# gmongaras/Stable-Diffusion-3-From-Scratch

Hardware: AMD Instinct MI355X
Metric: train images/sec MMDiT-B 256^2 bf16 (higher is better)
Workload: dtype bf16

## Files before the change

stable-diffusion-3-from-scratch_amd/_lib.py:

```python
import ctypes
import os
import re

_HERE = os.path.dirname(os.path.abspath(__file__))
def experiment(name: str, default: str) -> str:
    return os.environ.get(name, default) if os.environ.get("MMDIT_EXPERIMENTS") == "1" else default


LIB_PATH = os.environ.get("MMDIT_LIB") or os.path.join(_HERE, "libmmdit_hip.so")
HEADER_PATH = os.path.join(_HERE, "..", "include", "mmdit_hip.h")
HEADER_EXT_PATH = os.path.join(_HERE, "..", "include", "mmdit_hip_ext.h")
HEADER_HD128_PATH = os.path.join(_HERE, "..", "include", "mmdit_hip_hd128.h")
HEADER_ROPE3_PATH = os.path.join(_HERE, "..", "include", "mmdit_hip_rope3.h")

F32, BF16 = 0, 1
ACT_NONE, ACT_SILU, ACT_SWIGLU, ACT_SWIGLU_BWD = 0, 1, 2, 3
PREC_BF16, PREC_SPLIT = 0, 1
FP8 = 2

_vp, _i, _i64, _f, _d = ctypes.c_void_p, ctypes.c_int, ctypes.c_int64, ctypes.c_float, ctypes.c_double


class GemmArgs(ctypes.Structure):
    _fields_ = [
        ("A", _vp), ("a_dtype", _i), ("a_kmajor", _i), ("lda", _i64),
        ("B", _vp), ("b_dtype", _i), ("b_kmajor", _i), ("ldb", _i64),
        ("C", _vp), ("c_dtype", _i), ("ldc", _i64),
        ("M", _i), ("N", _i), ("K", _i),
        ("bias", _vp),
        ("act", _i),
        ("gate", _vp), ("ld_gate", _i64), ("rows_per_batch", _i),
        ("residual", _vp), ("ld_res", _i64),
        ("aux", _vp), ("aux_dtype", _i), ("ld_aux", _i64),
        ("accumulate", _i),
        ("precision", _i),
        ("split_k", _i),
        ("stream_k", _i),
        ("conv_mode", _i), ("conv_H", _i), ("conv_W", _i), ("conv_C", _i),
        ("scale_a", _vp), ("scale_b", _vp), ("scale_mode", _i), ("c_scales", _vp),
        ("dbias", _vp),
        ("cu_budget", _i),
    ]


class LnFwdProblem(ctypes.Structure):
    _fields_ = [("x", ctypes.c_void_p), ("acc", ctypes.c_void_p), ("gate", ctypes.c_void_p), ("ld_gate", ctypes.c_int64), ("x_out", ctypes.c_void_p),
                ("scale", ctypes.c_void_p), ("shift", ctypes.c_void_p), ("ld_mod", ctypes.c_int64), ("rows", ctypes.c_int), ("rows_per_batch", ctypes.c_int),
                ("out", ctypes.c_void_p), ("mean", ctypes.c_void_p), ("rstd", ctypes.c_void_p)]


class LnBwdProblem(ctypes.Structure):
    _fields_ = [("dout", ctypes.c_void_p), ("x", ctypes.c_void_p), ("mean", ctypes.c_void_p), ("rstd", ctypes.c_void_p), ("scale", ctypes.c_void_p),
                ("ld_mod", ctypes.c_int64), ("dres", ctypes.c_void_p), ("rows", ctypes.c_int), ("rows_per_batch", ctypes.c_int),
                ("dx", ctypes.c_void_p), ("dscale", ctypes.c_void_p), ("dshift", ctypes.c_void_p), ("ld_dmod", ctypes.c_int64),
                ("acc", ctypes.c_void_p), ("gate", ctypes.c_void_p), ("ld_gate", ctypes.c_int64), ("dacc", ctypes.c_void_p), ("dgate", ctypes.c_void_p),
                ("ld_dgate", ctypes.c_int64), ("dbias", ctypes.c_void_p), ("ld_dbias", ctypes.c_int64)]


class QkProblem(ctypes.Structure):
    _fields_ = [("qkv", ctypes.c_void_p), ("wq", ctypes.c_void_p), ("wk", ctypes.c_void_p), ("rope_cos", ctypes.c_void_p), ("rope_sin", ctypes.c_void_p),
                ("tokens", ctypes.c_int), ("tok0", ctypes.c_int), ("dqkv", ctypes.c_void_p), ("dwq", ctypes.c_void_p), ("dwk", ctypes.c_void_p)]


class MlpBwdProblem(ctypes.Structure):
    _fields_ = [("dh", ctypes.c_void_p), ("gu", ctypes.c_void_p), ("dgu", ctypes.c_void_p), ("rows", ctypes.c_int), ("dbias", ctypes.c_void_p)]


class QkEpilogue(ctypes.Structure):
    _fields_ = [("wq", _vp), ("wk", _vp), ("rope_cos", _vp), ("rope_sin", _vp), ("tokens", _i), ("tok0", _i)]


_SIGNATURES = {
    "mmdit_abi_version": ([], _i),
    "mmdit_struct_size": ([_i], _i),
    "mmdit_build_arch": ([], ctypes.c_char_p),
    "mmdit_gemm": ([ctypes.POINTER(GemmArgs), _vp], _i),
    "mmdit_gemm_grouped": ([ctypes.POINTER(GemmArgs), _i, _vp], _i),
    "mmdit_gemm_plan": ([ctypes.POINTER(GemmArgs), _i], _i),
    "mmdit_gemm_set_workspace": ([_vp, ctypes.c_longlong], _i),
    "mmdit_debug_occupy": ([_i, ctypes.c_longlong, _vp], _i),
    "mmdit_gemm_set_claiming": ([_i], _i),
    "mmdit_gemm_get_claiming": ([], _i),
    "mmdit_device_cus": ([], _i),
    "mmdit_gemm_qkv_norm_rope": ([ctypes.POINTER(GemmArgs), ctypes.POINTER(QkEpilogue), _i, _i, _i, _vp, _vp, _vp, _vp], _i),
    "mmdit_gemm_zero_mask": ([ctypes.POINTER(GemmArgs), _i, ctypes.POINTER(ctypes.c_uint)], _i),
    "mmdit_fp8_amax": ([_vp, _i, _i64, _vp, _vp], _i),
    "mmdit_fp8_quantize": ([_vp, _i, _i64, _vp, _vp, _vp, _vp], _i),
    "mmdit_fp8_quantize_delayed": ([_vp, _i, _i64, _vp, _i, ctypes.c_float, _vp, _vp], _i),
    "mmdit_mxfp8_quantize": ([_vp, _i, _i, _i, _i64, _vp, _vp, _vp], _i),
    "mmdit_ln_modulate_fwd_mx": ([_vp, _vp, _i, _vp, _i64, _vp, _vp, _vp, _i64, _i, _i, _i, _vp, _vp, _vp, _vp, _vp], _i),
    "mmdit_swiglu_fwd_mx": ([_vp, _i, _i, _i, _vp, _vp, _vp], _i),
    "mmdit_attn_fwd_mx": ([_vp, _vp, _vp, _i, _i, _i, _i, ctypes.c_float, _vp, _vp, _vp, _vp, _vp], _i),
    "mmdit_cast": ([_vp, _i, _vp, _i, _i64, _vp], _i),
    "mmdit_ln_modulate_fwd": ([ctypes.POINTER(LnFwdProblem), _i, _i, _i, _i, _vp], _i),
    "mmdit_ln_modulate_bwd": ([ctypes.POINTER(LnBwdProblem), _i, _i, _i, _vp], _i),
    "mmdit_qk_norm_rope_fwd": ([ctypes.POINTER(QkProblem), _i, _i, _i, _i, _i, _vp, _vp, _vp, _vp], _i),
    "mmdit_qk_norm_rope_bwd": ([ctypes.POINTER(QkProblem), _i, _vp, _vp, _vp, _i, _i, _i, _i, _i, _i, _vp], _i),
    "mmdit_qk_norm_rope_fwd_merge": ([ctypes.POINTER(QkProblem), _i, _i, _i, _i, _i, _vp, _vp, _vp, _vp], _i),
    "mmdit_qk_norm_rope_bwd_merge": ([ctypes.POINTER(QkProblem), _i, _vp, _vp, _vp, _i, _i, _i, _i, _i, _i, _vp], _i),
    "mmdit_mlp_act_bwd": ([ctypes.POINTER(MlpBwdProblem), _i, _i, _i, _i, _vp], _i),
    "mmdit_gate_residual_fwd": ([_vp, _vp, _i, _vp, _i64, _i, _i, _i, _vp, _vp], _i),
    "mmdit_text_rmsnorm_fwd": ([_vp, _i, _vp, _vp, _vp, _vp, _i, _i, _i, _i, _vp, _vp, _i, _vp], _i),
    "mmdit_text_rmsnorm_bwd": ([_vp, _vp, _i, _vp, _i, _vp, _vp, _vp, _vp, _i, _i, _i, _i, _vp, _vp, _vp, _vp, _vp], _i),
    "mmdit_attn_fwd": ([_vp, _vp, _vp, _i, _i, _i, _i, _f, _i, _vp, _vp, _vp, _vp], _i),
    "mmdit_attn_bwd_qk": ([_vp] * 9 + [_i, _i, _i, _i, _f] + [_vp] * 11 + [_vp], _i),
    "mmdit_attn_bwd": ([_vp, _vp, _vp, _vp, _vp, _vp, _vp, _vp, _vp, _i, _i, _i, _i, _f, _vp, _vp, _vp, _i, _vp], _i),
    "mmdit_attn_fwd_kv": ([_vp, _vp, _vp, _i, _i, _i, _i, _i, _f, _i, _vp, _vp, _vp, _vp], _i),
    "mmdit_attn_bwd_kv": ([_vp, _vp, _vp, _vp, _vp, _vp, _vp, _vp, _vp, _i, _i, _i, _i, _i, _f, _vp, _vp, _vp, _i, _vp], _i),
    "mmdit_swiglu_fwd": ([_vp, _vp, _i, _i, _i, _vp], _i),
    "mmdit_gelu_fwd": ([_vp, _vp, _i, _i, _i, _vp], _i),
    "mmdit_silu_bwd": ([_vp, _i, _vp, _vp, _i, _i, _i, _vp, _i, _vp], _i),
    "mmdit_gate_residual_bwd": ([_vp, _vp, _i, _vp, _i64, _i, _i, _i, _vp, _i, _vp, _i64, _vp, _i64, _vp], _i),
    "mmdit_flow_loss": ([_vp, _vp, _vp, _i, _i64, _f, _vp, _vp, _vp, _vp], _i),
    "mmdit_colsum": ([_vp, _i, _i, _i, _i64, _vp, _vp], _i),
    "mmdit_vae_nchw_to_nhwc": ([_vp, _i, _i, _i, _i, _i, _i, ctypes.c_float, ctypes.c_float, _vp, _vp], _i),
    "mmdit_vae_nhwc_to_nchw": ([_vp, _i, _i, _i, _i, _i, ctypes.c_float, ctypes.c_float, _vp, _vp], _i),
    "mmdit_vae_im2col3x3": ([_vp, _i, _i, _i, _i, _i, _vp, _vp], _i),
    "mmdit_vae_groupnorm": ([_vp, _i, _vp, _vp, _i, _i, _i, _i, _i, ctypes.c_float, _i, _vp, _vp, _i, _vp], _i),
    "mmdit_vae_pad_cast": ([_vp, _i, _i, _i, _i, _i, _i, _vp, _vp], _i),
    "mmdit_vae_softmax_rows": ([_vp, _i, _i, _i, ctypes.c_float, _vp, _vp], _i),
    "mmdit_vae_attn_fwd": ([_vp, _vp, _vp, _i, _i, _i, _i, _f, _vp, _vp], _i),
    "mmdit_patchify": ([_vp, _i, _i, _i, _i, _i, _vp, _i, _vp], _i),
    "mmdit_unpatchify": ([_vp, _i, _i, _i, _i, _i, _vp, _i, _vp], _i),
    "mmdit_time_embed_fwd": ([_vp, _vp, _vp, _i, _i, _vp, _i, _vp], _i),
    "mmdit_time_embed_bwd": ([_vp, _i, _vp, _vp, _vp, _i, _i, _vp, _vp], _i),
    "mmdit_grad_sumsq": ([_vp, _vp, _vp, _i, _vp, _vp], _i),
    "mmdit_clip_coef": ([_vp, _i, _vp, _f, _vp, _vp], _i),
    "mmdit_adamw_step": ([_vp, _vp, _vp, _i, _vp, _vp, _d, _d, _d, _d, _d, _vp], _i),
    "mmdit_adamw_step_dlr": ([_vp, _vp, _vp, _i, _vp, _vp, _vp, _d, _d, _d, _d, _vp], _i),
    "mmdit_cast_multi": ([_vp, _vp, _vp, _i, _vp], _i),
}
_EXT_SIGNATURES = {
    "mmdit_attn_fwd_e4m3": ([_vp, _vp, _vp, _i, _i, _i, _i, _f, _vp, _vp, _vp, _vp, _vp], _i),
}
ATTN_E4M3_KEY_TILE, ATTN_E4M3_QUERY_TILE = 64, 128
_HD128_SIGNATURES = {
    "mmdit_attn_fwd_hd128": _SIGNATURES["mmdit_attn_fwd"],
    "mmdit_attn_bwd_hd128": _SIGNATURES["mmdit_attn_bwd"],
    "mmdit_qk_norm_rope_fwd_hd128": _SIGNATURES["mmdit_qk_norm_rope_fwd"],
    "mmdit_qk_norm_rope_bwd_hd128": _SIGNATURES["mmdit_qk_norm_rope_bwd"],
}
ATTN_HD128_KEY_TILE, ATTN_HD128_QUERY_TILE = 32, 128
QK_HD128_MAX_HEADS, QK_HD128_RL_MIN_ROWS = 21, 2048
_ROPE3_SIGNATURES = {
    "mmdit_qk_norm_rope3_fwd": ([ctypes.POINTER(QkProblem), _i, _i, _i, _i, _i, _i, _vp, _vp, _vp, _vp], _i),
    "mmdit_qk_norm_rope3_bwd": ([ctypes.POINTER(QkProblem), _i, _vp, _vp, _vp, _i, _i, _i, _i, _i, _i, _i, _vp], _i),
}
HEAD_DIMS = (64, 128)
ADAMW_CHUNK = 65536
ABI_VERSION = 10
_STRUCTS = [("mmdit_gemm_args", GemmArgs), ("mmdit_ln_fwd_problem", LnFwdProblem), ("mmdit_ln_bwd_problem", LnBwdProblem),
            ("mmdit_qk_problem", QkProblem), ("mmdit_mlp_bwd_problem", MlpBwdProblem), ("mmdit_adamw_tensor", None), ("mmdit_cast_tensor", None), ("mmdit_qk_epilogue", QkEpilogue)]

_lib = None


def declared_symbols():
    with open(HEADER_PATH) as f:
        txt = f.read()
    return sorted(set(re.findall(r"\b(mmdit_[a-z0-9_]+)\s*\(", txt)) - {"mmdit_stream_t"})


def declared_ext_symbols():
    with open(HEADER_EXT_PATH) as f:
        txt = f.read()
    return sorted(set(re.findall(r"\b(mmdit_[a-z0-9_]+)\s*\(", txt)) - {"mmdit_stream_t"})


def declared_hd128_symbols():
    with open(HEADER_HD128_PATH) as f:
        txt = f.read()
    return sorted(set(re.findall(r"\b(mmdit_[a-z0-9_]+)\s*\(", txt)) - {"mmdit_stream_t"})


def declared_rope3_symbols():
    with open(HEADER_ROPE3_PATH) as f:
        txt = f.read()
    return sorted(set(re.findall(r"\b(mmdit_[a-z0-9_]+)\s*\(", txt)) - {"mmdit_stream_t"})


def lib():
    global _lib
    if _lib is None:
        if not os.path.exists(LIB_PATH):
            raise RuntimeError(
                f"{LIB_PATH} is missing: build it with `python __graft_entry__.py build` "
                "(hipcc --offload-arch=gfx950).  There is no PyTorch/CPU fallback for the MMDiT hot path.")
        try:
            import torch
            if torch.cuda.is_available():
                torch.cuda.init()
        except ImportError:
            pass
        L = ctypes.CDLL(LIB_PATH)
        for name, (argtypes, restype) in list(_SIGNATURES.items()) + list(_EXT_SIGNATURES.items()) + list(_HD128_SIGNATURES.items()) + list(_ROPE3_SIGNATURES.items()):
            fn = getattr(L, name)
            fn.argtypes = argtypes
            fn.restype = restype
        if L.mmdit_abi_version() != ABI_VERSION:
            raise RuntimeError(f"{LIB_PATH}: ABI version {L.mmdit_abi_version()}, this binding is written for {ABI_VERSION}: rebuild (python __graft_entry__.py build)")
        for which, (name, struct) in enumerate(_STRUCTS):
            if struct is not None and L.mmdit_struct_size(which) != ctypes.sizeof(struct):
                raise RuntimeError(f"{LIB_PATH}: sizeof({name}) = {L.mmdit_struct_size(which)}, the binding's ctypes mirror has {ctypes.sizeof(struct)} bytes")
        _lib = L
    return _lib


ERR_ARG, ERR_DTYPE, ERR_SHAPE = -1, -2, -3


def check(status: int, what: str):
    if status != 0:
        kind = {-1: "invalid argument", -2: "dtype combination not built", -3: "unsupported shape"}.get(status, f"hipError {status}")
        raise RuntimeError(f"{what} failed: {kind}")
```

stable-diffusion-3-from-scratch_amd/build.py:

```python
import hashlib
import os
import subprocess
import sys
from concurrent.futures import ThreadPoolExecutor

HERE = os.path.dirname(os.path.abspath(__file__))
CSRC = os.path.join(HERE, "csrc")
LIB = os.path.join(HERE, "libmmdit_hip.so")
HEADER = os.path.join(HERE, "..", "include", "mmdit_hip.h")
HEADER_EXT = os.path.join(HERE, "..", "include", "mmdit_hip_ext.h")
HEADER_HD128 = os.path.join(HERE, "..", "include", "mmdit_hip_hd128.h")
HEADER_ROPE3 = os.path.join(HERE, "..", "include", "mmdit_hip_rope3.h")
SOURCES = ["gemm.hip", "gemm_dma.hip", "gemm_lean.hip", "gemm8p.hip", "gemm8p_inf.hip", "rowops.hip", "attention.hip", "attention_e4m3.hip", "attention_hd128.hip", "rowops_rope3.hip", "vae.hip", "vae_attn.hip", "optim.hip"]
HIPCC = os.environ.get("HIPCC", "/opt/rocm/bin/hipcc")
FLAGS = ["--offload-arch=gfx950", "-O3", "-std=c++17", "-fPIC"] + os.environ.get("MMDIT_EXTRA_HIPCC_FLAGS", "").split()
SOURCE_FLAGS = {"vae_attn.hip": ["-mllvm", "-amdgpu-mfma-vgpr-form=1"]}


def _sha(paths, extra=""):
    h = hashlib.sha256(extra.encode())
    for p in paths:
        with open(p, "rb") as f:
            h.update(os.path.basename(p).encode() + b"\0" + f.read() + b"\0")
    return h.hexdigest()


def _read(path):
    try:
        with open(path) as f:
            return f.read().strip()
    except OSError:
        return None


def source_hash(src):
    headers = sorted(os.path.join(CSRC, f) for f in os.listdir(CSRC) if f.endswith(".h")) + [HEADER, HEADER_EXT, HEADER_HD128, HEADER_ROPE3]
    if src == "gemm8p_inf.hip":
        headers.append(os.path.join(CSRC, "gemm8p.hip"))
    return _sha([os.path.join(CSRC, src)] + headers, " ".join([HIPCC] + FLAGS + SOURCE_FLAGS.get(src, [])))


def build(force: bool = False, verbose: bool = False) -> str:
    want = {src: source_hash(src) for src in SOURCES}

    def cc(src):
        obj = os.path.join(CSRC, src.replace(".hip", ".o"))
        if not force and os.path.exists(obj) and _read(obj + ".sha") == want[src]:
            return obj, False
        cmd = [HIPCC] + FLAGS + SOURCE_FLAGS.get(src, []) + ["-c", os.path.join(CSRC, src), "-o", obj]
        if verbose:
            print(" ".join(cmd), flush=True)
        subprocess.run(cmd, check=True)
        with open(obj + ".sha", "w") as f:
            f.write(want[src])
        return obj, True

    with ThreadPoolExecutor(max_workers=8) as ex:
        res = list(ex.map(cc, SOURCES))
    objs = [o for o, _ in res]
    libsha = hashlib.sha256("".join(want[s] for s in SOURCES).encode()).hexdigest()
    if force or any(c for _, c in res) or not os.path.exists(LIB) or _read(LIB + ".sha") != libsha:
        cmd = [HIPCC, "--offload-arch=gfx950", "-shared", "-fPIC", "-o", LIB] + objs
        if verbose:
            print(" ".join(cmd), flush=True)
        subprocess.run(cmd, check=True)
        with open(LIB + ".sha", "w") as f:
            f.write(libsha)
    return LIB


def is_current() -> bool:
    libsha = hashlib.sha256("".join(source_hash(s) for s in SOURCES).encode()).hexdigest()
    return os.path.exists(LIB) and _read(LIB + ".sha") == libsha


if __name__ == "__main__":
    print(build(force="--force" in sys.argv, verbose=True))
```

stable-diffusion-3-from-scratch_amd/csrc/gemm.hip:

```cpp
#include "gemm_common.h"
#include <stdlib.h>

using namespace gemm;

namespace {

constexpr int BM = 128, BN = 128;
constexpr int RM_PITCH = 144;
constexpr int KM_PITCH = 320;
constexpr int TILE_BYTES = 20480;
constexpr int CHUNKS = 4;

template <typename T> struct Stage;
template <> struct Stage<bf16_t> { u32x4 v[CHUNKS]; };
template <> struct Stage<float> { f32x4 v[CHUNKS][2]; };

template <bool KM>
__device__ __forceinline__ void chunk_coords(int c, int& r, int& kc) {
  if (!KM) { r = c >> 3; kc = (c & 7) * 8; }
  else { kc = c >> 4; r = (c & 15) * 8; }
}

template <typename T, bool KM>
__device__ __forceinline__ void load_tile(Stage<T>& st, const T* base, int64_t ld, int row0, int k0, int rows, int K, int tid) {
#pragma unroll
  for (int i = 0; i < CHUNKS; i++) {
    int c = tid + 256 * i, r, kc;
    chunk_coords<KM>(c, r, kc);
    bool ok = (row0 + r < rows) && (k0 + kc < K);
    const T* p = KM ? base + (int64_t)(k0 + kc) * ld + row0 + r : base + (int64_t)(row0 + r) * ld + k0 + kc;
    if constexpr (sizeof(T) == 2) {
      st.v[i] = ok ? *(const u32x4*)p : (u32x4){0, 0, 0, 0};
    } else {
      st.v[i][0] = ok ? *(const f32x4*)p : (f32x4){0, 0, 0, 0};
      st.v[i][1] = ok ? *(const f32x4*)(p + 4) : (f32x4){0, 0, 0, 0};
    }
  }
}

template <typename T, bool KM, bool SPLIT>
__device__ __forceinline__ void store_tile(const Stage<T>& st, char* hi, char* mid, char* lo, int tid) {
#pragma unroll
  for (int i = 0; i < CHUNKS; i++) {
    int c = tid + 256 * i, r, kc;
    chunk_coords<KM>(c, r, kc);
    int off = KM ? kc * KM_PITCH + r * 2 : r * RM_PITCH + kc * 2;
    if constexpr (sizeof(T) == 2) {
      *LDS_PTR(u32x4, hi + off) = st.v[i];
    } else {
      float f[8] = {st.v[i][0][0], st.v[i][0][1], st.v[i][0][2], st.v[i][0][3], st.v[i][1][0], st.v[i][1][1], st.v[i][1][2], st.v[i][1][3]};
      uint32_t h[4], md[4], l[4];
#pragma unroll
      for (int j = 0; j < 4; j++) {
        bf16_t h0 = f2bf(f[2 * j]), h1 = f2bf(f[2 * j + 1]);
        h[j] = (uint32_t)h0 | ((uint32_t)h1 << 16);
        if constexpr (SPLIT) {
          const float r0 = f[2 * j] - bf2f(h0), r1 = f[2 * j + 1] - bf2f(h1);
          const bf16_t m0 = f2bf(r0), m1 = f2bf(r1);
          md[j] = (uint32_t)m0 | ((uint32_t)m1 << 16);
          l[j] = pack_bf2(r0 - bf2f(m0), r1 - bf2f(m1));
        }
      }
      *LDS_PTR(u32x4, hi + off) = (u32x4){h[0], h[1], h[2], h[3]};
      if constexpr (SPLIT) {
        *LDS_PTR(u32x4, mid + off) = (u32x4){md[0], md[1], md[2], md[3]};
        *LDS_PTR(u32x4, lo + off) = (u32x4){l[0], l[1], l[2], l[3]};
      }
    }
  }
}

template <bool KM>
__device__ __forceinline__ bf16x8 load_frag(const char* tile, int r0, int ks, int lane) {
  if (!KM) {
    const char* p = tile + (r0 + (lane & 31)) * RM_PITCH + (ks * 16 + (lane >> 5) * 8) * 2;
    return *LDS_PTR(const bf16x8, p);
  } else {
    int kr = ks * 16 + (lane >> 5) * 8 + ((lane & 15) >> 2);
    int col = r0 + 16 * ((lane >> 4) & 1) + (lane & 3) * 4;
    const char* p = tile + kr * KM_PITCH + col * 2;
    s16x4 lo = lds_tr16(p), hi = lds_tr16(p + 4 * KM_PITCH);
    s16x8 r = {lo[0], lo[1], lo[2], lo[3], hi[0], hi[1], hi[2], hi[3]};
    return __builtin_bit_cast(bf16x8, r);
  }
}

template <typename TA, typename TB, bool A_KM, bool B_KM, bool SPLIT, typename TC, typename TAUX>
__global__ __launch_bounds__(256) void gemm_kernel(GroupParams gp) {
  constexpr int NT = SPLIT ? 6 : 2;
  constexpr int NSTAGE = SPLIT ? 1 : 2;
  extern __shared__ __attribute__((aligned(16))) char smem[];

  int tm, tn, sk;
  const Problem& p = locate_tile(gp, blockIdx.x, tm, tn, sk);
  const int m0 = tm * BM, n0 = tn * BN;

  const int tid = threadIdx.x, lane = tid & 63, wave = tid >> 6;
  const int wm = wave >> 1, wn = wave & 1;
  const TA* A = (const TA*)p.A;
  const TB* B = (const TB*)p.B;
  const int M = p.M, N = p.N, K = p.K;
  const int64_t lda = p.lda, ldb = p.ldb;

  f32x16 acc[2][2];
#pragma unroll
  for (int i = 0; i < 2; i++)
#pragma unroll
    for (int j = 0; j < 2; j++)
#pragma unroll
      for (int r = 0; r < 16; r++) acc[i][j][r] = 0.f;

  Stage<TA> sa;
  Stage<TB> sb;
  const int nk = (K + BK - 1) / BK;
  auto tile_ptr = [&](int stage, int which) { return smem + (stage * NT + which) * TILE_BYTES; };

  load_tile<TA, A_KM>(sa, A, lda, m0, 0, M, K, tid);
  load_tile<TB, B_KM>(sb, B, ldb, n0, 0, N, K, tid);
  store_tile<TA, A_KM, SPLIT>(sa, tile_ptr(0, 0), tile_ptr(0, 2), tile_ptr(0, 4), tid);
  store_tile<TB, B_KM, SPLIT>(sb, tile_ptr(0, 1), tile_ptr(0, 3), tile_ptr(0, 5), tid);
  __syncthreads();

  int cur = 0;
  for (int kt = 0; kt < nk; kt++) {
    const bool more = kt + 1 < nk;
    if (more) {
      load_tile<TA, A_KM>(sa, A, lda, m0, (kt + 1) * BK, M, K, tid);
      load_tile<TB, B_KM>(sb, B, ldb, n0, (kt + 1) * BK, N, K, tid);
    }
    const char* ta = tile_ptr(cur, 0);
    const char* tb = tile_ptr(cur, 1);
#pragma unroll
    for (int ks = 0; ks < BK / 16; ks++) {
      bf16x8 a[2], b[2];
#pragma unroll
      for (int i = 0; i < 2; i++) a[i] = load_frag<A_KM>(ta, wm * 64 + i * 32, ks, lane);
#pragma unroll
      for (int j = 0; j < 2; j++) b[j] = load_frag<B_KM>(tb, wn * 64 + j * 32, ks, lane);
      if constexpr (SPLIT) {
        bf16x8 a1[2], b1[2], a2[2], b2[2];
#pragma unroll
        for (int i = 0; i < 2; i++) { a1[i] = load_frag<A_KM>(tile_ptr(cur, 2), wm * 64 + i * 32, ks, lane); a2[i] = load_frag<A_KM>(tile_ptr(cur, 4), wm * 64 + i * 32, ks, lane); }
#pragma unroll
        for (int j = 0; j < 2; j++) { b1[j] = load_frag<B_KM>(tile_ptr(cur, 3), wn * 64 + j * 32, ks, lane); b2[j] = load_frag<B_KM>(tile_ptr(cur, 5), wn * 64 + j * 32, ks, lane); }
#pragma unroll
        for (int i = 0; i < 2; i++)
#pragma unroll
          for (int j = 0; j < 2; j++) {
            acc[i][j] = __builtin_amdgcn_mfma_f32_32x32x16_bf16(b[j], a2[i], acc[i][j], 0, 0, 0);
            acc[i][j] = __builtin_amdgcn_mfma_f32_32x32x16_bf16(b1[j], a1[i], acc[i][j], 0, 0, 0);
            acc[i][j] = __builtin_amdgcn_mfma_f32_32x32x16_bf16(b2[j], a[i], acc[i][j], 0, 0, 0);
            acc[i][j] = __builtin_amdgcn_mfma_f32_32x32x16_bf16(b[j], a1[i], acc[i][j], 0, 0, 0);
            acc[i][j] = __builtin_amdgcn_mfma_f32_32x32x16_bf16(b1[j], a[i], acc[i][j], 0, 0, 0);
            acc[i][j] = __builtin_amdgcn_mfma_f32_32x32x16_bf16(b[j], a[i], acc[i][j], 0, 0, 0);
          }
      } else {
#pragma unroll
        for (int i = 0; i < 2; i++)
#pragma unroll
          for (int j = 0; j < 2; j++) acc[i][j] = __builtin_amdgcn_mfma_f32_32x32x16_bf16(b[j], a[i], acc[i][j], 0, 0, 0);
      }
    }
    if (more) {
      if constexpr (NSTAGE == 1) __syncthreads();
      const int nxt = NSTAGE == 1 ? 0 : cur ^ 1;
      store_tile<TA, A_KM, SPLIT>(sa, tile_ptr(nxt, 0), tile_ptr(nxt, 2), tile_ptr(nxt, 4), tid);
      store_tile<TB, B_KM, SPLIT>(sb, tile_ptr(nxt, 1), tile_ptr(nxt, 3), tile_ptr(nxt, 5), tid);
      __syncthreads();
      cur = nxt;
    }
  }

  __syncthreads();
  epilogue<TC, TAUX>(acc, p, gp, m0, n0, wm, wn, lane, sk, smem + wave * EP_WAVE_BYTES);
}

template <typename TA, typename TB, bool A_KM, bool B_KM, bool SPLIT, typename TC, typename TAUX>
int launch(const GroupParams& gp, hipStream_t s) {
  constexpr int smem = (SPLIT ? 6 : 4) * TILE_BYTES;
  auto k = gemm_kernel<TA, TB, A_KM, B_KM, SPLIT, TC, TAUX>;
  static unsigned long long attr_done = 0;
  if (!mmdit_device_once(attr_done)) {
    hipError_t e = hipFuncSetAttribute((const void*)k, hipFuncAttributeMaxDynamicSharedMemorySize, smem);
    if (e != hipSuccess) return (int)e;
    mmdit_device_mark(attr_done);
  }
  hipLaunchKernelGGL(k, dim3(gp.total_tiles), dim3(256), smem, s, gp);
  return mmdit_launch_status();
}

template <typename TA, typename TB, bool SPLIT, typename TC, typename TAUX>
int dispatch_layout(bool a_km, bool b_km, const GroupParams& p, hipStream_t s) {
  if (!a_km && !b_km) return launch<TA, TB, false, false, SPLIT, TC, TAUX>(p, s);
  if (!a_km && b_km) return launch<TA, TB, false, true, SPLIT, TC, TAUX>(p, s);
  if (a_km && b_km) return launch<TA, TB, true, true, SPLIT, TC, TAUX>(p, s);
  return MMDIT_ERR_DTYPE;
}

template <typename TA, typename TB, bool SPLIT>
int dispatch_out(int c_dt, int aux_dt, bool a_km, bool b_km, const GroupParams& p, hipStream_t s) {
  if (c_dt == MMDIT_F32 && aux_dt == MMDIT_F32) return dispatch_layout<TA, TB, SPLIT, float, float>(a_km, b_km, p, s);
  if (c_dt == MMDIT_F32 && aux_dt == MMDIT_BF16) return dispatch_layout<TA, TB, SPLIT, float, bf16_t>(a_km, b_km, p, s);
  if (c_dt == MMDIT_BF16 && aux_dt == MMDIT_BF16) return dispatch_layout<TA, TB, SPLIT, bf16_t, bf16_t>(a_km, b_km, p, s);
  if (c_dt == MMDIT_BF16 && aux_dt == MMDIT_F32) return dispatch_layout<TA, TB, SPLIT, bf16_t, float>(a_km, b_km, p, s);
  return MMDIT_ERR_DTYPE;
}

inline bool aligned16(const void* p) { return ((uintptr_t)p & 15) == 0; }

int check_problem(const mmdit_gemm_args* a) {
  MMDIT_CHECK_ARG(a->A && a->B && a->C);
  MMDIT_CHECK_ARG(a->M > 0 && a->N > 0 && a->K > 0 && a->N % 4 == 0);
  const int esa = a->a_dtype == MMDIT_F32 ? 4 : a->a_dtype == MMDIT_FP8 ? 1 : 2, esb = a->b_dtype == MMDIT_F32 ? 4 : a->b_dtype == MMDIT_FP8 ? 1 : 2, esc = a->c_dtype == MMDIT_F32 ? 4 : 2;
  MMDIT_CHECK_ARG(a->c_dtype == MMDIT_F32 || a->c_dtype == MMDIT_BF16 || (a->c_dtype == MMDIT_FP8 && a->act == MMDIT_ACT_SWIGLU && a->c_scales));
  MMDIT_CHECK_ARG(aligned16(a->A) && aligned16(a->B) && ((uintptr_t)a->C & (4 * esc - 1)) == 0);
  MMDIT_CHECK_ARG((a->lda * esa) % 16 == 0 && (a->ldb * esb) % 16 == 0 && a->ldc % 4 == 0);
  if (a->a_kmajor) { MMDIT_CHECK_ARG(a->M % 8 == 0 && a->lda >= a->M); } else { MMDIT_CHECK_ARG(a->K % 8 == 0 && a->lda >= a->K); }
  if (a->b_kmajor) { MMDIT_CHECK_ARG(a->N % 8 == 0 && a->ldb >= a->N); } else { MMDIT_CHECK_ARG(a->K % 8 == 0 && a->ldb >= a->K); }
  MMDIT_CHECK_ARG(a->ldc >= (a->act == MMDIT_ACT_SWIGLU ? a->N / 2 : a->act == MMDIT_ACT_SWIGLU_BWD ? 2 * a->N : a->N));
  if (a->bias) MMDIT_CHECK_ARG(aligned16(a->bias));
  if (a->gate) MMDIT_CHECK_ARG(a->residual && a->rows_per_batch > 0 && aligned16(a->gate) && a->ld_gate % 4 == 0);
  if (a->residual) MMDIT_CHECK_ARG(aligned16(a->residual) && a->ld_res % 4 == 0);
  if (a->aux) MMDIT_CHECK_ARG(a->ld_aux % 4 == 0 && ((uintptr_t)a->aux & 7) == 0);
  if (a->accumulate) MMDIT_CHECK_ARG(a->c_dtype == MMDIT_F32);
  return 0;
}

}

static void* g_ws[64] = {};
static long long g_ws_bytes[64] = {};
static unsigned g_sched_next[64] = {};
static int g_claiming[64] = {};
extern "C" int mmdit_gemm_set_claiming(int on) { g_claiming[mmdit_current_device()] = on != 0; return 0; }
extern "C" int mmdit_gemm_get_claiming(void) { return g_claiming[mmdit_current_device()]; }
extern "C" int mmdit_device_cus(void) {
  static int cus[64] = {};
  const int dev = mmdit_current_device();
  if (!cus[dev]) {
    int n = 0;
    if (hipDeviceGetAttribute(&n, hipDeviceAttributeMultiprocessorCount, dev) != hipSuccess || n < 8) { (void)hipGetLastError(); n = 256; }
    cus[dev] = n / 8 * 8;
  }
  return cus[dev];
}

struct PlannerSwitches {
  int cfg = -1, cfg_epi = -1;
  bool no_dma = false, no_streamk = false, no_persist = false;
  int lean = 1;
  bool qk8 = false;
  bool kdec_streamk = false, kdec_plain = false;
  int tail_s = 0, debug = 0;
  int epi_direct = 0, raster = 8;
};
#ifdef MMDIT_PROBES
static const PlannerSwitches& planner_switches() {
  static const PlannerSwitches sw = [] {
    PlannerSwitches w;
    auto num = [](const char* name, int& v) { if (const char* e = getenv(name)) v = atoi(e); };
    num("MMDIT_GEMM_CFG", w.cfg); num("MMDIT_GEMM_CFG_EPI", w.cfg_epi); num("MMDIT_GEMM_LEAN", w.lean); num("MMDIT_GEMM_TAIL_S", w.tail_s);
    num("MMDIT_GEMM_DEBUG", w.debug); num("MMDIT_GEMM_RASTER", w.raster);
    w.no_dma = getenv("MMDIT_GEMM_NO_DMA"); w.no_streamk = getenv("MMDIT_GEMM_NO_STREAMK"); w.no_persist = getenv("MMDIT_GEMM_NO_PERSIST");
    int qk8 = 0;
    num("MMDIT_QK_8PHASE", qk8); w.qk8 = qk8 > 0;
    if (const char* e = getenv("MMDIT_GEMM_EPI")) w.epi_direct = atoi(e) == 0;
    if (const char* e = getenv("MMDIT_GEMM_KDEC")) { w.kdec_streamk = e[0] == 's'; w.kdec_plain = e[0] == 'p'; }
    return w;
  }();
  return sw;
}
#else
static constexpr PlannerSwitches planner_switches() { return {}; }
#endif

static int pick_dma_cfg(const mmdit_gemm_args* args, int count, int split_k, bool stream_k, bool lean_ok, long cu) {
  const PlannerSwitches& sw = planner_switches();
  if (sw.cfg >= 0) return sw.cfg == CFG_320x256 && !lean_ok ? CFG_256x256 : sw.cfg;
  if (sw.cfg_epi >= 0 && args[0].gate) return sw.cfg_epi;
  if (stream_k) return CFG_256x256;
  long t128 = 0, t256 = 0;
  for (int i = 0; i < count; i++) {
    t128 += (long)((args[i].M + 127) / 128) * ((args[i].N + 127) / 128);
    t256 += (long)((args[i].M + 255) / 256) * ((args[i].N + 255) / 256);
  }
  const bool mx8 = args[0].a_dtype == MMDIT_FP8 && args[0].K % 128 == 0 && !args[0].gate && !args[0].residual && !args[0].aux &&
                   (args[0].c_dtype == MMDIT_BF16 || args[0].act == MMDIT_ACT_SWIGLU);
  const double r256 = mx8 ? 1.2 : args[0].a_dtype == MMDIT_FP8 ? 1.67 : 1.58;
  const double c128 = (double)((t128 * split_k + 2 * cu - 1) / (2 * cu)), c256 = r256 * (double)((t256 * split_k + cu - 1) / cu);
  if (lean_ok) {
    long t320 = 0;
    for (int i = 0; i < count; i++) t320 += (long)((args[i].M + 319) / 320) * ((args[i].N + 255) / 256);
    const double c320 = 1.25 * 1.58 * (double)((t320 + cu - 1) / cu);
    if (c320 < c256 && c320 < c128) return CFG_320x256;
  }
  return c256 < c128 ? CFG_256x256 : CFG_128x128;
}

static inline int split_k_of(const mmdit_gemm_args* a) { return a->split_k > 1 ? a->split_k : 1; }

struct QkRequest {
  const mmdit_qk_epilogue* qk;
  int heads, s_total;
  void* Q; void* K; void* V;
  unsigned no_raw;
};

enum GemmKernel { KERNEL_REG, KERNEL_DMA, KERNEL_WIDE, KERNEL_8P, KERNEL_8P_CONV };
struct GemmPlan {
  GroupParams gp;
  GemmKernel kernel;
  int cfg;
  bool a_km, b_km, fp8, mx8, ktail;
  int a_dt, b_dt, c_dt, aux_dt, precision;
  int cu;
  int* sched_page;
  int code;
  unsigned zero_mask;
};

struct DeviceState { bool claiming; void* ws; long long ws_bytes; };

static int choose_kernel(const mmdit_gemm_args* args, int count, const QkRequest* qkr, const DeviceState& ds, bool dma, bool conv, GemmPlan* pl) {
  const PlannerSwitches& sw = planner_switches();
  const mmdit_gemm_args* a0 = &args[0];
  const bool fp8 = pl->fp8;
  const int bk = fp8 ? 2 * BK : BK;
  const int split_k = split_k_of(a0);
  GroupParams& gp = pl->gp;
  gp.tail_first = -1; gp.tail_rounds = 0; gp.tail_G = 0;
  if (conv) MMDIT_CHECK_ARG(dma);
  const bool swiglu = a0->act == MMDIT_ACT_SWIGLU;
  if (swiglu) {
    if (!dma) return MMDIT_ERR_SHAPE;
    for (int i = 0; i < count; i++) {
      const mmdit_gemm_args* a = &args[i];
      MMDIT_CHECK_ARG(a->c_dtype == MMDIT_BF16 || (a->c_dtype == MMDIT_FP8 && a->c_scales && !a->aux && fp8 && a->scale_mode == 1 && a->c_dtype == a0->c_dtype));
      MMDIT_CHECK_ARG(!a->a_kmajor && !a->b_kmajor && (!a->aux || a->aux_dtype == MMDIT_BF16) && !a->gate && !a->residual &&
                      !a->accumulate && split_k == 1 && !a->stream_k && !a->conv_mode);
      if (a->N % 256 != 0) return MMDIT_ERR_SHAPE;
      MMDIT_CHECK_ARG(a->ldc >= a->N / 2 && a->ldc % 8 == 0 && aligned16(a->C));
      if (a->aux) MMDIT_CHECK_ARG(a->ld_aux >= a->N && a->ld_aux % 8 == 0 && aligned16(a->aux));
    }
  }
  const bool swiglu_bwd = a0->act == MMDIT_ACT_SWIGLU_BWD;
  if (swiglu_bwd) {
    if (!dma) return MMDIT_ERR_SHAPE;
    for (int i = 0; i < count; i++) {
      const mmdit_gemm_args* a = &args[i];
      MMDIT_CHECK_ARG(a->c_dtype == MMDIT_BF16 && !a->a_kmajor && a->b_kmajor && a->aux && a->aux_dtype == MMDIT_BF16 && !a->bias && !a->gate && !a->residual &&
                      !a->accumulate && split_k == 1 && !a->stream_k && !a->conv_mode && !fp8);
      MMDIT_CHECK_ARG(a->N % 8 == 0 && a->ldc >= 2 * a->N && a->ldc % 8 == 0 && aligned16(a->C) && a->ld_aux >= 2 * a->N && a->ld_aux % 8 == 0 && aligned16(a->aux));
      if (a->dbias) MMDIT_CHECK_ARG(((uintptr_t)a->dbias & 3) == 0);
    }
  }
  int bm = BM, bn = BN, cfg = CFG_128x128;
  const bool stream_k = dma && !sw.no_streamk && a0->stream_k && a0->c_dtype == MMDIT_F32 && split_k == 1 && a0->act == MMDIT_ACT_NONE && !a0->accumulate;
  bool lean_ok = dma && sw.lean > 0 && !fp8 && !conv && !stream_k && split_k == 1 && !a0->a_kmajor && a0->c_dtype == MMDIT_BF16 &&
                 (a0->act == MMDIT_ACT_NONE || a0->act == MMDIT_ACT_SILU || swiglu || swiglu_bwd) && !a0->accumulate;
  for (int i = 0; i < count && lean_ok; i++) {
    const mmdit_gemm_args* a = &args[i];
    lean_ok = (!a->aux || swiglu || swiglu_bwd) && !a->gate && !a->residual && a->N % 8 == 0 && a->ldc % 8 == 0 && aligned16(a->C) && (!a->b_kmajor || a->N >= 8);
  }
  if (dma) {
    cfg = pick_dma_cfg(args, count, split_k, stream_k, lean_ok, pl->cu);
    if (swiglu && cfg != CFG_320x256) cfg = CFG_256x256;
    if (swiglu_bwd) cfg = CFG_256x256;
    if (qkr && (fp8 || sw.qk8 || ds.claiming)) cfg = CFG_256x256;
    dma_cfg_tile(cfg, bm, bn);
  }
  const bool lean = lean_ok && (cfg == CFG_320x256 || (cfg == CFG_256x256 && sw.lean == 1));
  int tiles = 0, units = 0;
  int order[MAXG];
  for (int i = 0; i < count; i++) order[i] = i;
  if (stream_k && !sw.kdec_streamk)
    for (int i = 1; i < count; i++)
      for (int j = i; j > 0 && args[order[j]].K > args[order[j - 1]].K; j--) { const int t = order[j]; order[j] = order[j - 1]; order[j - 1] = t; }
  for (int i = 0; i < count; i++) {
    const mmdit_gemm_args* a = &args[order[i]];
    Problem& p = gp.p[i];
    p.A = a->A; p.B = a->B; p.C = a->C; p.aux = a->aux;
    p.bias = a->bias; p.gate = a->gate; p.residual = a->residual;
    p.lda = a->lda; p.ldb = a->ldb; p.ldc = a->ldc; p.ld_gate = a->ld_gate; p.ld_res = a->ld_res; p.ld_aux = a->ld_aux;
    p.M = a->M; p.N = a->N; p.K = a->K;
    p.rows_per_batch = a->rows_per_batch > 0 ? a->rows_per_batch : 1;
    p.conv_mode = a->conv_mode; p.cC = a->conv_C; p.cHp = a->conv_H + 2; p.cWp = a->conv_W + 2;
    p.cHo = a->conv_mode == 2 ? a->conv_H / 2 : a->conv_H; p.cWo = a->conv_mode == 2 ? a->conv_W / 2 : a->conv_W;
    p.tiles_n = (a->N + bn - 1) / bn;
    p.tiles_m = (a->M + bm - 1) / bm;
    p.tile_start = tiles;
    p.nk = a->K / bk;
    p.scale_a = (const float*)a->scale_a; p.scale_b = (const float*)a->scale_b; p.c_scales = (unsigned char*)a->c_scales;
    p.dbias = a->dbias;
    p.unit_start = units;
    tiles += p.tiles_n * p.tiles_m;
    units += p.tiles_n * p.tiles_m * p.nk;
    if (stream_k) MMDIT_CHECK_ARG(!a->aux && !a->gate && a->stream_k);
  }
  gp.stream_k = stream_k; gp.total_units = units;
  gp.mx = fp8 && a0->scale_mode == 1;
  int full_tiles = split_k > 1 ? 0 : tiles, tail_split = split_k;
  const bool tail_mode = stream_k && !sw.kdec_streamk;
  if (tail_mode) {
    gp.stream_k = 0;
    const int G = pl->cu * (cfg == CFG_128x128 ? 2 : 1), r = tiles % G;
    int nk_min = 1 << 30;
    for (int i = 0; i < count; i++) nk_min = gp.p[i].nk < nk_min ? gp.p[i].nk : nk_min;
    full_tiles = tiles - r;
    tail_split = 1;
    if (r) {
      double best = 1e30;
      for (int S = 1; S <= 64 && S * 2 <= nk_min; S++) {
        const double c = (double)((r * S + G - 1) / G) / S + (S > 1 ? 0.0028 * r * S : 0.0);
        if (c < best) { best = c; tail_split = S; }
      }
      if (sw.tail_s > 0 && sw.tail_s * 2 <= nk_min) { tail_split = sw.tail_s; best = -1.0; }
      if (full_tiles == G && !sw.kdec_plain) {
        const int nk_max = gp.p[0].nk;
        int first_short = G, nk_short = 0, nk_tail = 0;
        for (int i = 0; i < count; i++) {
          const Problem& q = gp.p[i];
          if (q.nk < nk_max && q.tile_start < G && first_short == G) { first_short = q.tile_start; nk_short = q.nk; }
          if (q.tile_start + q.tiles_m * q.tiles_n > full_tiles) nk_tail = q.nk > nk_tail ? q.nk : nk_tail;
        }
        const int E = G - first_short;
        if (E > 0) {
          double bbest = 1e30;
          int bS = 0, brounds = 0;
          for (int S = 1; S <= 64 && S * 2 <= nk_min; S++) {
            const int rounds = (r * S + E - 1) / E, extra = rounds * ((nk_tail + S - 1) / S);
            const double load = (double)(nk_short + extra) / nk_max, c = (load > 1.0 ? load - 1.0 : 0.0) + (S > 1 ? 0.0028 * r * S : 0.0);
            if (c < bbest) { bbest = c; bS = S; brounds = rounds; }
          }
          if (bbest < best) {
            tail_split = bS;
            if (!(ds.ws && ds.claiming)) { gp.tail_first = first_short; gp.tail_rounds = brounds; gp.tail_G = G; }
          }
        }
      }
    }
  }
  gp.persistent = !sw.no_persist;
  gp.count = count; gp.total_tiles = tiles; gp.act = a0->act; gp.accumulate = a0->accumulate; gp.split_k = tail_split; gp.full_tiles = full_tiles;
  gp.debug = sw.debug; gp.epi_direct = sw.epi_direct; gp.raster = sw.raster;
  if (split_k > 1) {
    MMDIT_CHECK_ARG(dma && a0->c_dtype == MMDIT_F32 && a0->act == MMDIT_ACT_NONE && !a0->accumulate && split_k <= 64);
    for (int i = 0; i < count; i++) MMDIT_CHECK_ARG(!args[i].aux && !args[i].gate);
  }
  bool wgrad8 = dma && !fp8 && !conv && !gp.stream_k && cfg == CFG_256x256 && a0->a_kmajor && a0->b_kmajor &&
            a0->c_dtype == MMDIT_F32 && a0->act == MMDIT_ACT_NONE;
  for (int i = 0; i < count && wgrad8; i++) {
    const mmdit_gemm_args* a = &args[i];
    wgrad8 = !a->bias && !a->gate && !a->residual && !a->aux && a->N % 4 == 0 && a->ldc % 4 == 0 && aligned16(a->C);
  }
  gp.ws_slots = nullptr; gp.ws_count = nullptr; gp.sched = nullptr;
  gp.qk_on = 0; gp.qkQ = gp.qkK = gp.qkV = nullptr; gp.qk_heads = 0; gp.qk_s_total = 0;
  if (qkr) {
    const bool mxqk = dma && fp8 && gp.mx && cfg == CFG_256x256 && !a0->a_kmajor && a0->c_dtype == MMDIT_BF16;
    if (!(lean || mxqk) || count > 2 || a0->act != MMDIT_ACT_NONE || a0->b_kmajor) return MMDIT_ERR_SHAPE;
    if (qkr->no_raw && !(cfg == CFG_256x256 && (mxqk || ds.claiming))) return MMDIT_ERR_SHAPE;
    for (int i = 0; i < count; i++) {
      if (order[i] != i || args[i].bias || args[i].N != 3 * qkr->heads * 64 || qkr->qk[i].tokens <= 0 || args[i].M % qkr->qk[i].tokens) return MMDIT_ERR_SHAPE;
      gp.qk[i].wq = qkr->qk[i].wq; gp.qk[i].wk = qkr->qk[i].wk;
      gp.qk[i].rcos = qkr->qk[i].rope_cos; gp.qk[i].rsin = qkr->qk[i].rope_sin;
      gp.qk[i].tokens = qkr->qk[i].tokens; gp.qk[i].tok0 = qkr->qk[i].tok0;
    }
    if (count == 1) gp.qk[1] = gp.qk[0];
    for (int i = 0; i < count; i++)
      if ((qkr->no_raw >> i) & 1) gp.p[i].C = nullptr;
    gp.qk_on = 1; gp.qk_heads = qkr->heads; gp.qk_s_total = qkr->s_total;
    gp.qkQ = (bf16_t*)qkr->Q; gp.qkK = (bf16_t*)qkr->K; gp.qkV = (bf16_t*)qkr->V;
  }
  if (wgrad8 && gp.split_k > 1) {
    const long long tail_tiles = tiles - full_tiles;
    if (ds.ws && tail_tiles <= 1024 && 8192 + tail_tiles * gp.split_k * 65536LL * 4 <= ds.ws_bytes) {
      gp.ws_count = (int*)ds.ws;
      gp.ws_slots = (float*)((char*)ds.ws + 8192);
    }
  }
  pl->zero_mask = 0;
  for (int i = 0; i < count; i++) {
    const Problem& q = gp.p[i];
    if (dma && !gp.ws_slots && (gp.stream_k || (gp.split_k > 1 && q.tile_start + q.tiles_m * q.tiles_n > gp.full_tiles))) pl->zero_mask |= 1u << order[i];
  }
  bool mx8 = dma && fp8 && cfg == CFG_256x256 && (!qkr || gp.mx) && !stream_k && split_k == 1 && (a0->act == MMDIT_ACT_NONE || swiglu) && !a0->accumulate;
  for (int i = 0; i < count && mx8; i++) {
    const mmdit_gemm_args* a = &args[i];
    mx8 = (a->c_dtype == MMDIT_BF16 || (swiglu && a->c_dtype == MMDIT_FP8)) && (!a->aux || (swiglu && a->c_dtype == MMDIT_BF16)) && !a->gate && !a->residual && a->K % 128 == 0 &&
          a->N % 8 == 0 && a->ldc % 8 == 0 && aligned16(a->C) && (int64_t)a->M * a->lda < (1ll << 32) && (int64_t)a->N * a->ldb < (1ll << 32);
  }
  const bool p8 = mx8 || wgrad8 || (lean && (cfg == CFG_256x256 || (cfg == CFG_320x256 && !qkr)));
  bool conv8 = conv && dma && !fp8 && cfg == CFG_256x256 && !stream_k && split_k == 1 && a0->act == MMDIT_ACT_NONE && !a0->accumulate &&
               (a0->c_dtype == MMDIT_BF16 || a0->c_dtype == MMDIT_F32);
  for (int i = 0; i < count && conv8; i++) {
    const mmdit_gemm_args* a = &args[i];
    conv8 = a->conv_mode && a->conv_C % 64 == 0 && !a->aux && !a->gate && (a->c_dtype == MMDIT_F32 || !a->residual) && a->N % 8 == 0 && a->ldc % 8 == 0 && aligned16(a->C) &&
            (!a->residual || (a->ld_res % 4 == 0 && aligned16(a->residual))) && (!a->bias || aligned16(a->bias));
  }
  if (swiglu_bwd && !p8) return MMDIT_ERR_SHAPE;
  pl->kernel = conv8 ? KERNEL_8P_CONV : p8 ? KERNEL_8P : lean ? KERNEL_WIDE : dma ? KERNEL_DMA : KERNEL_REG;
  pl->cfg = cfg; pl->mx8 = mx8;
  pl->code = dma ? (cfg | (gp.stream_k ? 16 : 0) | (tail_mode ? 32 : 0) | (lean || wgrad8 ? 128 : 0) | (p8 || conv8 ? 256 : 0)) : 64;
  const bool claimed = pl->kernel == KERNEL_8P && !mx8 && cfg == CFG_256x256 && gp.persistent && gp.tail_first < 0 && total_work(gp) > pl->cu;
  pl->sched_page = claimed && ds.ws && ds.claiming ? (int*)((char*)ds.ws + 4096) : nullptr;
  return 0;
}

static int plan_gemm(const mmdit_gemm_args* args, int count, const QkRequest* qkr, GemmPlan* pl) {
  MMDIT_CHECK_ARG(args && count >= 1 && count <= MAXG);
  const mmdit_gemm_args* a0 = &args[0];
  const int dev = mmdit_current_device();
  const DeviceState ds{g_claiming[dev] != 0, g_ws[dev], g_ws_bytes[dev]};
  const int cus = mmdit_device_cus();
  MMDIT_CHECK_ARG(a0->cu_budget == 0 || (a0->cu_budget >= 64 && a0->cu_budget <= cus && a0->cu_budget % 8 == 0));
  pl->cu = a0->cu_budget ? a0->cu_budget : cus;
  int aux_dt = -1;
  const bool fp8 = a0->a_dtype == MMDIT_FP8 || a0->b_dtype == MMDIT_FP8;
  bool dma = !planner_switches().no_dma && a0->precision == MMDIT_PREC_BF16 && a0->a_dtype == MMDIT_BF16 && a0->b_dtype == MMDIT_BF16;
  bool ktail = false;
  if (fp8) {
    MMDIT_CHECK_ARG(a0->a_dtype == MMDIT_FP8 && a0->b_dtype == MMDIT_FP8 && a0->precision == MMDIT_PREC_BF16 && split_k_of(a0) == 1 && !a0->stream_k);
    dma = true;
  }
  const int bk = fp8 ? 2 * BK : BK;
  bool conv = false;
  const int split_k = split_k_of(a0);
  for (int i = 0; i < count; i++) {
    const mmdit_gemm_args* a = &args[i];
    int rc = check_problem(a);
    if (rc) return rc;
    MMDIT_CHECK_ARG(a->a_dtype == a0->a_dtype && a->b_dtype == a0->b_dtype && a->c_dtype == a0->c_dtype && a->a_kmajor == a0->a_kmajor &&
                    a->b_kmajor == a0->b_kmajor && a->precision == a0->precision && a->act == a0->act && a->accumulate == a0->accumulate &&
                    a->cu_budget == a0->cu_budget);
    if (a->aux) { MMDIT_CHECK_ARG(aux_dt < 0 || aux_dt == a->aux_dtype); aux_dt = a->aux_dtype; }
    MMDIT_CHECK_ARG(split_k_of(a) == split_k);
    if (fp8) MMDIT_CHECK_ARG(!a->a_kmajor && !a->b_kmajor && a->K % bk == 0 && a->scale_a && a->scale_b && !a->conv_mode && a->scale_mode == a0->scale_mode &&
                             (a->scale_mode == 0 || (a->scale_mode == 1 && aligned16(a->scale_a) && aligned16(a->scale_b))));
    if (a->K % bk != 0) {
      if (!fp8 && a->a_kmajor && a->b_kmajor && a->c_dtype == MMDIT_F32 && a->K > bk && !a->conv_mode) ktail = true;
      else dma = false;
    }
    if (a->a_kmajor && a->M < 8) dma = false;
    if (a->b_kmajor && a->N < 8) dma = false;
    if (a->conv_mode) {
      MMDIT_CHECK_ARG((a->conv_mode == 1 || a->conv_mode == 2) && !a->a_kmajor && !a->b_kmajor && a->conv_C > 0 && a->conv_C % 32 == 0 && a->K == 9 * a->conv_C && a->K % BK == 0);
      MMDIT_CHECK_ARG(a->conv_H > 0 && a->conv_W > 0 && (a->conv_mode == 1 || (a->conv_H % 2 == 0 && a->conv_W % 2 == 0)));
      const int64_t px = a->conv_mode == 1 ? (int64_t)a->conv_H * a->conv_W : (int64_t)(a->conv_H / 2) * (a->conv_W / 2);
      MMDIT_CHECK_ARG(a->M % px == 0 && split_k == 1 && !a->stream_k && a->a_dtype == MMDIT_BF16 && a->b_dtype == MMDIT_BF16 && a->precision == MMDIT_PREC_BF16);
      MMDIT_CHECK_ARG((a->M / px) * (int64_t)(a->conv_H + 2) * (a->conv_W + 2) * a->conv_C * 2 < (1ll << 32));
      conv = true;
      continue;
    }
    if ((int64_t)(a->a_kmajor ? a->K : a->M) * a->lda * 2 >= (1ll << 32) || (int64_t)(a->b_kmajor ? a->K : a->N) * a->ldb * 2 >= (1ll << 32)) {
      MMDIT_CHECK_ARG(!fp8);
      dma = false;
    }
  }
  pl->a_km = a0->a_kmajor; pl->b_km = a0->b_kmajor; pl->fp8 = fp8; pl->ktail = ktail;
  pl->a_dt = a0->a_dtype; pl->b_dt = a0->b_dtype; pl->c_dt = a0->c_dtype; pl->precision = a0->precision;
  pl->aux_dt = aux_dt >= 0 ? aux_dt : a0->c_dtype == MMDIT_FP8 ? MMDIT_BF16 : a0->c_dtype;
  int rc = choose_kernel(args, count, qkr, ds, dma, conv, pl);
  if (rc == 0 && dma && ktail && pl->kernel != KERNEL_8P) rc = choose_kernel(args, count, qkr, ds, false, conv, pl);
  return rc;
}

static int launch_plan(const GemmPlan& pl, hipStream_t s) {
  const GroupParams* gp = &pl.gp;
  GroupParams claimed;
  if (pl.sched_page) {
    claimed = pl.gp;
    claimed.sched = pl.sched_page + (__atomic_fetch_add(&g_sched_next[mmdit_current_device()], 1u, __ATOMIC_RELAXED) & 63u) * 16;
    gp = &claimed;
  }
  switch (pl.kernel) {
    case KERNEL_8P_CONV: return launch_gemm8_conv(pl.c_dt == MMDIT_F32, *gp, s, pl.cu);
    case KERNEL_8P: return launch_gemm8(pl.cfg, pl.a_km, pl.b_km, *gp, s, pl.cu, pl.ktail, pl.mx8);
    case KERNEL_WIDE: return launch_lean_cfg(pl.cfg, pl.b_km, *gp, s, pl.cu);
    case KERNEL_DMA: return launch_dma(pl.cfg, pl.a_km, pl.b_km, pl.c_dt, pl.aux_dt, pl.fp8, *gp, s, pl.cu);
    case KERNEL_REG:
      if (pl.precision == MMDIT_PREC_BF16 && pl.a_dt == MMDIT_BF16 && pl.b_dt == MMDIT_BF16) return dispatch_out<bf16_t, bf16_t, false>(pl.c_dt, pl.aux_dt, pl.a_km, pl.b_km, *gp, s);
      if (pl.precision == MMDIT_PREC_SPLIT && pl.a_dt == MMDIT_F32 && pl.b_dt == MMDIT_F32) return dispatch_out<float, float, true>(pl.c_dt, pl.aux_dt, pl.a_km, pl.b_km, *gp, s);
      return MMDIT_ERR_DTYPE;
  }
  return MMDIT_ERR_ARG;
}

extern "C" int mmdit_gemm_grouped(const mmdit_gemm_args* args, int count, mmdit_stream_t stream) {
  GemmPlan pl;
  const int rc = plan_gemm(args, count, nullptr, &pl);
  return rc ? rc : launch_plan(pl, (hipStream_t)stream);
}

extern "C" int mmdit_gemm_qkv_norm_rope(const mmdit_gemm_args* args, const mmdit_qk_epilogue* qk, int count, int heads, int s_total,
                                        void* Q, void* K, void* V, mmdit_stream_t stream) {
  MMDIT_CHECK_ARG(args && qk && count >= 1 && count <= 2 && heads > 0 && s_total > 0 && Q && K && V);
  for (int i = 0; i < count; i++) {
    MMDIT_CHECK_ARG(qk[i].wq && qk[i].wk && qk[i].tokens > 0 && qk[i].tok0 >= 0 && qk[i].tok0 + qk[i].tokens <= s_total);
    MMDIT_CHECK_ARG((qk[i].rope_cos == nullptr) == (qk[i].rope_sin == nullptr));
  }
  mmdit_gemm_args tmp[2];
  unsigned no_raw = 0;
  for (int i = 0; i < count; i++) {
    tmp[i] = args[i];
    if (!tmp[i].C) { tmp[i].C = Q; no_raw |= 1u << i; }
  }
  const QkRequest r{qk, heads, s_total, Q, K, V, no_raw};
  GemmPlan pl;
  const int rc = plan_gemm(no_raw ? tmp : args, count, &r, &pl);
  return rc ? rc : launch_plan(pl, (hipStream_t)stream);
}

extern "C" int mmdit_gemm_set_workspace(void* ptr, long long bytes) {
  MMDIT_CHECK_ARG((ptr == nullptr && bytes == 0) || (ptr != nullptr && bytes >= 8192 + 65536 * 4 && ((uintptr_t)ptr & 15) == 0));
  const int dev = mmdit_current_device();
  g_ws[dev] = ptr;
  g_ws_bytes[dev] = bytes;
  return 0;
}

namespace {
__global__ void occupy_kernel(long long cycles, int* sink) {
  __shared__ int pad[256];
  pad[threadIdx.x & 255] = threadIdx.x;
  const long long t0 = __builtin_readcyclecounter();
  while ((long long)__builtin_readcyclecounter() - t0 < cycles) __builtin_amdgcn_s_sleep(32);
  if (cycles < 0) sink[0] = pad[0];
}
}
extern "C" int mmdit_debug_occupy(int wgs, long long cycles, mmdit_stream_t stream) {
  MMDIT_CHECK_ARG(wgs >= 1 && wgs <= 256 && cycles >= 0 && cycles <= (1ll << 36));
  hipLaunchKernelGGL(occupy_kernel, dim3(wgs), dim3(64), 0, (hipStream_t)stream, cycles, (int*)nullptr);
  return mmdit_launch_status();
}

extern "C" int mmdit_gemm_plan(const mmdit_gemm_args* args, int count) {
  GemmPlan pl;
  const int rc = plan_gemm(args, count, nullptr, &pl);
  return rc ? rc : pl.code;
}

extern "C" int mmdit_gemm_zero_mask(const mmdit_gemm_args* args, int count, unsigned* mask) {
  MMDIT_CHECK_ARG(mask);
  GemmPlan pl;
  const int rc = plan_gemm(args, count, nullptr, &pl);
  *mask = rc ? 0 : pl.zero_mask;
  return rc;
}

extern "C" int mmdit_gemm(const mmdit_gemm_args* a, mmdit_stream_t stream) {
  MMDIT_CHECK_ARG(a);
  return mmdit_gemm_grouped(a, 1, stream);
}
```

stable-diffusion-3-from-scratch_amd/csrc/gemm8p.hip:

```cpp
#include "gemm_tile.h"

using namespace gemm;
typedef __attribute__((ext_vector_type(4))) int i32x4_t;

namespace {

template <int MT> struct Geo {
  static constexpr int QR = MT / 4, FI = QR / 16;
  static constexpr int HTA = 2 * QR * 128, HTB = 16384;
  static constexpr int KBUF = 2 * HTA + 2 * HTB;
  static constexpr int XA0 = 0, XA1 = HTA, XB0 = 2 * HTA, XB1 = 2 * HTA + HTB;
  static constexpr int PA = 2 * QR / 8;
  static constexpr int PAW = (PA + 7) / 8;
  static constexpr int STAGE0 = MT == 256 ? 2 * KBUF : 0;
  static constexpr int SMEM = MT == 256 ? 2 * KBUF + 8 * EP32_WAVE_BYTES : 2 * KBUF;
  static constexpr int NB32 = MT / 64;
};

enum Epi8 { EPI_BF16 = 0, EPI_SWIGLU = 1, EPI_QK = 2, EPI_F32 = 3, EPI_SWIGLU_BWD = 4, EPI_F32R = 5 };

#define SWZ_R(r) (((r) >> 1) & 7)
#define SWZ_K(k) ((((k) & 3) << 2) ^ ((((k) >> 3) & 1) << 1))

template <int MT> struct AccT { f32x4 a[2][2][2 * Geo<MT>::FI]; };

template <int MT>
__device__ __forceinline__ f32x4& grp(AccT<MT>& acc, int i32, int q) {
  constexpr int FI = Geo<MT>::FI;
  const int f16 = i32 * 2 + (q >> 2), j16 = q & 3;
  return acc.a[f16 / FI][j16 >> 1][(f16 % FI) * 2 + (j16 & 1)];
}

template <int MT, bool SC = false, bool LAUNDER = SC>
__device__ __forceinline__ void epi8_bf16(AccT<MT>& acc, const Problem& p, const GroupParams& gp, int m0, int n0, int wm, int wn, int lane, char* stage, float alpha = 1.f) {
  bf16_t* C = (bf16_t*)p.C;
  const float* bias = p.bias;
  const int wr = lane & 15, wq = lane >> 4;
  const int rr = lane >> 3, rc = lane & 7;
  const int colw = n0 + wn * 64;
  float bv[4][4];
  if (bias) {
#pragma unroll
    for (int j = 0; j < 4; j++) {
      const int c = colw + j * 16 + wq * 4;
      ld4(bias + (c < p.N ? c : 0), bv[j]);
      if (c >= p.N) bv[j][0] = bv[j][1] = bv[j][2] = bv[j][3] = 0.f;
    }
  }
#ifdef MMDIT_PROBES
  if (gp.debug & 64) {
#pragma unroll
    for (int i = 0; i < Geo<MT>::NB32; i++)
#pragma unroll
      for (int q = 0; q < 8; q++) {
        const f32x4& a = grp(acc, i, q);
        float v[4] = {a[0], a[1], a[2], a[3]};
        if (bias) {
#pragma unroll
          for (int e = 0; e < 4; e++) v[e] += bv[q & 3][e];
        }
        if (gp.act == MMDIT_ACT_SILU) {
#pragma unroll
          for (int e = 0; e < 4; e++) v[e] = silu_f(v[e]);
        }
        const int row = m0 + wm * (MT / 2) + i * 32 + (q >> 2) * 16 + wr, col = colw + (q & 3) * 16 + wq * 4;
        if (row < p.M && col < p.N) *(u32x2*)(C + (int64_t)row * p.ldc + col) = (u32x2){pack_bf2(v[0], v[1]), pack_bf2(v[2], v[3])};
      }
    return;
  }
  if (gp.debug & 32) {
#pragma unroll
    for (int i = 0; i < Geo<MT>::NB32; i++)
#pragma unroll
      for (int it = 0; it < 4; it++) {
        const f32x4& a = grp(acc, i, it);
        const int row = m0 + wm * (MT / 2) + i * 32 + it * 8 + rr, col = colw + rc * 8;
        if (row < p.M && col < p.N) *(u32x4*)(C + (int64_t)row * p.ldc + col) = __builtin_bit_cast(u32x4, a);
      }
    return;
  }
#endif
#pragma unroll
  for (int i = 0; i < Geo<MT>::NB32; i++) {
    int ln = lane;
    if constexpr (LAUNDER) asm volatile("" : "+v"(ln));
    const int wr = ln & 15, wq = ln >> 4, rr = ln >> 3, rc = ln & 7;
#pragma unroll
    for (int q = 0; q < 8; q++) {
      const f32x4& a = grp(acc, i, q);
      float v[4] = {a[0], a[1], a[2], a[3]};
      if constexpr (SC) {
#pragma unroll
        for (int e = 0; e < 4; e++) v[e] *= alpha;
      }
      if (bias) {
#pragma unroll
        for (int e = 0; e < 4; e++) v[e] += bv[q & 3][e];
      }
      if (gp.act == MMDIT_ACT_SILU) {
#pragma unroll
        for (int e = 0; e < 4; e++) v[e] = silu_f(v[e]);
      }
      const int row = (q >> 2) * 16 + wr, chunk = (q & 3) * 2 + (wq >> 1);
      *LDS_PTR(u32x2, stage + row * 128 + ((chunk ^ (row & 7)) << 4) + (wq & 1) * 8) = (u32x2){pack_bf2(v[0], v[1]), pack_bf2(v[2], v[3])};
    }
    asm volatile("s_waitcnt lgkmcnt(0)" ::: "memory");
    const int col = colw + rc * 8;
#pragma unroll
    for (int it = 0; it < 4; it++) {
      const int r = it * 8 + rr;
      const u32x4 t = *LDS_PTR(const u32x4, stage + r * 128 + ((rc ^ (r & 7)) << 4));
      const int row = m0 + wm * (MT / 2) + i * 32 + r;
#ifdef MMDIT_PROBES
      if (gp.debug & 16) { if (t[0] == 0x12345678u) *(u32x4*)(C + (int64_t)row * p.ldc + col) = t; continue; }
#endif
#ifdef MMDIT_PROBES
      if (gp.debug & 1024) { if (row < p.M && col < p.N) __builtin_nontemporal_store(t, (u32x4*)(C + (int64_t)row * p.ldc + col)); continue; }
#endif
      if (row < p.M && col < p.N) *(u32x4*)(C + (int64_t)row * p.ldc + col) = t;
    }
    asm volatile("s_waitcnt lgkmcnt(0)" ::: "memory");
  }
}

template <int MT>
__device__ __forceinline__ void epi8_swiglu_bwd(AccT<MT>& acc, const Problem& p, int m0, int n0, int wm, int wn, int lane, char* stage) {
  constexpr int NB = Geo<MT>::NB32;
  const bf16_t* GU = (const bf16_t*)p.aux;
  bf16_t* D = (bf16_t*)p.C;
  const int wr = lane & 15, wq = lane >> 4;
  const int rr = lane >> 3, rc = lane & 7;
  const int col = n0 + wn * 64 + rc * 8;
  const bool cok = col < p.N;
  const int row0 = m0 + wm * (MT / 2) + rr;
  u32x4 gq[2][4], uq[2][4];
  const int colc = cok ? col : p.N - 8;
  auto request = [&](int i, int b) __attribute__((always_inline)) {
#pragma unroll
    for (int it = 0; it < 4; it++) {
      const int row = min(row0 + i * 32 + it * 8, p.M - 1);
      const bf16_t* src = GU + (int64_t)row * p.ld_aux + colc;
      gq[b][it] = __builtin_nontemporal_load((const u32x4*)src);
      uq[b][it] = __builtin_nontemporal_load((const u32x4*)(src + p.N));
    }
  };
  float sg[8], su[8];
#pragma unroll
  for (int e = 0; e < 8; e++) sg[e] = su[e] = 0.f;
  request(0, 0);
#pragma unroll
  for (int i = 0; i < NB; i++) {
    if (i + 1 < NB) request(i + 1, (i + 1) & 1);
#pragma unroll
    for (int q = 0; q < 8; q++) {
      const f32x4& a = grp(acc, i, q);
      const int row = (q >> 2) * 16 + wr, chunk = (q & 3) * 2 + (wq >> 1);
      *LDS_PTR(u32x2, stage + row * 128 + ((chunk ^ (row & 7)) << 4) + (wq & 1) * 8) = (u32x2){pack_bf2(a[0], a[1]), pack_bf2(a[2], a[3])};
    }
    asm volatile("s_waitcnt lgkmcnt(0)" ::: "memory");
#pragma unroll
    for (int it = 0; it < 4; it++) {
      const int r = it * 8 + rr;
      const u32x4 t = *LDS_PTR(const u32x4, stage + r * 128 + ((rc ^ (r & 7)) << 4));
      const int row = row0 + i * 32 + it * 8;
      const u32x4 gw = gq[i & 1][it], uw = uq[i & 1][it];
      float og[8], ou[8];
#pragma unroll
      for (int e = 0; e < 4; e++) {
#pragma unroll
        for (int h = 0; h < 2; h++) {
          const float d = __builtin_bit_cast(float, h ? t[e] & 0xffff0000u : t[e] << 16);
          const float g = __builtin_bit_cast(float, h ? gw[e] & 0xffff0000u : gw[e] << 16);
          const float u = __builtin_bit_cast(float, h ? uw[e] & 0xffff0000u : uw[e] << 16);
          swiglu_bwd_f(d, g, u, og[2 * e + h], ou[2 * e + h]);
        }
      }
      if (row < p.M && cok) {
#pragma unroll
        for (int e = 0; e < 8; e++) { sg[e] += og[e]; su[e] += ou[e]; }
        bf16_t* dst = D + (int64_t)row * p.ldc + col;
        st8_uncounted(dst, og);
        st8_uncounted(dst + p.N, ou);
      }
    }
    asm volatile("s_waitcnt lgkmcnt(0)" ::: "memory");
  }
  if (p.dbias) {
#pragma unroll
    for (int e = 0; e < 8; e++) {
#pragma unroll
      for (int o = 8; o < 64; o <<= 1) { sg[e] += __shfl_xor(sg[e], o, 64); su[e] += __shfl_xor(su[e], o, 64); }
    }
    if (rr == 0 && cok) {
#pragma unroll
      for (int e = 0; e < 8; e++) { atomicAdd(p.dbias + col + e, sg[e]); atomicAdd(p.dbias + p.N + col + e, su[e]); }
    }
  }
}

template <int MT>
__device__ __forceinline__ void epi8_qk(AccT<MT>& acc, const Problem& p, const GroupParams& gp, const QkEpi& e, int m0, int n0, int wm, int wn, int lane, char* stage) {
  bf16_t* C = (bf16_t*)p.C;
  const int colw = n0 + wn * 64;
  const int D = gp.qk_heads * 64, part = colw / D, head = (colw - part * D) >> 6;
  if (colw >= p.N) return;
  bf16_t* obase = part == 0 ? gp.qkQ : part == 1 ? gp.qkK : gp.qkV;
  const int rowt = m0 + wm * (MT / 2);
  const bool rope = e.rcos != nullptr;
  const float* tc = rope ? e.rcos : e.wq;
  const float* ts = rope ? e.rsin : e.wq;
  float w8[8], cb[2][8], sb[2][8];
#pragma unroll
  for (int q = 0; q < 8; q++) w8[q] = 0.f;
  if (part < 2) ld8((part == 0 ? e.wq : e.wk) + (lane & 7) * 8, w8);
  auto token_of = [&](int rowb, int b0, int r, int& b, int& n) __attribute__((always_inline)) {
    b = b0; n = rowb - b0 * e.tokens + r;
    if (e.tokens >= 32) { if (n >= e.tokens) { n -= e.tokens; b++; } }
    else { b = (rowb + r) / e.tokens; n = rowb + r - b * e.tokens; }
  };
  auto request = [&](int i, int it, int ln, float (&cn)[8], float (&sn)[8]) __attribute__((always_inline)) {
    const int rowb = rowt + i * 32;
    const int b0 = __builtin_amdgcn_readfirstlane(rowb / e.tokens);
    int b, n;
    token_of(rowb, b0, it * 8 + (ln >> 3), b, n);
    n = rope ? min(n, e.tokens - 1) : 0;
    ld8(tc + (int64_t)n * 64 + (ln & 7) * 8, cn);
    ld8(ts + (int64_t)n * 64 + (ln & 7) * 8, sn);
  };
  auto stage_block = [&](int i, int ln) __attribute__((always_inline)) {
    const int wr = ln & 15, wq = ln >> 4;
#pragma unroll
    for (int q = 0; q < 8; q++) {
      const f32x4& a = grp(acc, i, q);
      const int row = (q >> 2) * 16 + wr, chunk = (q & 3) * 2 + (wq >> 1);
      *LDS_PTR(u32x2, stage + row * 128 + ((chunk ^ (row & 7)) << 4) + (wq & 1) * 8) = (u32x2){pack_bf2(a[0], a[1]), pack_bf2(a[2], a[3])};
    }
    asm volatile("s_waitcnt lgkmcnt(0)" ::: "memory");
  };
  if (part == 2) {
#pragma unroll
    for (int i = 0; i < Geo<MT>::NB32; i++) {
      int ln = lane;
      asm volatile("" : "+v"(ln));
      stage_block(i, ln);
      const int rr = ln >> 3, rc = ln & 7;
      const int rowb = rowt + i * 32;
      const int b0 = __builtin_amdgcn_readfirstlane(rowb / e.tokens);
#pragma unroll
      for (int it = 0; it < 4; it++) {
        const int r = it * 8 + rr;
        const u32x4 t = *LDS_PTR(const u32x4, stage + r * 128 + ((rc ^ (r & 7)) << 4));
        int b, n;
        token_of(rowb, b0, r, b, n);
        if (rowb + r < p.M) *(u32x4*)(obase + (((int64_t)b * gp.qk_heads + head) * gp.qk_s_total + e.tok0 + n) * 64 + rc * 8) = t;
      }
      asm volatile("s_waitcnt lgkmcnt(0)" ::: "memory");
    }
    return;
  }
  auto qk_loop = [&](auto full_t, auto raw_t) __attribute__((always_inline)) {
    constexpr bool FULL = decltype(full_t)::value;
    constexpr bool RAW = decltype(raw_t)::value;
    request(0, 0, lane, cb[0], sb[0]);
#pragma unroll
    for (int i = 0; i < Geo<MT>::NB32; i++) {
      int ln = lane;
      asm volatile("" : "+v"(ln));
      stage_block(i, ln);
      const int rr = ln >> 3, rc = ln & 7;
      const int col = colw + rc * 8;
      const int rowb = rowt + i * 32;
      const int b0 = __builtin_amdgcn_readfirstlane(rowb / e.tokens);
#pragma unroll
      for (int it = 0; it < 4; it++) {
        const int r = it * 8 + rr;
        const u32x4 t = *LDS_PTR(const u32x4, stage + r * 128 + ((rc ^ (r & 7)) << 4));
        const int row = rowb + r;
        int b, n;
        token_of(rowb, b0, r, b, n);
        bf16_t* dst = obase + (((int64_t)b * gp.qk_heads + head) * gp.qk_s_total + e.tok0 + n) * 64 + rc * 8;
        const int cur = (i * 4 + it) & 1;
        float (&c8)[8] = cb[cur];
        float (&s8)[8] = sb[cur];
        if (it < 3) request(i, it + 1, ln, cb[cur ^ 1], sb[cur ^ 1]);
        else if (i + 1 < Geo<MT>::NB32) request(i + 1, 0, ln, cb[cur ^ 1], sb[cur ^ 1]);
        float x[8];
#pragma unroll
        for (int q = 0; q < 4; q++) { x[2 * q] = __builtin_bit_cast(float, t[q] << 16); x[2 * q + 1] = __builtin_bit_cast(float, t[q] & 0xffff0000u); }
        float ss = 0.f;
#pragma unroll
        for (int q = 0; q < 8; q++) ss += x[q] * x[q];
        ss = sum8(ss);
        const float rinv = rsqrtf(ss * (1.f / 64.f) + 1.1920929e-07f);
#pragma unroll
        for (int q = 0; q < 8; q++) x[q] = x[q] * rinv * w8[q];
        if (rope) {
#pragma unroll
          for (int q = 0; q < 4; q++) {
            const float a = x[2 * q], bb = x[2 * q + 1];
            x[2 * q] = a * c8[2 * q] - bb * s8[2 * q];
            x[2 * q + 1] = bb * c8[2 * q + 1] + a * s8[2 * q + 1];
          }
        }
        if (FULL || row < p.M) {
          if constexpr (RAW) *(u32x4*)(C + (int64_t)row * p.ldc + col) = t;
          st8(dst, x);
        }
      }
      asm volatile("s_waitcnt lgkmcnt(0)" ::: "memory");
    }
  };
  using std::integral_constant;
  const bool full = m0 + MT <= p.M;
  if (C) {
    if (full) qk_loop(integral_constant<bool, true>{}, integral_constant<bool, true>{});
    else qk_loop(integral_constant<bool, false>{}, integral_constant<bool, true>{});
  } else {
    if (full) qk_loop(integral_constant<bool, true>{}, integral_constant<bool, false>{});
    else qk_loop(integral_constant<bool, false>{}, integral_constant<bool, false>{});
  }
}

template <int MT, bool MXOUT = false>
__device__ __forceinline__ void epi8_swiglu(AccT<MT>& acc, const Problem& p, int m0, int tn, int wm, int wn, int lane, char* stage, float alpha = 1.f) {
  bf16_t* Hout = (bf16_t*)p.C;
  bf16_t* GU = (bf16_t*)p.aux;
  const float* bias = p.bias;
  const int h = p.N >> 1;
  const int wr = lane & 15, wq = lane >> 4;
  const int hc = tn * 128 + wn * 32;
  float bgv[2][4], buv[2][4];
#pragma unroll
  for (int j = 0; j < 2; j++)
#pragma unroll
    for (int e = 0; e < 4; e++) bgv[j][e] = buv[j][e] = 0.f;
  if (bias) {
#pragma unroll
    for (int j = 0; j < 2; j++) {
      ld4(bias + hc + j * 16 + wq * 4, bgv[j]);
      ld4(bias + h + hc + j * 16 + wq * 4, buv[j]);
    }
  }
#pragma unroll
  for (int i = 0; i < Geo<MT>::NB32; i++) {
    u32x2 pa[2][2];
    int ln = lane;
    if constexpr (MXOUT) asm volatile("" : "+v"(ln));
    const int wr = ln & 15, wq = ln >> 4;
#pragma unroll
    for (int il = 0; il < 2; il++)
#pragma unroll
      for (int j = 0; j < 2; j++) {
        const f32x4& ag = grp(acc, i, il * 4 + j);
        const f32x4& au = grp(acc, i, il * 4 + 2 + j);
        float vg[4] = {ag[0], ag[1], ag[2], ag[3]}, vu[4] = {au[0], au[1], au[2], au[3]};
        if constexpr (MXOUT) {
#pragma unroll
          for (int e = 0; e < 4; e++) { vg[e] *= alpha; vu[e] *= alpha; }
        }
#pragma unroll
        for (int e = 0; e < 4; e++) { vg[e] += bgv[j][e]; vu[e] += buv[j][e]; }
        const u32x2 pg = {pack_bf2(vg[0], vg[1]), pack_bf2(vg[2], vg[3])}, pu = {pack_bf2(vu[0], vu[1]), pack_bf2(vu[2], vu[3])};
        const int row = il * 16 + wr;
        if (GU) {
          *LDS_PTR(u32x2, stage + row * 128 + (((j * 2 + (wq >> 1)) ^ (row & 7)) << 4) + (wq & 1) * 8) = pg;
          *LDS_PTR(u32x2, stage + row * 128 + (((4 + j * 2 + (wq >> 1)) ^ (row & 7)) << 4) + (wq & 1) * 8) = pu;
        }
        float a[4];
#pragma unroll
        for (int e = 0; e < 2; e++) {
          const float g0 = __builtin_bit_cast(float, pg[e] << 16), g1 = __builtin_bit_cast(float, pg[e] & 0xffff0000u);
          const float u0 = __builtin_bit_cast(float, pu[e] << 16), u1 = __builtin_bit_cast(float, pu[e] & 0xffff0000u);
          a[2 * e] = silu_f(g0) * u0;
          a[2 * e + 1] = silu_f(g1) * u1;
        }
        pa[il][j] = u32x2{pack_bf2(a[0], a[1]), pack_bf2(a[2], a[3])};
      }
    asm volatile("s_waitcnt lgkmcnt(0)" ::: "memory");
    if (GU) {
      const int rr = ln >> 3, rc = ln & 7;
      const int col = (rc & 4 ? h : 0) + hc + (rc & 3) * 8;
#pragma unroll
      for (int it = 0; it < 4; it++) {
        const int r = it * 8 + rr;
        const u32x4 t = *LDS_PTR(const u32x4, stage + r * 128 + ((rc ^ (r & 7)) << 4));
        const int row = m0 + wm * (MT / 2) + i * 32 + r;
        if (row < p.M) __builtin_nontemporal_store(t, (u32x4*)(GU + (int64_t)row * p.ld_aux + col));
      }
    }
    asm volatile("s_waitcnt lgkmcnt(0)" ::: "memory");
    if (MXOUT && p.c_scales) {
#pragma unroll
      for (int il = 0; il < 2; il++) {
        float hv[8];
#pragma unroll
        for (int j = 0; j < 2; j++)
#pragma unroll
          for (int e = 0; e < 2; e++) { hv[4 * j + 2 * e] = __builtin_bit_cast(float, pa[il][j][e] << 16); hv[4 * j + 2 * e + 1] = __builtin_bit_cast(float, pa[il][j][e] & 0xffff0000u); }
        float amax = 0.f;
#pragma unroll
        for (int e = 0; e < 8; e++) amax = fmaxf(amax, fabsf(hv[e]));
        amax = fmaxf(amax, __shfl_xor(amax, 16, 64));
        amax = fmaxf(amax, __shfl_xor(amax, 32, 64));
        float inv;
        const int ex = mx_exponent(amax, inv);
        const int row = il * 16 + wr;
#pragma unroll
        for (int j = 0; j < 2; j++) *LDS_PTR(unsigned, stage + row * 32 + j * 16 + wq * 4) = mx_pack4(hv + 4 * j, inv);
        const int myrow = m0 + wm * (MT / 2) + i * 32 + row;
        if (wq == 0 && myrow < p.M) p.c_scales[mx_scale_index(myrow, hc >> 5, p.M)] = (unsigned char)(ex + 127);
      }
      asm volatile("s_waitcnt lgkmcnt(0)" ::: "memory");
      const int r = ln >> 1, row = m0 + wm * (MT / 2) + i * 32 + r;
      const u32x4 t = *LDS_PTR(const u32x4, stage + r * 32 + (ln & 1) * 16);
      if (row < p.M) *(u32x4*)((unsigned char*)p.C + (int64_t)row * p.ldc + hc + (ln & 1) * 16) = t;
      asm volatile("s_waitcnt lgkmcnt(0)" ::: "memory");
      continue;
    }
#pragma unroll
    for (int il = 0; il < 2; il++)
#pragma unroll
      for (int j = 0; j < 2; j++) {
        const int row = il * 16 + wr;
        *LDS_PTR(u32x2, stage + row * 64 + (((j * 2 + (wq >> 1)) ^ (row & 3)) << 4) + (wq & 1) * 8) = pa[il][j];
      }
    asm volatile("s_waitcnt lgkmcnt(0)" ::: "memory");
    {
      const int rr = ln >> 2, rc = ln & 3;
#pragma unroll
      for (int it = 0; it < 2; it++) {
        const int r = it * 16 + rr;
        const u32x4 t = *LDS_PTR(const u32x4, stage + r * 64 + ((rc ^ (r & 3)) << 4));
        const int row = m0 + wm * (MT / 2) + i * 32 + r;
        if (row < p.M) *(u32x4*)(Hout + (int64_t)row * p.ldc + hc + rc * 8) = t;
      }
    }
    asm volatile("s_waitcnt lgkmcnt(0)" ::: "memory");
  }
}

template <int MT>
__device__ __forceinline__ void epi8_f32(AccT<MT>& acc, const Problem& p, int m0, int n0, int wm, int wn, int lane, char* stage, bool atomic_out, bool accumulate) {
  float* C = (float*)p.C;
  const int wr = lane & 15, wq = lane >> 4;
  const int rr = lane >> 3, rc = lane & 7;
#pragma unroll
  for (int i = 0; i < Geo<MT>::NB32; i++)
#pragma unroll
    for (int j = 0; j < 2; j++) {
      const int col = n0 + wn * 64 + j * 32 + rc * 4;
      const int row0 = m0 + wm * (MT / 2) + i * 32 + rr;
#pragma unroll
      for (int il = 0; il < 2; il++)
#pragma unroll
        for (int jj = 0; jj < 2; jj++) {
          const int row = il * 16 + wr;
          *LDS_PTR(f32x4, stage + row * 128 + (((jj * 4 + wq) ^ (row & 7)) << 4)) = grp(acc, i, il * 4 + j * 2 + jj);
        }
      asm volatile("s_waitcnt lgkmcnt(0)" ::: "memory");
#pragma unroll
      for (int it = 0; it < 4; it++) {
        const int r = it * 8 + rr;
        f32x4 t = *LDS_PTR(const f32x4, stage + r * 128 + ((rc ^ (r & 7)) << 4));
        const int row = row0 + it * 8;
        if (row >= p.M || col >= p.N) continue;
        float* cp = C + (int64_t)row * p.ldc + col;
        if (atomic_out) {
#pragma unroll
          for (int e = 0; e < 4; e++) atomicAdd(cp + e, t[e]);
          continue;
        }
        if (accumulate) t += *(const f32x4*)cp;
        __builtin_nontemporal_store(t, (f32x4*)cp);
      }
      asm volatile("s_waitcnt lgkmcnt(0)" ::: "memory");
    }
}

template <int MT>
__device__ __forceinline__ void epi8_f32r(AccT<MT>& acc, const Problem& p, int m0, int n0, int wm, int wn, int lane, char* stage) {
  float* C = (float*)p.C;
  constexpr int NBLK = Geo<MT>::NB32 * 2;
  const int wr = lane & 15, wq = lane >> 4;
  const int rr = lane >> 3, rc = lane & 7;
  const int rowt = m0 + wm * (MT / 2) + rr;
  const int colj[2] = {n0 + wn * 64 + rc * 4, n0 + wn * 64 + 32 + rc * 4};
  f32x4 b4[2] = {{0.f, 0.f, 0.f, 0.f}, {0.f, 0.f, 0.f, 0.f}};
  if (p.bias) {
#pragma unroll
    for (int j = 0; j < 2; j++) b4[j] = *(const f32x4*)(p.bias + min(colj[j], p.N - 4));
  }
  auto stage_block = [&](int k) __attribute__((always_inline)) {
    const int i = k >> 1, j = k & 1;
#pragma unroll
    for (int il = 0; il < 2; il++)
#pragma unroll
      for (int jj = 0; jj < 2; jj++) {
        const int row = il * 16 + wr;
        *LDS_PTR(f32x4, stage + row * 128 + (((jj * 4 + wq) ^ (row & 7)) << 4)) = grp(acc, i, il * 4 + j * 2 + jj);
      }
    asm volatile("s_waitcnt lgkmcnt(0)" ::: "memory");
  };
  if (!p.residual) {
#pragma unroll
    for (int k = 0; k < NBLK; k++) {
      stage_block(k);
      const int col = colj[k & 1];
#pragma unroll
      for (int it = 0; it < 4; it++) {
        const int r = it * 8 + rr;
        f32x4 t = *LDS_PTR(const f32x4, stage + r * 128 + ((rc ^ (r & 7)) << 4));
        const int row = rowt + (k >> 1) * 32 + it * 8;
        if (row >= p.M || col >= p.N) continue;
        t += b4[k & 1];
        *(f32x4*)(C + (int64_t)row * p.ldc + col) = t;
      }
      asm volatile("s_waitcnt lgkmcnt(0)" ::: "memory");
    }
    return;
  }
  f32x4 res[2][4];
  auto request = [&](int k, f32x4 (&dst)[4]) __attribute__((always_inline)) {
    const int col = min(colj[k & 1], p.N - 4);
#pragma unroll
    for (int it = 0; it < 4; it++) {
      const int row = min(rowt + (k >> 1) * 32 + it * 8, p.M - 1);
      dst[it] = *(const f32x4*)(p.residual + (int64_t)row * p.ld_res + col);
    }
  };
  request(0, res[0]);
#pragma unroll
  for (int k = 0; k < NBLK; k++) {
    if (k + 1 < NBLK) request(k + 1, res[(k + 1) & 1]);
    stage_block(k);
    const int col = colj[k & 1];
#pragma unroll
    for (int it = 0; it < 4; it++) {
      const int r = it * 8 + rr;
      f32x4 t = *LDS_PTR(const f32x4, stage + r * 128 + ((rc ^ (r & 7)) << 4));
      const int row = rowt + (k >> 1) * 32 + it * 8;
      t += b4[k & 1];
      t += res[k & 1][it];
      if (row < p.M && col < p.N) st16_uncounted(C + (int64_t)row * p.ldc + col, __builtin_bit_cast(u32x4, t));
    }
    asm volatile("s_waitcnt lgkmcnt(0)" ::: "memory");
  }
}

template <int MT>
__device__ __forceinline__ void epi8_f32_slot(AccT<MT>& acc, float* slot, int wm, int wn, int lane, char* stage) {
#pragma unroll
  for (int i = 0; i < Geo<MT>::NB32; i++)
#pragma unroll
    for (int j = 0; j < 2; j++) {
      int ln = lane;
      asm volatile("" : "+v"(ln));
      const int wr = ln & 15, wq = ln >> 4;
      const int rr = ln >> 3, rc = ln & 7;
#pragma unroll
      for (int il = 0; il < 2; il++)
#pragma unroll
        for (int jj = 0; jj < 2; jj++) {
          const int row = il * 16 + wr;
          *LDS_PTR(f32x4, stage + row * 128 + (((jj * 4 + wq) ^ (row & 7)) << 4)) = grp(acc, i, il * 4 + j * 2 + jj);
        }
      asm volatile("s_waitcnt lgkmcnt(0)" ::: "memory");
#pragma unroll
      for (int it = 0; it < 4; it++) {
        const int r = it * 8 + rr;
        const f32x4 t = *LDS_PTR(const f32x4, stage + r * 128 + ((rc ^ (r & 7)) << 4));
        float* dst = slot + (int64_t)(wm * (MT / 2) + i * 32 + r) * 256 + wn * 64 + j * 32 + rc * 4;
        asm volatile("global_store_dwordx4 %0, %1, off sc1" ::"v"(dst), "v"(t) : "memory");
      }
      asm volatile("s_waitcnt lgkmcnt(0)" ::: "memory");
    }
}

#define BAR8() asm volatile("s_barrier" ::: "memory")
#define LGKM0() asm volatile("s_waitcnt lgkmcnt(0)" ::: "memory")
#define VMCNT8(n) asm volatile("s_waitcnt vmcnt(%0)" ::"n"(n) : "memory")

template <int MT, bool A_KM, bool B_KM, int EPI, bool KT = false, bool MX = false, bool CONV = false, bool PT = false>
__global__ __launch_bounds__(512) void gemm8_kernel(GroupParams gp) {
  static_assert(!PT || MX, "per-tensor scales: the e4m3-operand kernel");
  static_assert(MT == 256 || MT == 320, "tile rows");
  static_assert(!CONV || (!A_KM && !B_KM && MT == 256 && !MX && (EPI == EPI_BF16 || EPI == EPI_F32R)), "implicit-GEMM convolution: row-major operands, 256-row tiles");
  static_assert(EPI != EPI_F32R || (!A_KM && MT == 256), "fp32 + residual epilogue: row-major A, 256-row tiles");
  static_assert(!MX || (!A_KM && !B_KM && MT == 256 && (EPI == EPI_BF16 || EPI == EPI_SWIGLU || EPI == EPI_QK)), "MX: row-major e4m3 operands, 256-row tiles, bf16 / SwiGLU / QKV epilogue");
  static_assert(!KT || (A_KM && B_KM && EPI == EPI_F32), "K tail: the weight-gradient kernel");
  static_assert(EPI == EPI_F32 ? (A_KM && B_KM && MT == 256) : !A_KM, "fp32 epilogue = weight gradients (both operands k-major, 256 rows); bf16 epilogues take a row-major A");
  static_assert(!(EPI == EPI_SWIGLU || EPI == EPI_QK) || !B_KM, "fused epilogues: row-major weight");
  static_assert(EPI != EPI_SWIGLU_BWD || (B_KM && MT == 256), "SwiGLU backward epilogue: the data-gradient layout, 256-row tiles");
  using GE = Geo<MT>;
  constexpr int QR = GE::QR, FI = GE::FI, KBUF = GE::KBUF, XA0 = GE::XA0, XA1 = GE::XA1, XB0 = GE::XB0, XB1 = GE::XB1, PAW = GE::PAW;
  extern __shared__ __attribute__((aligned(1024))) char smem[];
  const int tid = threadIdx.x, lane = tid & 63, wave = __builtin_amdgcn_readfirstlane(tid >> 6);
  const int wr = wave >> 2, wc = wave & 3;
  const uint32_t lds0 = (uint32_t)(uintptr_t)LDS_PTR(char, smem);
  const uint32_t ldsw = lds0 + wave * 1024;
  const int G = (int)gridDim.x;
  const bool hiw = wave + 8 * (PAW - 1) < GE::PA;

  int pos = (int)blockIdx.x, end = total_work(gp);
  if (gp.tail_first >= 0) {
    const int e = xcd_chunk((int)blockIdx.x, gp.full_tiles) - gp.tail_first, E = gp.tail_G - gp.tail_first;
    const int left = (gp.total_tiles - gp.full_tiles) * gp.split_k - e;
    end = gp.full_tiles + (e < 0 || left <= 0 ? 0 : (left + E - 1) / E) * gp.tail_G;
  }
  end = __builtin_amdgcn_readfirstlane(end);

  int* const sq = gp.sched;
  const bool dyn = MT == 256 && !MX && !CONV && sq != nullptr;
  const int xq = (int)blockIdx.x & (NXCD - 1);
  char* const s_next = smem + 16;
  uint32_t claim_v = 0;
  auto claim_issue = [&](int q) {
    if (wave == 0) {
      uint64_t sv;
      asm volatile("s_nop 4\n\ts_mov_b64 %1, exec\n\ts_mov_b64 exec, 1\n\tglobal_atomic_add %0, %2, %3, %4 sc0\n\ts_mov_b64 exec, %1"
                   : "=&v"(claim_v), "=&s"(sv)
                   : "v"((uint32_t)(q * 4)), "v"(1u), "s"(sq)
                   : "memory");
    }
  };
  auto claim_take = [&](int q) -> int {
    asm volatile("s_waitcnt vmcnt(0)" : "+v"(claim_v)::"memory");
    if (tid == 0) {
      int got = (int)claim_v * NXCD + q;
      if (got >= end) {
        got = end;
        int hd[NXCD];
#pragma unroll
        for (int t = 1; t < NXCD; t++) hd[t] = __hip_atomic_load(sq + ((q + t) & (NXCD - 1)), __ATOMIC_RELAXED, __HIP_MEMORY_SCOPE_AGENT);
#pragma unroll
        for (int t = 1; t < NXCD; t++) {
          const int qq = (q + t) & (NXCD - 1);
          if (got == end && hd[t] * NXCD + qq < end) {
            const int p = atomicAdd(sq + qq, 1) * NXCD + qq;
            if (p < end) got = p;
          }
        }
      }
      *LDS_PTR(int, s_next) = got;
    }
    LGKM0(); BAR8();
    const int r = *LDS_PTR(const volatile int, s_next);
    LGKM0(); BAR8();
    return __builtin_amdgcn_readfirstlane(r);
  };
  if (dyn) claim_issue(xq);

  constexpr int NAO = A_KM ? 2 * FI : 2, NBO = B_KM ? 4 : 2;
  uint32_t aoff[NAO], boff[NBO];
#pragma unroll
  for (int ks = 0; ks < 2; ks++) {
    if (A_KM) {
#pragma unroll
      for (int i = 0; i < FI; i++) { const int kr = ks * 32 + 8 * (lane >> 4) + ((lane & 15) >> 2), c = wr * QR + i * 16 + 4 * (lane & 3); aoff[i * 2 + ks] = kr * 256 + (((c >> 3) ^ SWZ_K(kr)) << 4) + (c & 7) * 2; }
    } else {
      const int r = wr * QR + (lane & 15), kp = ks * 4 + (lane >> 4);
      aoff[ks] = r * 128 + ((kp ^ SWZ_R(r)) << 4);
    }
    if (B_KM) {
#pragma unroll
      for (int j = 0; j < 2; j++) { const int kr = ks * 32 + 8 * (lane >> 4) + ((lane & 15) >> 2), c = wc * 32 + j * 16 + 4 * (lane & 3); boff[j * 2 + ks] = kr * 256 + (((c >> 3) ^ SWZ_K(kr)) << 4) + (c & 7) * 2; }
    } else {
      const int r = wc * 32 + (lane & 15), kp = ks * 4 + (lane >> 4);
      boff[ks] = r * 128 + ((kp ^ SWZ_R(r)) << 4);
    }
  }
  auto frag = [&](bool km, const char* p) -> bf16x8 {
    if (!km) return *LDS_PTR(const bf16x8, p);
    const s16x4 lo = lds_tr16(p), hi = lds_tr16(p + 4 * 256);
    return __builtin_bit_cast(bf16x8, (s16x8){lo[0], lo[1], lo[2], lo[3], hi[0], hi[1], hi[2], hi[3]});
  };

  AccT<MT> acc;
  bf16x8 fa[2 * FI], fb0[4], fb1s[4];
  bf16x8 (&fb1)[4] = MT == 256 ? fb1s : fb0;
#define FB1 fb1
#ifdef MMDIT_G8_SPLITWAIT
  auto readA1 = [&](int buf, int x, int ks) {
#pragma unroll
    for (int i = 0; i < FI; i++) fa[i * 2 + ks] = frag(A_KM, smem + buf * KBUF + x + (A_KM ? aoff[A_KM ? i * 2 + ks : 0] : aoff[ks] + i * 2048));
  };
  auto readB1 = [&](bf16x8 (&fb)[4], int buf, int x, int ks) {
#pragma unroll
    for (int j = 0; j < 2; j++) fb[j * 2 + ks] = frag(B_KM, smem + buf * KBUF + x + (B_KM ? boff[B_KM ? j * 2 + ks : 0] : boff[ks] + j * 2048));
  };
#endif
  auto readA = [&](int buf, int x) {
#pragma unroll
    for (int i = 0; i < FI; i++)
#pragma unroll
      for (int ks = 0; ks < 2; ks++) fa[i * 2 + ks] = frag(A_KM, smem + buf * KBUF + x + (A_KM ? aoff[A_KM ? i * 2 + ks : 0] : aoff[ks] + i * 2048));
  };
  auto readB = [&](bf16x8 (&fb)[4], int buf, int x) {
#pragma unroll
    for (int j = 0; j < 2; j++)
#pragma unroll
      for (int ks = 0; ks < 2; ks++) fb[j * 2 + ks] = frag(B_KM, smem + buf * KBUF + x + (B_KM ? boff[B_KM ? j * 2 + ks : 0] : boff[ks] + j * 2048));
  };
  auto mma = [&](f32x4 (&c)[2 * FI], const bf16x8 (&fb)[4]) {
#pragma unroll
    for (int ks = 0; ks < 2; ks++)
#pragma unroll
      for (int i = 0; i < FI; i++)
#pragma unroll
        for (int j = 0; j < 2; j++) c[i * 2 + j] = __builtin_amdgcn_mfma_f32_16x16x32_bf16(fb[j * 2 + ks], fa[i * 2 + ks], c[i * 2 + j], 0, 0, 0);
  };

  auto mma0 = [&](f32x4 (&c)[2 * FI], const bf16x8 (&fb)[4]) {
    const f32x4 z = {0.f, 0.f, 0.f, 0.f};
#pragma unroll
    for (int i = 0; i < FI; i++)
#pragma unroll
      for (int j = 0; j < 2; j++) c[i * 2 + j] = __builtin_amdgcn_mfma_f32_16x16x32_bf16(fb[j * 2], fa[i * 2], z, 0, 0, 0);
#pragma unroll
    for (int i = 0; i < FI; i++)
#pragma unroll
      for (int j = 0; j < 2; j++) c[i * 2 + j] = __builtin_amdgcn_mfma_f32_16x16x32_bf16(fb[j * 2 + 1], fa[i * 2 + 1], c[i * 2 + j], 0, 0, 0);
  };

  uint32_t rowA = 0, chkA = 0, rowB = 0, chkB = 0;
  uint32_t ld2A = 0, ld2B = 0;
  int limA = 0, limB = 0;
  uint64_t curA = 0, curB = 0, stepA = 0, stepB = 0;
  int nkt = 0, krem = 0;
#ifdef MMDIT_G8_STREAM
  constexpr bool STREAM = MT == 256 && EPI != EPI_F32 && !CONV && !KT;
#else
  constexpr bool STREAM = false;
#endif
  uint32_t rowA_n = 0, rowB_n = 0;
  uint64_t curA_n = 0, curB_n = 0;
  uint64_t scurA_n = 0, scurB_n = 0;
  int nkt_n = 0;
  bool strm = false;
  int swig_h = 0;
  constexpr int NSC = !MX ? 1 : EPI == EPI_SWIGLU ? 6 : 4;
  i32x8 xa[MX ? FI : 1], xb0[MX ? 2 : 1], xb1[MX ? 2 : 1];
  uint32_t sc[2][NSC];
  uint32_t soffA = 0, soffB = 0;
  uint64_t scurA = 0, scurB = 0, sstepA = 0, sstepB = 0, supB = 0;
  auto xreadA = [&](int buf, int x) {
#pragma unroll
    for (int i = 0; i < (MX ? FI : 1); i++) {
      xa[i].lo = *LDS_PTR(const i32x4_t, smem + buf * KBUF + x + aoff[0] + i * 2048);
      xa[i].hi = *LDS_PTR(const i32x4_t, smem + buf * KBUF + x + aoff[1] + i * 2048);
    }
  };
  auto xreadB = [&](i32x8 (&xb)[MX ? 2 : 1], int buf, int x) {
#pragma unroll
    for (int j = 0; j < (MX ? 2 : 1); j++) {
      xb[j].lo = *LDS_PTR(const i32x4_t, smem + buf * KBUF + x + boff[0] + j * 2048);
      xb[j].hi = *LDS_PTR(const i32x4_t, smem + buf * KBUF + x + boff[1] + j * 2048);
    }
  };
  auto sload = [&](int set, int d, bool gen = true) {
    if constexpr (MX && !PT) {
      const bool nx = gen && STREAM && strm && d > krem;
      const int dd = !gen ? d : nx ? min(d - krem - 1, nkt_n - 1) : min(d, krem);
      const uint64_t pa = (nx ? scurA_n : scurA) + (uint64_t)(uint32_t)dd * sstepA, pb = (nx ? scurB_n : scurB) + (uint64_t)(uint32_t)dd * sstepB;
      const uint64_t ua = ((uint64_t)(uint32_t)__builtin_amdgcn_readfirstlane((uint32_t)(pa >> 32)) << 32) | (uint32_t)__builtin_amdgcn_readfirstlane((uint32_t)pa);
      const uint64_t ub = ((uint64_t)(uint32_t)__builtin_amdgcn_readfirstlane((uint32_t)(pb >> 32)) << 32) | (uint32_t)__builtin_amdgcn_readfirstlane((uint32_t)pb);
      asm volatile("s_nop 4\n\tglobal_load_dword %0, %2, %3\n\tglobal_load_dword %1, %2, %3 offset:128" : "=v"(sc[set][0]), "=v"(sc[set][1]) : "v"(soffA), "s"(ua) : "memory");
      asm volatile("s_nop 4\n\tglobal_load_dword %0, %2, %3\n\tglobal_load_dword %1, %2, %3 offset:128" : "=v"(sc[set][2]), "=v"(sc[set][3]) : "v"(soffB), "s"(ub) : "memory");
      if constexpr (EPI == EPI_SWIGLU) {
        const uint64_t pu = pb + supB;
        const uint64_t uu = ((uint64_t)(uint32_t)__builtin_amdgcn_readfirstlane((uint32_t)(pu >> 32)) << 32) | (uint32_t)__builtin_amdgcn_readfirstlane((uint32_t)pu);
        asm volatile("s_nop 4\n\tglobal_load_dword %0, %2, %3\n\tglobal_load_dword %1, %2, %3 offset:128" : "=v"(sc[set][4]), "=v"(sc[set][5]) : "v"(soffB), "s"(uu) : "memory");
      }
    }
  };
  auto spin = [&](int set) {
    if constexpr (MX && !PT) {
#pragma unroll
      for (int k = 0; k < NSC; k++) asm volatile("" : "+v"(sc[set][k]));
    }
  };
  auto mmax = [&](f32x4 (&c)[2 * FI], const i32x8 (&xb)[MX ? 2 : 1], int set, int qm, int qn) {
    if constexpr (MX) {
      uint32_t sb[2];
#pragma unroll
      for (int j = 0; j < 2; j++) sb[j] = PT ? 0x7f7f7f7fu : EPI == EPI_SWIGLU ? sc[set][2 + 2 * qn + j] >> (8 * wc) : sc[set][2 + j] >> (16 * (wc & 1));
#pragma unroll
      for (int i = 0; i < FI; i++)
#pragma unroll
        for (int j = 0; j < 2; j++)
          c[i * 2 + j] = mx16_mfma(xb[j], xa[i], c[i * 2 + j], EPI == EPI_SWIGLU ? 0 : qn, (int)sb[j], qm * 2 + (i >> 1), PT ? 0x7f7f7f7f : (int)sc[set][i & 1]);
    }
  };

  uint32_t cvA[2][CONV ? PAW : 1];
  int cseg_left = 0, cseg_len = 0;
  uint64_t cjump = 0;
  auto item_rows = [&](const Item& it, uint32_t& ra, uint32_t& rb) {
    const int m0 = it.tm * MT, n0 = it.tn * 256;
    if (A_KM) { const int kr = wave * 4 + (lane >> 4), lr0 = ((lane & 15) ^ SWZ_K(kr)) * 8; ra = m0 + (lr0 >> 6) * 128 + (lr0 & 63); }
    else ra = m0 + wave * 8 + (lane >> 3);
    if (B_KM) { const int kr = wave * 4 + (lane >> 4), lr0 = ((lane & 15) ^ SWZ_K(kr)) * 8; rb = n0 + (lr0 >> 5) * 64 + (lr0 & 31); }
    else { const int lr = wave * 8 + (lane >> 3); rb = EPI == EPI_SWIGLU ? it.tn * 128 + lr : n0 + (lr >> 5) * 64 + (lr & 31); }
  };
  auto item_setup = [&](const Item& it) {
    const Problem& q = gp.p[it.pi];
    const int m0 = it.tm * MT, n0 = it.tn * 256;
    ld2A = (uint32_t)q.lda * (MX ? 1 : 2); ld2B = (uint32_t)q.ldb * (MX ? 1 : 2);
    item_rows(it, rowA, rowB);
    if (A_KM) {
      const int kr = wave * 4 + (lane >> 4);
      chkA = kr * ld2A; limA = q.M - 8;
    } else {
      const int lr = wave * 8 + (lane >> 3);
      chkA = ((lane & 7) ^ SWZ_R(lr)) * 16; limA = q.M - 1;
    }
    if (B_KM) {
      const int kr = wave * 4 + (lane >> 4);
      chkB = kr * ld2B; limB = q.N - 8;
    } else {
      const int lr = wave * 8 + (lane >> 3);
      chkB = ((lane & 7) ^ SWZ_R(lr)) * 16;
      if (EPI == EPI_SWIGLU) swig_h = q.N >> 1;
      limB = q.N - 1;
    }
    const int kt0 = it.h0 >> 1;
    nkt = (it.h1 - it.h0) >> 1;
    krem = nkt - 1;
    stepA = A_KM ? (uint64_t)64 * q.lda * 2 : 128;
    stepB = B_KM ? (uint64_t)64 * q.ldb * 2 : 128;
    curA = (uint64_t)(uintptr_t)q.A + kt0 * stepA;
    curB = (uint64_t)(uintptr_t)q.B + kt0 * stepB;
    if constexpr (CONV) {
      const int hw = q.cHo * q.cWo, sdn = q.conv_mode == 2 ? 2 : 1, o = q.conv_mode == 2 ? 1 : 0;
#pragma unroll
      for (int h = 0; h < 2; h++)
#pragma unroll
        for (int i = 0; i < PAW; i++) {
          const int lr = 64 * i + wave * 8 + (lane >> 3);
          const int m = min(m0 + (lr >> 6) * 128 + h * 64 + (lr & 63), q.M - 1);
          const int bimg = m / hw, rem = m - bimg * hw, yo = rem / q.cWo, xo = rem - yo * q.cWo;
          cvA[h][i] = (uint32_t)((((int64_t)bimg * q.cHp + sdn * yo) * q.cWp + sdn * xo) * q.cC * 2);
        }
      cseg_len = 3 * (q.cC / 64);
      const int kh = kt0 / cseg_len, within = kt0 - kh * cseg_len;
      cjump = (uint64_t)((int64_t)q.cWp - 3) * q.cC * 2;
      curA = (uint64_t)(uintptr_t)q.A + (uint64_t)((((int64_t)(kh + o) * q.cWp + o) * q.cC) * 2) + (uint64_t)within * 128;
      cseg_left = cseg_len - within;
    }
    if constexpr (MX && !PT) {
      const int64_t padA = ((int64_t)q.M + 127) & ~(int64_t)127, padB = ((int64_t)q.N + 127) & ~(int64_t)127;
      sstepA = (uint64_t)padA * 4; sstepB = (uint64_t)padB * 4;
      const uint32_t lane_part = (uint32_t)((lane & 15) * 8 + ((lane >> 4) & 1) * 4);
      soffA = (uint32_t)(wr * 256) + lane_part + (uint32_t)(lane >> 5) * (uint32_t)(padA * 2);
      scurA = (uint64_t)(uintptr_t)q.scale_a + (uint64_t)kt0 * sstepA + (uint64_t)m0 * 2;
      if constexpr (EPI == EPI_SWIGLU) {
        soffB = lane_part + (uint32_t)(lane >> 5) * (uint32_t)(padB * 2);
        scurB = (uint64_t)(uintptr_t)q.scale_b + (uint64_t)kt0 * sstepB + (uint64_t)(it.tn * 128) * 2;
        supB = (uint64_t)(q.N >> 1) * 2;
      } else {
        soffB = (uint32_t)((wc >> 1) * 256) + lane_part + (uint32_t)(lane >> 5) * (uint32_t)(padB * 2);
        scurB = (uint64_t)(uintptr_t)q.scale_b + (uint64_t)kt0 * sstepB + (uint64_t)n0 * 2;
      }
    }
  };
  auto stageA = [&](int h, int d, int buf, bool gen = true) {
    const bool nx = gen && STREAM && strm && d > krem;
    const int dd = !gen ? d : nx ? min(d - krem - 1, nkt_n - 1) : min(d, krem);
    const char* src = (const char*)(uintptr_t)((nx ? curA_n : curA) + (uint64_t)(uint32_t)dd * stepA + (CONV && dd >= cseg_left ? cjump : 0));
    const uint32_t rA = nx ? rowA_n : rowA;
    const uint32_t dst = ldsw + buf * KBUF + (h ? XA1 : XA0);
#pragma unroll
    for (int i = 0; i < PAW; i++) {
      if (!(i < PAW - 1 || GE::PA % 8 == 0 || hiw)) continue;
      uint32_t voff;
      if (A_KM) voff = (uint32_t)min((int)rA + h * 64, limA) * 2 + chkA + (uint32_t)(i * 32) * ld2A;
      else {
        const int lr0 = 64 * i;
        int drow;
        if (MT == 256) drow = i * 128 + h * 64;
        else drow = 0;
        if (CONV) voff = cvA[h][CONV ? i : 0] + chkA;
        else if (MT == 256) voff = (uint32_t)min((int)rA + drow, limA) * ld2A + chkA;
        else {
          const int lr = lr0 + (int)rA;
          const int lrl = lr0 + wave * 8;
          voff = (uint32_t)min(lr + (lrl >= 80 ? 80 : 0) + h * 80, limA) * ld2A + chkA;
        }
      }
      glds16(voff, src, dst + i * 8192);
    }
  };
  auto stageB = [&](int h, int d, int buf, bool gen = true) {
    const bool nx = gen && STREAM && strm && d > krem;
    const int dd = !gen ? d : nx ? min(d - krem - 1, nkt_n - 1) : min(d, krem);
    const char* src = (const char*)(uintptr_t)((nx ? curB_n : curB) + (uint64_t)(uint32_t)dd * stepB);
    const uint32_t rB = nx ? rowB_n : rowB;
    const uint32_t dst = ldsw + buf * KBUF + (h ? XB1 : XB0);
#pragma unroll
    for (int i = 0; i < 2; i++) {
      uint32_t voff;
      if (B_KM) voff = (uint32_t)min((int)rB + h * 32, limB) * 2 + chkB + (uint32_t)(i * 32) * ld2B;
      else if (EPI == EPI_SWIGLU) voff = (uint32_t)((int)rB + i * 64 + h * swig_h) * ld2B + chkB;
      else voff = (uint32_t)min((int)rB + i * 128 + h * 32, limB) * ld2B + chkB;
      glds16(voff, src, dst + i * 8192);
    }
  };
  auto next_ktile = [&]() {
    curA += stepA; curB += stepB; krem--;
    if constexpr (MX && !PT) { scurA += sstepA; scurB += sstepB; }
    if constexpr (CONV) { if (--cseg_left == 0) { curA += cjump; cseg_left = cseg_len; } }
  };
  constexpr bool REREAD = MT != 256;
  auto wait3 = [&]() {
    constexpr int NA = REREAD ? 2 : 1, NB = REREAD ? 1 : 2;
    if (GE::PA % 8 == 0 || hiw) VMCNT8(NA * PAW + NB * 2);
    else VMCNT8(NA * (PAW - 1) + NB * 2);
  };

#ifdef MMDIT_G8_SPLITWAIT
#define P1_READS(cur) readB1(fb0, cur, XB0, 0); readA1(cur, XA0, 0); __builtin_amdgcn_sched_barrier(0); readB1(fb0, cur, XB0, 1); readA1(cur, XA0, 1);
#define P1_WAIT() asm volatile("s_waitcnt lgkmcnt(%0)" ::"n"(((A_KM ? 2 : 1) * FI + (B_KM ? 4 : 2)) > 15 ? 15 : ((A_KM ? 2 : 1) * FI + (B_KM ? 4 : 2))) : "memory")
#define P3_READS(cur) readA1(cur, XA1, 0); __builtin_amdgcn_sched_barrier(0); readA1(cur, XA1, 1);
#define P3_WAIT() asm volatile("s_waitcnt lgkmcnt(%0)" ::"n"((A_KM ? 2 : 1) * FI) : "memory")
#else
#define P1_READS(cur) readB(fb0, cur, XB0); __builtin_amdgcn_sched_barrier(0); readA(cur, XA0);
#define P1_WAIT() LGKM0()
#define P3_READS(cur) readA(cur, XA1);
#define P3_WAIT() LGKM0()
#endif
#ifdef MMDIT_PROBES
#define WAIT3X() do { if (DRAIN && relax > 0) { relax--; VMCNT8(1 * PAW + 2 * 2 + 4 * FI); } else wait3(); } while (0)
#else
#define WAIT3X() wait3()
#endif
#define KTILE8(cur, gen)                                                                                          \
  {                                                                                                          \
                                                                                                     \
    P1_READS(cur)                                                                                            \
    if (REREAD) stageB(0, 1, (cur) ^ 1, gen); else stageA(1, 1, (cur) ^ 1, gen);                           \
    P1_WAIT(); BAR8(); __builtin_amdgcn_sched_barrier(0);                                                    \
    mma(acc.a[0][0], fb0);                                                                                   \
    __builtin_amdgcn_sched_barrier(0); BAR8();                                                               \
                                                                                                     \
    readB(FB1, cur, XB1);                                                                                    \
    stageA(0, 2, cur, gen);                                                                                 \
    LGKM0(); BAR8(); __builtin_amdgcn_sched_barrier(0);                                                      \
    mma(acc.a[0][1], FB1);                                                                                   \
    __builtin_amdgcn_sched_barrier(0); BAR8();                                                               \
                                                                                                     \
    P3_READS(cur)                                                                                            \
    if (REREAD) stageB(1, 2, cur, gen); else stageB(0, 2, cur, gen);                                       \
    P3_WAIT(); BAR8(); __builtin_amdgcn_sched_barrier(0);                                                    \
    mma(acc.a[1][1], FB1);                                                                                   \
    __builtin_amdgcn_sched_barrier(0); BAR8();                                                               \
                                                                                                     \
    if (REREAD) { readB(fb0, cur, XB0); stageA(1, 2, cur, gen); } else stageB(1, 2, cur, gen);             \
    WAIT3X();                                                                                                \
    LGKM0(); BAR8(); __builtin_amdgcn_sched_barrier(0);                                                      \
    mma(acc.a[1][0], fb0);                                                                                   \
    __builtin_amdgcn_sched_barrier(0); BAR8();                                                               \
    next_ktile();                                                                                            \
  }

#define KTILE8X(cur, gen)                                                                                         \
  {                                                                                                          \
    xreadB(xb0, cur, XB0); __builtin_amdgcn_sched_barrier(0); xreadA(cur, XA0);                              \
    sload((cur) ^ 1, 1, gen);                                                                                     \
    stageA(1, 1, (cur) ^ 1, gen);                                                                                 \
    LGKM0(); BAR8(); __builtin_amdgcn_sched_barrier(0);                                                      \
    mmax(acc.a[0][0], xb0, cur, 0, 0);                                                                       \
    __builtin_amdgcn_sched_barrier(0); BAR8();                                                               \
    xreadB(xb1, cur, XB1);                                                                                   \
    stageA(0, 2, cur, gen);                                                                                       \
    LGKM0(); BAR8(); __builtin_amdgcn_sched_barrier(0);                                                      \
    mmax(acc.a[0][1], xb1, cur, 0, 1);                                                                       \
    __builtin_amdgcn_sched_barrier(0); BAR8();                                                               \
    xreadA(cur, XA1);                                                                                        \
    stageB(0, 2, cur, gen);                                                                                       \
    LGKM0(); BAR8(); __builtin_amdgcn_sched_barrier(0);                                                      \
    mmax(acc.a[1][1], xb1, cur, 1, 1);                                                                       \
    __builtin_amdgcn_sched_barrier(0); BAR8();                                                               \
    stageB(1, 2, cur, gen);                                                                                       \
    wait3();                                                                                                 \
    spin((cur) ^ 1);                                                                                         \
    LGKM0(); BAR8(); __builtin_amdgcn_sched_barrier(0);                                                      \
    mmax(acc.a[1][0], xb0, cur, 1, 0);                                                                       \
    __builtin_amdgcn_sched_barrier(0); BAR8();                                                               \
    next_ktile();                                                                                            \
  }

#define KTILE8D(cur)                                                                                         \
  {                                                                                                          \
    P1_READS(cur)                                                                                            \
    if (dr) drain_q(acc.a[0][0], 0, 0);                                                                      \
    stageA(1, 1, (cur) ^ 1);                                                                                 \
    P1_WAIT(); BAR8(); __builtin_amdgcn_sched_barrier(0);                                                    \
    mma0(acc.a[0][0], fb0);                                                                                  \
    __builtin_amdgcn_sched_barrier(0); BAR8();                                                               \
    readB(FB1, cur, XB1);                                                                                    \
    if (dr) drain_q(acc.a[0][1], 0, 1);                                                                      \
    stageA(0, 2, cur);                                                                                       \
    LGKM0(); BAR8(); __builtin_amdgcn_sched_barrier(0);                                                      \
    mma0(acc.a[0][1], FB1);                                                                                  \
    __builtin_amdgcn_sched_barrier(0); BAR8();                                                               \
    P3_READS(cur)                                                                                            \
    if (dr) drain_q(acc.a[1][1], 1, 1);                                                                      \
    stageB(0, 2, cur);                                                                                       \
    P3_WAIT(); BAR8(); __builtin_amdgcn_sched_barrier(0);                                                    \
    mma0(acc.a[1][1], FB1);                                                                                  \
    __builtin_amdgcn_sched_barrier(0); BAR8();                                                               \
    if (dr) drain_q(acc.a[1][0], 1, 0);                                                                      \
    stageB(1, 2, cur);                                                                                       \
    if (dr) VMCNT8(1 * PAW + 2 * 2 + 3 * FI); else wait3();                                                  \
    LGKM0(); BAR8(); __builtin_amdgcn_sched_barrier(0);                                                      \
    mma0(acc.a[1][0], fb0);                                                                                  \
    __builtin_amdgcn_sched_barrier(0); BAR8();                                                               \
    next_ktile();                                                                                            \
  }

  char* stage = smem + GE::STAGE0 + wave * EP32_WAVE_BYTES;
  int* s_ticket = (int*)smem;

  constexpr bool DEFER = MT == 256 && EPI != EPI_F32;
#ifdef MMDIT_PROBES
  constexpr bool DRAIN = DEFER && EPI == EPI_BF16 && !MX;
#else
  constexpr bool DRAIN = false;
#endif
  char* dr_ptr = nullptr;
  uint32_t dr_ld = 0;
  bool prev_drain = false;
  auto drain_q = [&](f32x4 (&c)[2 * FI], int qm, int qn) {
    char* pq = dr_ptr + (int64_t)(qm * QR) * dr_ld + qn * 64;
#pragma unroll
    for (int i = 0; i < FI; i++) {
      const f32x4 a = c[i * 2], b = c[i * 2 + 1];
      const uint32_t a0 = pack_bf2(a[0], a[1]), a1 = pack_bf2(a[2], a[3]), b0 = pack_bf2(b[0], b[1]), b1 = pack_bf2(b[2], b[3]);
      const auto x = __builtin_amdgcn_permlane16_swap(a0, b0, false, false), y = __builtin_amdgcn_permlane16_swap(a1, b1, false, false);
#ifdef MMDIT_PROBES
      if (gp.debug & 512) { asm volatile("" ::"v"(x[0]), "v"(y[0]), "v"(x[1]), "v"(y[1])); continue; }
#endif
#ifdef MMDIT_PROBES
      if (gp.debug & 1024) { __builtin_nontemporal_store((u32x4){x[0], y[0], x[1], y[1]}, (u32x4*)(pq + (int64_t)(i * 16) * dr_ld)); continue; }
#endif
      *(u32x4*)(pq + (int64_t)(i * 16) * dr_ld) = (u32x4){x[0], y[0], x[1], y[1]};
    }
  };
  auto run_epilogue = [&](const Item& it) __attribute__((always_inline)) {
  const Problem& q = gp.p[it.pi];
  const int m0 = it.tm * MT, n0 = it.tn * 256;
#ifdef MMDIT_PROBES
  if (gp.debug & 8) { if (acc.a[0][0][0][0] == 12345.f) ((float*)q.C)[0] = 1.f; return; }
#endif
  float alpha = 1.f;
  if constexpr (PT) alpha = q.scale_a[0] * q.scale_b[0];
  if constexpr (EPI == EPI_BF16) epi8_bf16<MT, MX, MX || (MT == 320 && B_KM)>(acc, q, gp, m0, n0, wr, wc, lane, stage, alpha);
  else if constexpr (EPI == EPI_SWIGLU) epi8_swiglu<MT, MX>(acc, q, m0, it.tn, wr, wc, lane, stage, alpha);
  else if constexpr (EPI == EPI_QK) epi8_qk<MT>(acc, q, gp, gp.qk[it.pi & 1], m0, n0, wr, wc, lane, stage);
  else if constexpr (EPI == EPI_SWIGLU_BWD) epi8_swiglu_bwd<MT>(acc, q, m0, n0, wr, wc, lane, stage);
  else if constexpr (EPI == EPI_F32R) epi8_f32r<MT>(acc, q, m0, n0, wr, wc, lane, stage);
  else {
    if (it.atomic && gp.ws_slots) {
      constexpr int TE = 256 * 256, NW = 8;
      const int tt = it.tile - gp.full_tiles, S = gp.split_k;
      float* slots = gp.ws_slots + (int64_t)tt * S * TE;
      epi8_f32_slot<MT>(acc, slots + (int64_t)it.sk * TE, wr, wc, lane, stage);
      asm volatile("s_waitcnt vmcnt(0)" ::: "memory");
      __syncthreads();
      if (tid == 0) *s_ticket = atomicAdd(gp.ws_count + tt, 1);
      __syncthreads();
      if (*s_ticket == S - 1) {
        float* C = (float*)q.C;
        constexpr int NCH = TE / 4 / (64 * NW);
#pragma unroll 1
        for (int b0 = 0; b0 < NCH; b0 += 4) {
          f32x4 tsum[4];
#pragma unroll
          for (int u = 0; u < 4; u++) tsum[u] = (f32x4){0.f, 0.f, 0.f, 0.f};
#pragma unroll 1
          for (int s0 = 0; s0 < S; s0 += 4) {
            f32x4 v[4][4];
#pragma unroll
            for (int u = 0; u < 4; u++) {
              const int idx = tid + (b0 + u) * (64 * NW), r = idx / 64, c = (idx % 64) * 4;
#pragma unroll
              for (int k = 0; k < 4; k++) {
                const float* src = slots + (int64_t)min(s0 + k, S - 1) * TE + (int64_t)r * 256 + c;
                asm volatile("global_load_dwordx4 %0, %1, off sc1" : "=v"(v[u][k]) : "v"(src) : "memory");
              }
            }
#pragma unroll
            for (int u = 0; u < 4; u++)
              asm volatile("s_waitcnt vmcnt(0)" : "+v"(v[u][0]), "+v"(v[u][1]), "+v"(v[u][2]), "+v"(v[u][3])::"memory");
#pragma unroll
            for (int u = 0; u < 4; u++)
#pragma unroll
              for (int k = 0; k < 4; k++)
                if (s0 + k < S) tsum[u] += v[u][k];
          }
#pragma unroll
          for (int u = 0; u < 4; u++) {
            const int idx = tid + (b0 + u) * (64 * NW), r = idx / 64, c = (idx % 64) * 4;
            if (m0 + r < q.M && n0 + c < q.N) {
              float* cp = C + (int64_t)(m0 + r) * q.ldc + n0 + c;
              if (gp.accumulate) tsum[u] += *(const f32x4*)cp;
              __builtin_nontemporal_store(tsum[u], (f32x4*)cp);
            }
          }
        }
        if (tid == 0) gp.ws_count[tt] = 0;
      }
      __syncthreads();
    } else {
      epi8_f32<MT>(acc, q, m0, n0, wr, wc, lane, stage, it.atomic, gp.accumulate != 0);
    }
  }
  };

#ifdef MMDIT_PROBES
  if (gp.debug >> 16) {
    const long long span = (long long)(gp.debug >> 16) * 256, until = __builtin_readcyclecounter() + span * (((int)blockIdx.x / 8) % 32) / 32;
    while ((long long)__builtin_readcyclecounter() < until) __builtin_amdgcn_s_sleep(8);
  }
#endif
  if (dyn) pos = claim_take(xq);
  bool left = false;
  Item item = item_at(gp, pos, end), prev = item;
  bool pending = false;
  bool streamed = false;
  while (item.valid) {
    if (STREAM && streamed) {
      rowA = rowA_n; rowB = rowB_n; curA = curA_n; curB = curB_n; nkt = nkt_n; krem = nkt - 1;
      if constexpr (MX && !PT) { scurA = scurA_n; scurB = scurB_n; }
    } else {
      item_setup(item);
    }
    if constexpr (STREAM) {
      const Item nxt = item_at(gp, item.pos + G, end);
      strm = !dyn && nxt.valid && nxt.pi == item.pi && nkt >= 2 && (nkt & 1) == 0 && nxt.h1 > nxt.h0;
#ifdef MMDIT_PROBES
      if (gp.debug & 4096) strm = false;
#endif
      if (strm) {
        const Problem& q = gp.p[nxt.pi];
        item_rows(nxt, rowA_n, rowB_n);
        curA_n = (uint64_t)(uintptr_t)q.A + (uint64_t)(nxt.h0 >> 1) * stepA;
        curB_n = (uint64_t)(uintptr_t)q.B + (uint64_t)(nxt.h0 >> 1) * stepB;
        nkt_n = (nxt.h1 - nxt.h0) >> 1;
        if constexpr (MX && !PT) {
          scurA_n = (uint64_t)(uintptr_t)q.scale_a + (uint64_t)(nxt.h0 >> 1) * sstepA + (uint64_t)(nxt.tm * MT) * 2;
          scurB_n = (uint64_t)(uintptr_t)q.scale_b + (uint64_t)(nxt.h0 >> 1) * sstepB + (uint64_t)(EPI == EPI_SWIGLU ? nxt.tn * 128 : nxt.tn * 256) * 2;
        }
      }
    }
    constexpr bool LATE = !DRAIN && !STREAM;
    const int qcl = item.pos & (NXCD - 1), tcl = dyn ? (LATE && nkt >= 2 ? (nkt - 2) & ~1 : -1) : -2;
    if (tcl == -1) claim_issue(qcl);
    if (nkt > 0 && !(STREAM && streamed)) {
      if constexpr (MX) sload(0, 0);
      if (REREAD) { stageA(0, 0, 0); stageB(1, 0, 0); stageA(1, 0, 0); stageB(0, 0, 0); stageA(0, 1, 1); stageB(1, 1, 1); stageA(1, 1, 1); }
      else { stageA(0, 0, 0); stageB(0, 0, 0); stageB(1, 0, 0); stageA(1, 0, 0); stageA(0, 1, 1); stageB(0, 1, 1); stageB(1, 1, 1); }
    }
    const bool dr = DRAIN && pending && prev_drain && nkt > 0;
#ifdef MMDIT_PROBES
    int relax = (dr && (gp.debug & 256)) ? 2 : 0;
#endif
    if (DEFER && pending && !dr) run_epilogue(prev);
    if (!DRAIN || nkt == 0) {
#pragma unroll
      for (int a = 0; a < 2; a++)
#pragma unroll
        for (int b = 0; b < 2; b++)
#pragma unroll
          for (int i = 0; i < 2 * FI; i++) acc.a[a][b][i] = (f32x4){0.f, 0.f, 0.f, 0.f};
    }
    if (nkt > 0) {
      if (!(STREAM && streamed)) wait3();
      BAR8();
      if (wr == 1) BAR8();
      int t = 0;
      if constexpr (DRAIN) {
        KTILE8D(0)
#pragma unroll 1
        for (t = 1; t + 1 < nkt; t += 2) {
          KTILE8(1, true)
          KTILE8(0, true)
        }
        if (t < nkt) KTILE8(1, true)
      } else if constexpr (MX) {
        spin(0);
        if constexpr (STREAM) {
#pragma unroll 1
          for (; t + 3 < nkt; t += 2) {
            KTILE8X(0, false)
            KTILE8X(1, false)
          }
        }
#pragma unroll 1
        for (; t + 1 < nkt; t += 2) {
          if (t == tcl) claim_issue(qcl);
          KTILE8X(0, true)
          KTILE8X(1, true)
        }
        if (t < nkt) KTILE8X(0, true)
      } else {
        if constexpr (STREAM) {
#pragma unroll 1
          for (; t + 3 < nkt; t += 2) {
            KTILE8(0, false)
            KTILE8(1, false)
          }
        }
#pragma unroll 1
        for (; t + 1 < nkt; t += 2) {
          if (t == tcl) claim_issue(qcl);
          KTILE8(0, true)
          KTILE8(1, true)
        }
        if (t < nkt) KTILE8(0, true)
      }
      if (!(STREAM && strm)) VMCNT8(0);
      if (wr == 0) BAR8();
      BAR8();
    }
    if constexpr (KT) {
      const Problem& q = gp.p[item.pi];
      const int kfull = q.nk * 64, ktail = q.K - kfull;
      if (ktail > 0 && item.h1 == 2 * q.nk && item.h0 < item.h1) {
        const bf16_t* Ab = (const bf16_t*)q.A + (int64_t)kfull * q.lda;
        const bf16_t* Bb = (const bf16_t*)q.B + (int64_t)kfull * q.ldb;
        const int kr0 = wave * 4 + (lane >> 4);
#pragma unroll
        for (int h = 0; h < 2; h++)
#pragma unroll
          for (int i = 0; i < 2; i++) {
            const int kr = kr0 + 32 * i;
            u32x4 va = {0u, 0u, 0u, 0u}, vb = {0u, 0u, 0u, 0u};
            if (kr < ktail) {
              va = *(const u32x4*)(Ab + (int64_t)kr * q.lda + min((int)rowA + h * 64, limA));
              vb = *(const u32x4*)(Bb + (int64_t)kr * q.ldb + min((int)rowB + h * 32, limB));
            }
            *LDS_PTR(u32x4, smem + (h ? XA1 : XA0) + wave * 1024 + lane * 16 + i * 8192) = va;
            *LDS_PTR(u32x4, smem + (h ? XB1 : XB0) + wave * 1024 + lane * 16 + i * 8192) = vb;
          }
        __syncthreads();
        readB(fb0, 0, XB0); readB(fb1s, 0, XB1); readA(0, XA0);
        mma(acc.a[0][0], fb0); mma(acc.a[0][1], fb1s);
        readA(0, XA1);
        mma(acc.a[1][1], fb1s); mma(acc.a[1][0], fb0);
        __syncthreads();
      }
    }
    int npos = item.pos + G;
    if (dyn) {
      npos = claim_take(qcl);
      if (npos == end) { claim_issue(NXCD); left = true; }
    }
    if (DEFER) {
      prev = item; pending = true;
      if constexpr (DRAIN) {
        const Problem& q = gp.p[item.pi];
        const int m0 = item.tm * MT, n0 = item.tn * 256;
        prev_drain = m0 + MT <= q.M && n0 + 256 <= q.N && !q.bias && gp.act == MMDIT_ACT_NONE && (q.ldc & 7) == 0 && ((uintptr_t)q.C & 15) == 0;
#ifdef MMDIT_PROBES
        if (gp.debug & 128) prev_drain = false;
#endif
        dr_ld = (uint32_t)q.ldc * 2;
#ifdef MMDIT_PROBES
        const int m0w = (gp.debug & 2048) ? 0 : m0;
#else
        const int m0w = m0;
#endif
        dr_ptr = (char*)q.C + ((int64_t)(m0w + wr * (MT / 2) + (lane & 15)) * q.ldc + n0 + wc * 64 + ((lane >> 4) & 1) * 16 + (lane >> 5) * 8) * 2;
      }
    } else {
      run_epilogue(item);
      if (MT != 256) BAR8();
    }
    streamed = STREAM && strm;
    item = item_at(gp, npos, end);
  }
  if (DEFER && pending) run_epilogue(prev);
  if (dyn) {
    if (!left) claim_issue(NXCD);
    asm volatile("s_waitcnt vmcnt(0)" : "+v"(claim_v)::"memory");
    if (tid == 0 && (int)claim_v == G - 1) {
#pragma unroll
      for (int q = 0; q <= NXCD; q++) atomicExch(sq + q, 0);
    }
  }
}

template <int MT, bool A_KM, bool B_KM, int EPI, bool KT = false, bool MX = false, bool CONV = false, bool PT = false>
int launch8(const GroupParams& gp, hipStream_t s, int cu) {
  auto k = gemm8_kernel<MT, A_KM, B_KM, EPI, KT, MX, CONV, PT>;
  constexpr int smem = Geo<MT>::SMEM;
  static unsigned long long attr_done = 0;
  if (!mmdit_device_once(attr_done)) {
    hipError_t e = hipFuncSetAttribute((const void*)k, hipFuncAttributeMaxDynamicSharedMemorySize, smem);
    if (e != hipSuccess) return (int)e;
    mmdit_device_mark(attr_done);
  }
  const int work = total_work(gp);
  const int all = mmdit_device_cus(), grid = gp.sched ? (work < all ? work : all) : gp.persistent && work > cu ? cu : work;
  hipLaunchKernelGGL(k, dim3(grid), dim3(512), smem, s, gp);
  return mmdit_launch_status();
}

#ifndef MMDIT_G8_PART
#define MMDIT_G8_PART 1
#endif

#if MMDIT_G8_PART == 2
}
int gemm::launch_gemm8_fp8(bool b_km, const GroupParams& gp, hipStream_t s, int cu) {
  if (b_km || gp.act == MMDIT_ACT_SWIGLU_BWD || gp.act == MMDIT_ACT_SILU) return MMDIT_ERR_ARG;
  if (gp.qk_on) return gp.mx && gp.act == MMDIT_ACT_NONE ? launch8<256, false, false, EPI_QK, false, true>(gp, s, cu) : MMDIT_ERR_ARG;
  if (!gp.mx) return gp.act == MMDIT_ACT_SWIGLU ? launch8<256, false, false, EPI_SWIGLU, false, true, false, true>(gp, s, cu) : launch8<256, false, false, EPI_BF16, false, true, false, true>(gp, s, cu);
  return gp.act == MMDIT_ACT_SWIGLU ? launch8<256, false, false, EPI_SWIGLU, false, true>(gp, s, cu) : launch8<256, false, false, EPI_BF16, false, true>(gp, s, cu);
}

int gemm::launch_gemm8_conv(bool f32_out, const GroupParams& gp, hipStream_t s, int cu) {
  return f32_out ? launch8<256, false, false, EPI_F32R, false, false, true>(gp, s, cu) : launch8<256, false, false, EPI_BF16, false, false, true>(gp, s, cu);
}

#else

template <int MT>
int launch8_bf16(bool b_km, const GroupParams& gp, hipStream_t s, int cu) {
  if (gp.qk_on) {
    if constexpr (MT == 256) return b_km ? MMDIT_ERR_ARG : launch8<MT, false, false, EPI_QK>(gp, s, cu);
    else return MMDIT_ERR_SHAPE;
  }
  if (gp.act == MMDIT_ACT_SWIGLU) return b_km ? MMDIT_ERR_ARG : launch8<MT, false, false, EPI_SWIGLU>(gp, s, cu);
  if (gp.act == MMDIT_ACT_SWIGLU_BWD) {
    if constexpr (MT == 256) return b_km ? launch8<MT, false, true, EPI_SWIGLU_BWD>(gp, s, cu) : MMDIT_ERR_ARG;
    else return MMDIT_ERR_SHAPE;
  }
  return b_km ? launch8<MT, false, true, EPI_BF16>(gp, s, cu) : launch8<MT, false, false, EPI_BF16>(gp, s, cu);
}

}

int gemm::launch_gemm8(int cfg, bool a_km, bool b_km, const GroupParams& gp, hipStream_t s, int cu, bool ktail, bool fp8) {
  if (fp8) return cfg == CFG_256x256 && !a_km && !ktail ? launch_gemm8_fp8(b_km, gp, s, cu) : MMDIT_ERR_ARG;
  if (a_km) {
    if (!b_km || cfg != CFG_256x256) return MMDIT_ERR_ARG;
    return ktail ? launch8<256, true, true, EPI_F32, true>(gp, s, cu) : launch8<256, true, true, EPI_F32>(gp, s, cu);
  }
  if (ktail) return MMDIT_ERR_ARG;
  if (cfg == CFG_320x256) return launch8_bf16<320>(b_km, gp, s, cu);
  if (cfg == CFG_256x256) return launch8_bf16<256>(b_km, gp, s, cu);
  return MMDIT_ERR_ARG;
}
#endif
```

stable-diffusion-3-from-scratch_amd/csrc/gemm_common.h:

```cpp
#pragma once
#include "common.h"

namespace gemm {

constexpr int BK = 64;
constexpr int MAXG = 12;
constexpr int NXCD = 8;

struct Problem {
  const void* A; const void* B; void* C; void* aux;
  const float* bias; const float* gate; const float* residual;
  int64_t lda, ldb, ldc, ld_gate, ld_res, ld_aux;
  int M, N, K;
  int rows_per_batch, tiles_n, tiles_m, tile_start;
  int nk, unit_start;
  int conv_mode, cHo, cWo, cHp, cWp, cC;
  const float* scale_a; const float* scale_b;
  unsigned char* c_scales;
  float* dbias;
};
struct QkEpi {
  const float* wq; const float* wk;
  const float* rcos; const float* rsin;
  int tokens, tok0;
};
struct GroupParams {
  Problem p[MAXG];
  int count, total_tiles, act, accumulate, split_k, raster, debug, epi_direct;
  int full_tiles;
  int tail_first, tail_rounds, tail_G;
  int stream_k, total_units, persistent;
  int mx;
  float* ws_slots;
  int* ws_count;
  int* sched;
  QkEpi qk[2];
  bf16_t* qkQ; bf16_t* qkK; bf16_t* qkV;
  int qk_on, qk_heads, qk_s_total;
};

__device__ __host__ __forceinline__ int total_work(const GroupParams& gp) {
  return gp.tail_first >= 0 ? gp.full_tiles + gp.tail_rounds * gp.tail_G : gp.full_tiles + (gp.total_tiles - gp.full_tiles) * gp.split_k;
}
__device__ __forceinline__ bool is_split_work(const GroupParams& gp, int work) { return work >= gp.full_tiles && gp.split_k > 1; }

__device__ __forceinline__ int xcd_chunk(int w, int W) {
  const int q = W / NXCD, r = W % NXCD, xcd = w % NXCD, j = w / NXCD;
  return (xcd < r ? xcd * (q + 1) : r * (q + 1) + (xcd - r) * q) + j;
}

__device__ __forceinline__ const Problem& locate_in_problem(const GroupParams& gp, int t, int& tm, int& tn);

__device__ __forceinline__ int work_tile(const GroupParams& gp, int work, int& sk) {
  int t;
  if (work < gp.full_tiles) {
    sk = 0;
    t = xcd_chunk(work, gp.full_tiles);
  } else {
    const int Tt = gp.total_tiles - gp.full_tiles, lin = xcd_chunk(work - gp.full_tiles, Tt * gp.split_k);
    sk = lin / Tt;
    t = gp.full_tiles + lin - sk * Tt;
  }
  return t;
}

__device__ __forceinline__ const Problem& locate_tile(const GroupParams& gp, int work, int& tm, int& tn, int& sk) {
  return locate_in_problem(gp, work_tile(gp, work, sk), tm, tn);
}

__device__ __forceinline__ const Problem& locate_in_problem(const GroupParams& gp, int t, int& tm, int& tn) {
  int pi = 0;
#pragma unroll 1
  for (int i = 1; i < gp.count; i++) pi = (t >= gp.p[i].tile_start) ? i : pi;
  const Problem& p = gp.p[pi];
  t -= p.tile_start;
  const int gw = gp.raster, per_group = gw * p.tiles_m, grp = t / per_group, rem = t - grp * per_group;
  const int w = min(gw, p.tiles_n - grp * gw);
  tm = rem / w;
  tn = grp * gw + rem - tm * w;
  return p;
}

constexpr int EP_PITCH = 272;
constexpr int EP_WAVE_BYTES = 32 * EP_PITCH;

template <typename TC, typename TAUX, int MI = 2, int NJ = 2>
__device__ __forceinline__ void epilogue(const f32x16 (&acc)[MI][NJ], const Problem& p, const GroupParams& gp, int m0, int n0, int wm, int wn,
                                         int lane, int sk, char* stage , bool atomic_out = false) {
  static_assert(NJ == 2, "wave sub-tile must be 64 columns wide");
  TC* C = (TC*)p.C;
  TAUX* AUX = (TAUX*)p.aux;
  const bool first = sk == 0;
  const float* bias = first ? p.bias : nullptr;
  const float* gate = p.gate;
  const float* res = first ? p.residual : nullptr;
  const int c4 = (lane & 15) * 4, col = n0 + wn * 64 + c4;
  float b4[4] = {0.f, 0.f, 0.f, 0.f};
  if (bias && col < p.N) ld4(bias + col, b4);
#pragma unroll
  for (int i = 0; i < MI; i++) {
#pragma unroll
    for (int j = 0; j < NJ; j++)
#pragma unroll
      for (int g = 0; g < 4; g++)
        *LDS_PTR(f32x4, stage + (lane & 31) * EP_PITCH + (j * 32 + 8 * g + 4 * (lane >> 5)) * 4) =
            (f32x4){acc[i][j][g * 4], acc[i][j][g * 4 + 1], acc[i][j][g * 4 + 2], acc[i][j][g * 4 + 3]};
    asm volatile("s_waitcnt lgkmcnt(0)" ::: "memory");
#pragma unroll
    for (int it = 0; it < 8; it++) {
      const int r = it * 4 + (lane >> 4);
      const f32x4 t = *LDS_PTR(const f32x4, stage + r * EP_PITCH + c4 * 4);
      const int row = m0 + wm * (MI * 32) + i * 32 + r;
      if (row >= p.M || col >= p.N) continue;
      float v[4] = {t[0] + b4[0], t[1] + b4[1], t[2] + b4[2], t[3] + b4[3]};
      if (AUX) st4(AUX + (int64_t)row * p.ld_aux + col, v);
      if (gp.act == MMDIT_ACT_SILU) {
#pragma unroll
        for (int e = 0; e < 4; e++) v[e] = silu_f(v[e]);
      }
      if (res) {
        float r4[4];
        ld4(res + (int64_t)row * p.ld_res + col, r4);
        if (gate) {
          float g4[4];
          ld4(gate + (int64_t)(row / p.rows_per_batch) * p.ld_gate + col, g4);
#pragma unroll
          for (int e = 0; e < 4; e++) v[e] = r4[e] + g4[e] * v[e];
        } else {
#pragma unroll
          for (int e = 0; e < 4; e++) v[e] += r4[e];
        }
      }
      TC* cp = C + (int64_t)row * p.ldc + col;
      if constexpr (sizeof(TC) == 4) {
        if (gp.split_k > 1 || atomic_out) {
#pragma unroll
          for (int e = 0; e < 4; e++) atomicAdd((float*)cp + e, v[e]);
          continue;
        }
      }
      if (gp.accumulate) {
        float c4v[4];
        ld4(cp, c4v);
#pragma unroll
        for (int e = 0; e < 4; e++) v[e] += c4v[e];
      }
      st4(cp, v);
    }
    asm volatile("s_waitcnt lgkmcnt(0)" ::: "memory");
  }
}

template <typename TC, typename TAUX, int MI = 2, int NJ = 2>
__device__ __forceinline__ void epilogue_direct(const f32x16 (&acc)[MI][NJ], const Problem& p, const GroupParams& gp, int m0, int n0, int wm, int wn, int lane, int sk) {
  TC* C = (TC*)p.C;
  TAUX* AUX = (TAUX*)p.aux;
  const bool first = sk == 0;
  const float* bias = first ? p.bias : nullptr;
  const float* gate = p.gate;
  const float* res = first ? p.residual : nullptr;
#pragma unroll
  for (int i = 0; i < MI; i++) {
    const int row = m0 + wm * (MI * 32) + i * 32 + (lane & 31);
    if (row >= p.M) continue;
    const float* grow = gate ? gate + (int64_t)(row / p.rows_per_batch) * p.ld_gate : nullptr;
#pragma unroll
    for (int j = 0; j < NJ; j++) {
#pragma unroll
      for (int g = 0; g < 4; g++) {
        const int col = n0 + wn * (NJ * 32) + j * 32 + 8 * g + 4 * (lane >> 5);
        if (col >= p.N) continue;
        float v[4] = {acc[i][j][g * 4], acc[i][j][g * 4 + 1], acc[i][j][g * 4 + 2], acc[i][j][g * 4 + 3]};
        if (bias) {
          float b4[4];
          ld4(bias + col, b4);
#pragma unroll
          for (int e = 0; e < 4; e++) v[e] += b4[e];
        }
        if (AUX) st4(AUX + (int64_t)row * p.ld_aux + col, v);
        if (gp.act == MMDIT_ACT_SILU) {
#pragma unroll
          for (int e = 0; e < 4; e++) v[e] = silu_f(v[e]);
        }
        if (res) {
          float r4[4];
          ld4(res + (int64_t)row * p.ld_res + col, r4);
          if (grow) {
            float g4[4];
            ld4(grow + col, g4);
#pragma unroll
            for (int e = 0; e < 4; e++) v[e] = r4[e] + g4[e] * v[e];
          } else {
#pragma unroll
            for (int e = 0; e < 4; e++) v[e] += r4[e];
          }
        }
        TC* cp = C + (int64_t)row * p.ldc + col;
        if constexpr (sizeof(TC) == 4) {
          if (gp.split_k > 1) {
#pragma unroll
            for (int e = 0; e < 4; e++) atomicAdd((float*)cp + e, v[e]);
            continue;
          }
        }
        if (gp.accumulate) {
          float c4[4];
          ld4(cp, c4);
#pragma unroll
          for (int e = 0; e < 4; e++) v[e] += c4[e];
        }
        st4(cp, v);
      }
    }
  }
}


enum DmaCfg { CFG_128x128 = 0, CFG_256x128 = 1, CFG_256x256 = 2, CFG_320x256 = 3 };
inline void dma_cfg_tile(int cfg, int& bm, int& bn) { bm = cfg == CFG_128x128 ? 128 : cfg == CFG_320x256 ? 320 : 256; bn = cfg >= CFG_256x256 ? 256 : 128; }
int launch_dma(int cfg, bool a_km, bool b_km, int c_dtype, int aux_dtype, bool fp8, const GroupParams& gp, hipStream_t s, int cu);
int launch_lean_cfg(int cfg, bool b_km, const GroupParams& gp, hipStream_t s, int cu);
int launch_gemm8_fp8(bool b_km, const GroupParams& gp, hipStream_t s, int cu);
int launch_gemm8_conv(bool f32_out, const GroupParams& gp, hipStream_t s, int cu);
int launch_gemm8(int cfg, bool a_km, bool b_km, const GroupParams& gp, hipStream_t s, int cu, bool ktail, bool fp8);

}
```

stable-diffusion-3-from-scratch_amd/csrc/gemm_tile.h:

```cpp
#pragma once
#include "gemm_common.h"
#include <type_traits>

namespace gemm {
namespace {

constexpr int BKH = 32;
#ifndef MMDIT_GEMM_RING
#define MMDIT_GEMM_RING 4
#endif
constexpr int RING = MMDIT_GEMM_RING;
constexpr int EP32_WAVE_BYTES = 4096;

template <bool KM, int R, int ESZ = 2>
__device__ __forceinline__ uint32_t piece_voff(int c, int lane, int64_t ld, int row0, int rows) {
  if (!KM) {
    const int r = 16 * c + (lane >> 2), slot = lane & 3, piece = slot ^ ((lane >> 4) & 3);
    return (uint32_t)((int64_t)min(row0 + r, rows - 1) * ld * ESZ + piece * 16);
  } else {
    constexpr int PPR = R / 8;
    const int k = c * (64 / PPR) + lane / PPR, slot = lane % PPR, piece = slot ^ ((k & 3) << 2);
    return (uint32_t)((int64_t)k * ld * 2 + (int64_t)min(row0 + piece * 8, rows - 8) * 2);
  }
}

__device__ __forceinline__ uint32_t conv_voff(int c, int lane, const Problem& q, int row0) {
  const int r = 16 * c + (lane >> 2), slot = lane & 3, piece = slot ^ ((lane >> 4) & 3);
  const int m = min(row0 + r, q.M - 1), hw = q.cHo * q.cWo;
  const int b = m / hw, rem = m - b * hw, yo = rem / q.cWo, xo = rem - yo * q.cWo;
  const int s = q.conv_mode == 2 ? 2 : 1;
  return (uint32_t)((((int64_t)b * q.cHp + s * yo) * q.cWp + s * xo) * q.cC * 2 + piece * 16);
}

__device__ __forceinline__ void glds16(uint32_t voff, const char* sbase_, uint32_t lds_dst_) {
  const uint64_t a = (uint64_t)(uintptr_t)sbase_;
  const char* sbase = (const char*)(uintptr_t)(((uint64_t)(uint32_t)__builtin_amdgcn_readfirstlane((uint32_t)(a >> 32)) << 32) | (uint64_t)(uint32_t)__builtin_amdgcn_readfirstlane((uint32_t)a));
  const uint32_t lds_dst = __builtin_amdgcn_readfirstlane(lds_dst_);
  asm volatile("s_nop 4\n\ts_mov_b32 m0, %2\n\ts_nop 0\n\tglobal_load_lds_dwordx4 %0, %1" ::"v"(voff), "s"(sbase), "s"(lds_dst) : "memory", "m0");
}

#ifdef MMDIT_WIDE_SWZ_OLD
#define MMDIT_WIDE_SWZ(r) ((r) & 7)
#else
#define MMDIT_WIDE_SWZ(r) (((r) >> 1) & 7)
#endif
template <int ESZ = 2>
__device__ __forceinline__ uint32_t wide_voff(int c, int lane, int64_t ld, int row0, int rows) {
  const int r = 8 * c + (lane >> 3), chunk = (lane & 7) ^ MMDIT_WIDE_SWZ(r);
  return (uint32_t)((int64_t)min(row0 + r, rows - 1) * ld * ESZ + chunk * 16);
}
__device__ __forceinline__ bf16x8 load_frag_w(const char* tile, int r0, int ks, int lane) {
  const int r = r0 + (lane & 31), kp = ks * 2 + (lane >> 5);
  return *LDS_PTR(const bf16x8, tile + r * 128 + ((kp ^ MMDIT_WIDE_SWZ(r)) << 4));
}

__device__ __forceinline__ void glds16p(const void* gptr, uint32_t lds_dst_) {
  const uint32_t lds_dst = __builtin_amdgcn_readfirstlane(lds_dst_);
  asm volatile("s_mov_b32 m0, %1\n\ts_nop 0\n\tglobal_load_lds_dwordx4 %0, off" ::"v"(gptr), "s"(lds_dst) : "memory", "m0");
}

template <bool KM, int R>
__device__ __forceinline__ bf16x8 load_frag_h(const char* tile, int r0, int ks, int lane) {
  if (!KM) {
    const int r = r0 + (lane & 31), kp = ks * 2 + (lane >> 5);
    return *LDS_PTR(const bf16x8, tile + r * 64 + ((kp ^ ((r >> 2) & 3)) << 4));
  } else {
    const int kr = ks * 16 + (lane >> 5) * 8 + ((lane & 15) >> 2);
    const int bcol = (r0 + 16 * ((lane >> 4) & 1) + (lane & 3) * 4) * 2;
    const char* p = tile + kr * (2 * R) + ((((bcol >> 4) ^ ((kr & 3) << 2)) << 4) | (bcol & 15));
    s16x4 lo = lds_tr16(p), hi = lds_tr16(p + 4 * (2 * R));
    s16x8 r = {lo[0], lo[1], lo[2], lo[3], hi[0], hi[1], hi[2], hi[3]};
    return __builtin_bit_cast(bf16x8, r);
  }
}

template <int OA, int OB>
__device__ __forceinline__ f32x16 mx_mfma_lit(i32x8 a, i32x8 b, f32x16 c, int sa, int sb) {
  return __builtin_amdgcn_mfma_scale_f32_32x32x64_f8f6f4(a, b, c, 0, 0, OA, sa, OB, sb);
}
__device__ __forceinline__ f32x16 mx_mfma(i32x8 a, i32x8 b, f32x16 c, int oa, int sa, int ob, int sb) {
  switch (oa * 4 + ob) {
#define MMDIT_MX_CASE(A, B) case A * 4 + B: return mx_mfma_lit<A, B>(a, b, c, sa, sb);
    MMDIT_MX_CASE(0, 0) MMDIT_MX_CASE(0, 1) MMDIT_MX_CASE(0, 2) MMDIT_MX_CASE(0, 3)
    MMDIT_MX_CASE(1, 0) MMDIT_MX_CASE(1, 1) MMDIT_MX_CASE(1, 2) MMDIT_MX_CASE(1, 3)
    MMDIT_MX_CASE(2, 0) MMDIT_MX_CASE(2, 1) MMDIT_MX_CASE(2, 2) MMDIT_MX_CASE(2, 3)
    MMDIT_MX_CASE(3, 0) MMDIT_MX_CASE(3, 1) MMDIT_MX_CASE(3, 2)
#undef MMDIT_MX_CASE
    default: return mx_mfma_lit<3, 3>(a, b, c, sa, sb);
  }
}

template <int OA, int OB>
__device__ __forceinline__ f32x4 mx16_mfma_lit(i32x8 a, i32x8 b, f32x4 c, int sa, int sb) {
  return __builtin_amdgcn_mfma_scale_f32_16x16x128_f8f6f4(a, b, c, 0, 0, OA, sa, OB, sb);
}
__device__ __forceinline__ f32x4 mx16_mfma(i32x8 a, i32x8 b, f32x4 c, int oa, int sa, int ob, int sb) {
  switch (oa * 4 + ob) {
#define MMDIT_MX_CASE(A, B) case A * 4 + B: return mx16_mfma_lit<A, B>(a, b, c, sa, sb);
    MMDIT_MX_CASE(0, 0) MMDIT_MX_CASE(0, 1) MMDIT_MX_CASE(0, 2) MMDIT_MX_CASE(0, 3)
    MMDIT_MX_CASE(1, 0) MMDIT_MX_CASE(1, 1) MMDIT_MX_CASE(1, 2) MMDIT_MX_CASE(1, 3)
    MMDIT_MX_CASE(2, 0) MMDIT_MX_CASE(2, 1) MMDIT_MX_CASE(2, 2) MMDIT_MX_CASE(2, 3)
    MMDIT_MX_CASE(3, 0) MMDIT_MX_CASE(3, 1) MMDIT_MX_CASE(3, 2)
#undef MMDIT_MX_CASE
    default: return mx16_mfma_lit<3, 3>(a, b, c, sa, sb);
  }
}

__device__ __forceinline__ i32x8 load_frag8(const char* tile, int r0, int lane) {
  const int r = r0 + (lane & 31), s = (r >> 2) & 3, c0 = lane >> 5;
  const u32x4 lo = *LDS_PTR(const u32x4, tile + r * 64 + ((c0 ^ s) << 4)), hi = *LDS_PTR(const u32x4, tile + r * 64 + (((c0 + 2) ^ s) << 4));
  return i32x8{(int)lo[0], (int)lo[1], (int)lo[2], (int)lo[3], (int)hi[0], (int)hi[1], (int)hi[2], (int)hi[3]};
}

template <typename TC, typename TAUX, int MI, int NJ>
__device__ __forceinline__ void epilogue32(f32x16 (&acc)[MI][NJ], const Problem& p, const GroupParams& gp, int m0, int n0, int wm, int wn,
                                           int lane, int sk, char* stage, bool atomic_out, float alpha = 1.f, bool nt_out = false) {
  TC* C = (TC*)p.C;
  TAUX* AUX = (TAUX*)p.aux;
  const bool first = sk == 0;
  const float* bias = first ? p.bias : nullptr;
  const float* gate = p.gate;
  const float* res = first ? p.residual : nullptr;
  const int wr = lane & 31, wc = lane >> 5;
  const int rr = lane >> 3, rc = lane & 7;
#pragma unroll
  for (int i = 0; i < MI; i++) {
#pragma unroll
    for (int j = 0; j < NJ; j++) {
      const int col = n0 + wn * (NJ * 32) + j * 32 + rc * 4;
      const int row0 = m0 + wm * (MI * 32) + i * 32 + rr;
      float r4[4][4];
      if (res) {
#pragma unroll
        for (int it = 0; it < 4; it++) {
          const int row = row0 + it * 8;
          if (row < p.M && col < p.N) {
            ld4(res + (int64_t)row * p.ld_res + col, r4[it]);
          }
        }
      }
#pragma unroll
      for (int g = 0; g < 4; g++)
        *LDS_PTR(f32x4, stage + wr * 128 + (((2 * g + wc) ^ (wr & 7)) << 4)) =
            (f32x4){acc[i][j][g * 4], acc[i][j][g * 4 + 1], acc[i][j][g * 4 + 2], acc[i][j][g * 4 + 3]};
      asm volatile("s_waitcnt lgkmcnt(0)" ::: "memory");
      float b4[4] = {0.f, 0.f, 0.f, 0.f};
      if (bias && col < p.N) ld4(bias + col, b4);
#pragma unroll
      for (int it = 0; it < 4; it++) {
        const int r = it * 8 + rr;
        const f32x4 t = *LDS_PTR(const f32x4, stage + r * 128 + ((rc ^ (r & 7)) << 4));
        const int row = row0 + it * 8;
        if (row >= p.M || col >= p.N) continue;
        float v[4] = {t[0] * alpha + b4[0], t[1] * alpha + b4[1], t[2] * alpha + b4[2], t[3] * alpha + b4[3]};
        if (AUX) st4(AUX + (int64_t)row * p.ld_aux + col, v);
        if (gp.act == MMDIT_ACT_SILU) {
#pragma unroll
          for (int e = 0; e < 4; e++) v[e] = silu_f(v[e]);
        }
        if (res) {
          if (gate) {
            float g4[4];
            ld4(gate + (int64_t)(row / p.rows_per_batch) * p.ld_gate + col, g4);
#pragma unroll
            for (int e = 0; e < 4; e++) v[e] = r4[it][e] + g4[e] * v[e];
          } else {
#pragma unroll
            for (int e = 0; e < 4; e++) v[e] += r4[it][e];
          }
        }
        TC* cp = C + (int64_t)row * p.ldc + col;
        if constexpr (sizeof(TC) == 4) {
          if (atomic_out) {
#pragma unroll
            for (int e = 0; e < 4; e++) atomicAdd((float*)cp + e, v[e]);
            continue;
          }
        }
        if (gp.accumulate) {
          float c4v[4];
          ld4(cp, c4v);
#pragma unroll
          for (int e = 0; e < 4; e++) v[e] += c4v[e];
        }
        if constexpr (sizeof(TC) == 4) {
          if (nt_out) {
            __builtin_nontemporal_store(f32x4{v[0], v[1], v[2], v[3]}, (f32x4*)cp);
            continue;
          }
        }
        st4(cp, v);
      }
      asm volatile("s_waitcnt lgkmcnt(0)" ::: "memory");
    }
  }
}

template <int MI, int NJ>
__device__ __forceinline__ void epilogue_bf16(f32x16 (&acc)[MI][NJ], const Problem& p, const GroupParams& gp, int m0, int n0, int wm, int wn,
                                              int lane, char* stage, float alpha = 1.f) {
  static_assert(NJ == 2, "wave sub-tile must be 64 columns wide");
  bf16_t* C = (bf16_t*)p.C;
  const float* bias = p.bias;
  const int wr = lane & 31, wc = lane >> 5;
  const int rr = lane >> 3, rc = lane & 7;
  const int colw = n0 + wn * 64;
  float bv[NJ * 4][4];
  if (bias) {
#pragma unroll
    for (int q = 0; q < NJ * 4; q++) {
      const int c = colw + (q >> 2) * 32 + 8 * (q & 3) + 4 * wc;
      ld4(bias + (c < p.N ? c : 0), bv[q]);
      if (c >= p.N) bv[q][0] = bv[q][1] = bv[q][2] = bv[q][3] = 0.f;
    }
  }
#pragma unroll
  for (int i = 0; i < MI; i++) {
#pragma unroll
    for (int j = 0; j < NJ; j++)
#pragma unroll
      for (int g = 0; g < 4; g++) {
        float v[4] = {acc[i][j][g * 4] * alpha, acc[i][j][g * 4 + 1] * alpha, acc[i][j][g * 4 + 2] * alpha, acc[i][j][g * 4 + 3] * alpha};
        if (bias) {
#pragma unroll
          for (int e = 0; e < 4; e++) v[e] += bv[j * 4 + g][e];
        }
        if (gp.act == MMDIT_ACT_SILU) {
#pragma unroll
          for (int e = 0; e < 4; e++) v[e] = silu_f(v[e]);
        }
        const u32x2 pk = {pack_bf2(v[0], v[1]), pack_bf2(v[2], v[3])};
        *LDS_PTR(u32x2, stage + wr * 128 + (((j * 4 + g) ^ (wr & 7)) << 4) + wc * 8) = pk;
      }
    asm volatile("s_waitcnt lgkmcnt(0)" ::: "memory");
    const int col = colw + rc * 8;
#pragma unroll
    for (int it = 0; it < 4; it++) {
      const int r = it * 8 + rr;
      const u32x4 t = *LDS_PTR(const u32x4, stage + r * 128 + ((rc ^ (r & 7)) << 4));
      const int row = m0 + wm * (MI * 32) + i * 32 + r;
      if (row < p.M && col < p.N) *(u32x4*)(C + (int64_t)row * p.ldc + col) = t;
    }
    asm volatile("s_waitcnt lgkmcnt(0)" ::: "memory");
  }
}

template <int MI, int NJ>
__device__ __forceinline__ void epilogue_bf16_qk(f32x16 (&acc)[MI][NJ], const Problem& p, const GroupParams& gp, const QkEpi& e, int m0, int n0, int wm, int wn,
                                                 int lane, char* stage) {
  static_assert(NJ == 2, "wave sub-tile must be 64 columns wide");
  bf16_t* C = (bf16_t*)p.C;
  const int wr = lane & 31, wc = lane >> 5;
  const int rr = lane >> 3, rc = lane & 7;
  const int colw = n0 + wn * 64;
  const int D = gp.qk_heads * 64, part = colw / D, head = (colw - part * D) >> 6;
  const bool live = colw < p.N;
  float w8[8], c8[8], s8[8];
#pragma unroll
  for (int q = 0; q < 8; q++) w8[q] = 0.f;
  if (live && part < 2) ld8((part == 0 ? e.wq : e.wk) + rc * 8, w8);
  bf16_t* obase = part == 0 ? gp.qkQ : part == 1 ? gp.qkK : gp.qkV;
#pragma unroll
  for (int i = 0; i < MI; i++) {
#pragma unroll
    for (int j = 0; j < NJ; j++)
#pragma unroll
      for (int g = 0; g < 4; g++) {
        const u32x2 pk = {pack_bf2(acc[i][j][g * 4], acc[i][j][g * 4 + 1]), pack_bf2(acc[i][j][g * 4 + 2], acc[i][j][g * 4 + 3])};
        *LDS_PTR(u32x2, stage + wr * 128 + (((j * 4 + g) ^ (wr & 7)) << 4) + wc * 8) = pk;
      }
    asm volatile("s_waitcnt lgkmcnt(0)" ::: "memory");
    const int col = colw + rc * 8;
    const int rowb = m0 + wm * (MI * 32) + i * 32;
    const int b0 = __builtin_amdgcn_readfirstlane(rowb / e.tokens), n0r = rowb - b0 * e.tokens;
#pragma unroll
    for (int it = 0; it < 4; it++) {
      const int r = it * 8 + rr;
      const u32x4 t = *LDS_PTR(const u32x4, stage + r * 128 + ((rc ^ (r & 7)) << 4));
      const int row = rowb + r;
      if (!live || row >= p.M) continue;
      int b = b0, n = n0r + r;
      if (e.tokens >= 32) { if (n >= e.tokens) { n -= e.tokens; b++; } }
      else { b = row / e.tokens; n = row - b * e.tokens; }
      bf16_t* dst = obase + (((int64_t)b * gp.qk_heads + head) * gp.qk_s_total + e.tok0 + n) * 64 + rc * 8;
      if (part == 2) {
        *(u32x4*)dst = t;
        continue;
      }
      *(u32x4*)(C + (int64_t)row * p.ldc + col) = t;
      float x[8];
#pragma unroll
      for (int q = 0; q < 4; q++) { x[2 * q] = __builtin_bit_cast(float, t[q] << 16); x[2 * q + 1] = __builtin_bit_cast(float, t[q] & 0xffff0000u); }
      if (e.rcos) {
        ld8(e.rcos + (int64_t)n * 64 + rc * 8, c8);
        ld8(e.rsin + (int64_t)n * 64 + rc * 8, s8);
      }
      float ss = 0.f;
#pragma unroll
      for (int q = 0; q < 8; q++) ss += x[q] * x[q];
      ss += __shfl_xor(ss, 1, 64); ss += __shfl_xor(ss, 2, 64); ss += __shfl_xor(ss, 4, 64);
      const float rinv = rsqrtf(ss * (1.f / 64.f) + 1.1920929e-07f);
#pragma unroll
      for (int q = 0; q < 8; q++) x[q] = x[q] * rinv * w8[q];
      if (e.rcos) {
#pragma unroll
        for (int q = 0; q < 4; q++) {
          const float a = x[2 * q], bb = x[2 * q + 1];
          x[2 * q] = a * c8[2 * q] - bb * s8[2 * q];
          x[2 * q + 1] = bb * c8[2 * q + 1] + a * s8[2 * q + 1];
        }
      }
      st8(dst, x);
    }
    asm volatile("s_waitcnt lgkmcnt(0)" ::: "memory");
  }
}

template <int ESZ>
__device__ __forceinline__ uint32_t swiglu_voff(int c, int lane, int64_t ld, int tn, int h) {
  const int r = 16 * c + (lane >> 2), slot = lane & 3, piece = slot ^ ((lane >> 4) & 3);
  const int row = ((r >> 5) & 1) * h + tn * 128 + (r >> 6) * 32 + (r & 31);
  return (uint32_t)((int64_t)row * ld * ESZ + piece * 16);
}

template <int MI, bool SCALED>
__device__ __forceinline__ void epilogue_swiglu(f32x16 (&acc)[MI][2], const Problem& p, int m0, int tn, int wm, int wn, int lane, char* stage, float alpha_) {
  const float alpha = SCALED ? alpha_ : 1.f;
  bf16_t* Hout = (bf16_t*)p.C;
  bf16_t* GU = (bf16_t*)p.aux;
  const float* bias = p.bias;
  const int h = p.N >> 1;
  const int wr = lane & 31, wc = lane >> 5;
  const int hc = tn * 128 + wn * 32;
  float bgv[4][4], buv[4][4];
  if (bias) {
#pragma unroll
    for (int g = 0; g < 4; g++) {
      const int c = hc + 8 * g + 4 * wc;
      ld4(bias + c, bgv[g]);
      ld4(bias + h + c, buv[g]);
    }
  }
#pragma unroll
  for (int i = 0; i < MI; i++) {
    u32x2 pa[4];
#pragma unroll
    for (int g = 0; g < 4; g++) {
      float vg[4] = {acc[i][0][g * 4] * alpha, acc[i][0][g * 4 + 1] * alpha, acc[i][0][g * 4 + 2] * alpha, acc[i][0][g * 4 + 3] * alpha};
      float vu[4] = {acc[i][1][g * 4] * alpha, acc[i][1][g * 4 + 1] * alpha, acc[i][1][g * 4 + 2] * alpha, acc[i][1][g * 4 + 3] * alpha};
      if (bias) {
#pragma unroll
        for (int e = 0; e < 4; e++) { vg[e] += bgv[g][e]; vu[e] += buv[g][e]; }
      }
      const u32x2 pg = {pack_bf2(vg[0], vg[1]), pack_bf2(vg[2], vg[3])}, pu = {pack_bf2(vu[0], vu[1]), pack_bf2(vu[2], vu[3])};
      if (GU) {
        *LDS_PTR(u32x2, stage + wr * 128 + ((g ^ (wr & 7)) << 4) + wc * 8) = pg;
        *LDS_PTR(u32x2, stage + wr * 128 + (((4 + g) ^ (wr & 7)) << 4) + wc * 8) = pu;
      }
      float a[4];
#pragma unroll
      for (int e = 0; e < 2; e++) {
        const float g0 = __builtin_bit_cast(float, pg[e] << 16), g1 = __builtin_bit_cast(float, pg[e] & 0xffff0000u);
        const float u0 = __builtin_bit_cast(float, pu[e] << 16), u1 = __builtin_bit_cast(float, pu[e] & 0xffff0000u);
        a[2 * e] = silu_f(g0) * u0;
        a[2 * e + 1] = silu_f(g1) * u1;
      }
      pa[g] = u32x2{pack_bf2(a[0], a[1]), pack_bf2(a[2], a[3])};
    }
    asm volatile("s_waitcnt lgkmcnt(0)" ::: "memory");
    if (GU) {
      const int rr = lane >> 3, rc = lane & 7;
      const int col = (rc & 4 ? h : 0) + hc + (rc & 3) * 8;
#pragma unroll
      for (int it = 0; it < 4; it++) {
        const int r = it * 8 + rr;
        const u32x4 t = *LDS_PTR(const u32x4, stage + r * 128 + ((rc ^ (r & 7)) << 4));
        const int row = m0 + wm * (MI * 32) + i * 32 + r;
        if (row < p.M) __builtin_nontemporal_store(t, (u32x4*)(GU + (int64_t)row * p.ld_aux + col));
      }
    }
    asm volatile("s_waitcnt lgkmcnt(0)" ::: "memory");
    if (p.c_scales) {
      float hv[16];
#pragma unroll
      for (int g = 0; g < 4; g++)
#pragma unroll
        for (int e = 0; e < 2; e++) { hv[4 * g + 2 * e] = __builtin_bit_cast(float, pa[g][e] << 16); hv[4 * g + 2 * e + 1] = __builtin_bit_cast(float, pa[g][e] & 0xffff0000u); }
      float amax = 0.f;
#pragma unroll
      for (int e = 0; e < 16; e++) amax = fmaxf(amax, fabsf(hv[e]));
      amax = fmaxf(amax, __shfl_xor(amax, 32, 64));
      float inv;
      const int ex = mx_exponent(amax, inv);
#pragma unroll
      for (int g = 0; g < 4; g++) *LDS_PTR(unsigned, stage + wr * 32 + g * 8 + wc * 4) = mx_pack4(hv + 4 * g, inv);
      asm volatile("s_waitcnt lgkmcnt(0)" ::: "memory");
      const int r = lane >> 1, row = m0 + wm * (MI * 32) + i * 32 + r;
      const u32x4 t = *LDS_PTR(const u32x4, stage + r * 32 + (lane & 1) * 16);
      if (row < p.M) *(u32x4*)((unsigned char*)p.C + (int64_t)row * p.ldc + hc + (lane & 1) * 16) = t;
      const int myrow = m0 + wm * (MI * 32) + i * 32 + wr;
      if (wc == 0 && myrow < p.M) p.c_scales[mx_scale_index(myrow, hc >> 5, p.M)] = (unsigned char)(ex + 127);
      asm volatile("s_waitcnt lgkmcnt(0)" ::: "memory");
      continue;
    }
#pragma unroll
    for (int g = 0; g < 4; g++) *LDS_PTR(u32x2, stage + wr * 64 + ((g ^ (wr & 3)) << 4) + wc * 8) = pa[g];
    asm volatile("s_waitcnt lgkmcnt(0)" ::: "memory");
    {
      const int rr = lane >> 2, rc = lane & 3;
#pragma unroll
      for (int it = 0; it < 2; it++) {
        const int r = it * 16 + rr;
        const u32x4 t = *LDS_PTR(const u32x4, stage + r * 64 + ((rc ^ (r & 3)) << 4));
        const int row = m0 + wm * (MI * 32) + i * 32 + r;
        if (row < p.M) *(u32x4*)(Hout + (int64_t)row * p.ldc + hc + rc * 8) = t;
      }
    }
    asm volatile("s_waitcnt lgkmcnt(0)" ::: "memory");
  }
}

struct Item {
  int pi;
  int tm, tn, h0, h1, sk;
  bool atomic;
  int tile;
  int pos;
  bool valid;
};

__device__ __forceinline__ Item item_at(const GroupParams& gp, int pos, int end) {
  Item it;
  it.pos = pos;
  it.valid = pos < end;
  it.pi = 0;
  it.tm = it.tn = it.h0 = it.h1 = it.sk = 0;
  it.atomic = false;
  it.tile = 0;
  if (!it.valid) return it;
  if (gp.stream_k) {
    int pi = 0;
#pragma unroll 1
    for (int i = 1; i < gp.count; i++) pi = (pos >= gp.p[i].unit_start) ? i : pi;
    const Problem& p = gp.p[pi];
    const int local = pos - p.unit_start, t = local / p.nk, k0 = local - t * p.nk, k1 = min(p.nk, k0 + (end - pos));
    it.pi = pi;
    it.tm = t / p.tiles_n;
    it.tn = t - it.tm * p.tiles_n;
    it.h0 = 2 * k0;
    it.h1 = 2 * k1;
    it.sk = k0 == 0 ? 0 : 1;
    it.atomic = true;
  } else {
    int sk, t;
    if (gp.tail_first >= 0 && pos >= gp.full_tiles) {
      const int rnd = (pos - gp.full_tiles) / gp.tail_G, l = xcd_chunk((int)blockIdx.x, gp.full_tiles);
      const int Tt = gp.total_tiles - gp.full_tiles, u = rnd * (gp.tail_G - gp.tail_first) + l - gp.tail_first;
      sk = u / Tt;
      t = gp.full_tiles + u - sk * Tt;
    } else {
      t = work_tile(gp, pos, sk);
    }
    const Problem& p = locate_in_problem(gp, t, it.tm, it.tn);
    const int S = is_split_work(gp, pos) ? gp.split_k : 1;
    const int nk_all = p.nk, per = (nk_all + S - 1) / S;
    const int kt0 = sk * per, kt1 = max(kt0, min(nk_all, kt0 + per));
    it.pi = (int)(&p - &gp.p[0]);
    it.h0 = 2 * kt0;
    it.h1 = 2 * kt1;
    it.sk = sk;
    it.atomic = S > 1;
    it.tile = t;
  }
  return it;
}

__device__ __forceinline__ int next_pos(const GroupParams& gp, const Item& it) {
  return gp.stream_k ? it.pos + (it.h1 - it.h0) / 2 : it.pos + (int)gridDim.x;
}

}
}
```

Before: 2319.

## Balance weight-grad GEMM tail by splitting long tiles into two K-halves

Adds a balanced tail schedule for the fp32 weight-gradient 8-phase GEMM. The planner searches a split count and a K cut point so some full tiles run only their first K portion, and the remainder plus the split-K tail pieces are spread over the remaining workgroups, reducing wave-quantization idle time at the end of the persistent grid. The two halves are reduced through workspace slots. It also exposes a host-side plan dump and a tunable partial-reduction cost. The cost is more complex scheduling math, extra workspace traffic, and an extra reduction pass for the cut tiles.

Measured after the change: 2319. About the same (-0.0%).

```diff
diff --git a/include/mmdit_hip_plan.h b/include/mmdit_hip_plan.h
--- /dev/null
+++ b/include/mmdit_hip_plan.h
@@ -0,0 +1,20 @@
+#ifndef MMDIT_HIP_PLAN_H
+#define MMDIT_HIP_PLAN_H
+
+#include "mmdit_hip.h"
+
+#ifdef __cplusplus
+extern "C" {
+#endif
+
+typedef struct { int problem, tile, k_first, k_count, owner, slot; } mmdit_gemm_work_item;
+
+int mmdit_gemm_plan_items(const mmdit_gemm_args* args, int count, mmdit_gemm_work_item* items, int capacity);
+
+int mmdit_gemm_set_partial_cost(double units);
+
+#ifdef __cplusplus
+}
+#endif
+
+#endif
diff --git a/stable-diffusion-3-from-scratch_amd/_lib.py b/stable-diffusion-3-from-scratch_amd/_lib.py
--- a/stable-diffusion-3-from-scratch_amd/_lib.py
+++ b/stable-diffusion-3-from-scratch_amd/_lib.py
@@ -146,6 +146,14 @@
     "mmdit_qk_norm_rope3_fwd": ([ctypes.POINTER(QkProblem), _i, _i, _i, _i, _i, _i, _vp, _vp, _vp, _vp], _i),
     "mmdit_qk_norm_rope3_bwd": ([ctypes.POINTER(QkProblem), _i, _vp, _vp, _vp, _i, _i, _i, _i, _i, _i, _i, _vp], _i),
 }
+class GemmWorkItem(ctypes.Structure):
+    _fields_ = [("problem", _i), ("tile", _i), ("k_first", _i), ("k_count", _i), ("owner", _i), ("slot", _i)]
+
+
+_PLAN_SIGNATURES = {
+    "mmdit_gemm_plan_items": ([ctypes.POINTER(GemmArgs), _i, ctypes.POINTER(GemmWorkItem), _i], _i),
+    "mmdit_gemm_set_partial_cost": ([_d], _i),
+}
 HEAD_DIMS = (64, 128)
 ADAMW_CHUNK = 65536
 ABI_VERSION = 10
@@ -193,7 +201,7 @@
         except ImportError:
             pass
         L = ctypes.CDLL(LIB_PATH)
-        for name, (argtypes, restype) in list(_SIGNATURES.items()) + list(_EXT_SIGNATURES.items()) + list(_HD128_SIGNATURES.items()) + list(_ROPE3_SIGNATURES.items()):
+        for name, (argtypes, restype) in list(_SIGNATURES.items()) + list(_EXT_SIGNATURES.items()) + list(_HD128_SIGNATURES.items()) + list(_ROPE3_SIGNATURES.items()) + list(_PLAN_SIGNATURES.items()):
             fn = getattr(L, name)
             fn.argtypes = argtypes
             fn.restype = restype
diff --git a/stable-diffusion-3-from-scratch_amd/build.py b/stable-diffusion-3-from-scratch_amd/build.py
--- a/stable-diffusion-3-from-scratch_amd/build.py
+++ b/stable-diffusion-3-from-scratch_amd/build.py
@@ -11,6 +11,7 @@
 HEADER_EXT = os.path.join(HERE, "..", "include", "mmdit_hip_ext.h")
 HEADER_HD128 = os.path.join(HERE, "..", "include", "mmdit_hip_hd128.h")
 HEADER_ROPE3 = os.path.join(HERE, "..", "include", "mmdit_hip_rope3.h")
+HEADER_PLAN = os.path.join(HERE, "..", "include", "mmdit_hip_plan.h")
 SOURCES = ["gemm.hip", "gemm_dma.hip", "gemm_lean.hip", "gemm8p.hip", "gemm8p_inf.hip", "rowops.hip", "attention.hip", "attention_e4m3.hip", "attention_hd128.hip", "rowops_rope3.hip", "vae.hip", "vae_attn.hip", "optim.hip"]
 HIPCC = os.environ.get("HIPCC", "/opt/rocm/bin/hipcc")
 FLAGS = ["--offload-arch=gfx950", "-O3", "-std=c++17", "-fPIC"] + os.environ.get("MMDIT_EXTRA_HIPCC_FLAGS", "").split()
@@ -34,7 +35,7 @@
 
 
 def source_hash(src):
-    headers = sorted(os.path.join(CSRC, f) for f in os.listdir(CSRC) if f.endswith(".h")) + [HEADER, HEADER_EXT, HEADER_HD128, HEADER_ROPE3]
+    headers = sorted(os.path.join(CSRC, f) for f in os.listdir(CSRC) if f.endswith(".h")) + [HEADER, HEADER_EXT, HEADER_HD128, HEADER_ROPE3, HEADER_PLAN]
     if src == "gemm8p_inf.hip":
         headers.append(os.path.join(CSRC, "gemm8p.hip"))
     return _sha([os.path.join(CSRC, src)] + headers, " ".join([HIPCC] + FLAGS + SOURCE_FLAGS.get(src, [])))
diff --git a/stable-diffusion-3-from-scratch_amd/csrc/gemm.hip b/stable-diffusion-3-from-scratch_amd/csrc/gemm.hip
--- a/stable-diffusion-3-from-scratch_amd/csrc/gemm.hip
+++ b/stable-diffusion-3-from-scratch_amd/csrc/gemm.hip
@@ -1,5 +1,7 @@
 #include "gemm_common.h"
+#include "../../include/mmdit_hip_plan.h"
 #include <stdlib.h>
+#include <math.h>
 
 using namespace gemm;
 
@@ -297,6 +299,14 @@
   return c256 < c128 ? CFG_256x256 : CFG_128x128;
 }
 
+static constexpr double WS_PARTIAL_UNITS = 20.2;
+static double g_partial_units[64] = {};
+extern "C" int mmdit_gemm_set_partial_cost(double units) {
+  MMDIT_CHECK_ARG(units < 0 || units <= 1e6);
+  g_partial_units[mmdit_current_device()] = units < 0 ? 0.0 : units + 1.0;
+  return 0;
+}
+
 static inline int split_k_of(const mmdit_gemm_args* a) { return a->split_k > 1 ? a->split_k : 1; }
 
 struct QkRequest {
@@ -313,13 +323,14 @@
   int cfg;
   bool a_km, b_km, fp8, mx8, ktail;
   int a_dt, b_dt, c_dt, aux_dt, precision;
+  int order[MAXG];
   int cu;
   int* sched_page;
   int code;
   unsigned zero_mask;
 };
 
-struct DeviceState { bool claiming; void* ws; long long ws_bytes; };
+struct DeviceState { bool claiming; void* ws; long long ws_bytes; double partial_units; };
 
 static int choose_kernel(const mmdit_gemm_args* args, int count, const QkRequest* qkr, const DeviceState& ds, bool dma, bool conv, GemmPlan* pl) {
   const PlannerSwitches& sw = planner_switches();
@@ -329,6 +340,7 @@
   const int split_k = split_k_of(a0);
   GroupParams& gp = pl->gp;
   gp.tail_first = -1; gp.tail_rounds = 0; gp.tail_G = 0;
+  gp.bal_kmain = 0; gp.bal_long = 0; gp.bal_na = 0;
   if (conv) MMDIT_CHECK_ARG(dma);
   const bool swiglu = a0->act == MMDIT_ACT_SWIGLU;
   if (swiglu) {
@@ -397,10 +409,17 @@
     units += p.tiles_n * p.tiles_m * p.nk;
     if (stream_k) MMDIT_CHECK_ARG(!a->aux && !a->gate && a->stream_k);
   }
+  for (int i = 0; i < MAXG; i++) pl->order[i] = i < count ? order[i] : -1;
   gp.stream_k = stream_k; gp.total_units = units;
   gp.mx = fp8 && a0->scale_mode == 1;
   int full_tiles = split_k > 1 ? 0 : tiles, tail_split = split_k;
   const bool tail_mode = stream_k && !sw.kdec_streamk;
+  bool wgrad8 = dma && !fp8 && !conv && !(stream_k && !tail_mode) && cfg == CFG_256x256 && a0->a_kmajor && a0->b_kmajor &&
+            a0->c_dtype == MMDIT_F32 && a0->act == MMDIT_ACT_NONE;
+  for (int i = 0; i < count && wgrad8; i++) {
+    const mmdit_gemm_args* a = &args[i];
+    wgrad8 = !a->bias && !a->gate && !a->residual && !a->aux && a->N % 4 == 0 && a->ldc % 4 == 0 && aligned16(a->C);
+  }
   if (tail_mode) {
     gp.stream_k = 0;
     const int G = pl->cu * (cfg == CFG_128x128 ? 2 : 1), r = tiles % G;
@@ -436,6 +455,34 @@
             tail_split = bS;
             if (!(ds.ws && ds.claiming)) { gp.tail_first = first_short; gp.tail_rounds = brounds; gp.tail_G = G; }
           }
+          if (wgrad8 && ds.ws && !sw.tail_s) {
+            const double cp = ds.partial_units;
+            const bool old_bal = bbest < best;
+            const int per0 = (nk_tail + tail_split - 1) / tail_split;
+            const double item0 = per0 + (tail_split > 1 ? cp : 0.0);
+            const double old_span = old_bal ? fmax((double)nk_max, nk_short + ((r * tail_split + E - 1) / E) * item0)
+                                            : nk_max + ((r * tail_split + G - 1) / G) * item0;
+            double nbest = old_span;
+            int nS = 0, nk_cut = 0, nna = 0, nrounds = 0;
+            const int L = first_short;
+            for (int S = 1; S <= 64 && S * 2 <= nk_min; S++) {
+              const int nls = r * S, na = nls < E - 1 ? nls : E - 1, EB = E - na;
+              if (na < 1 || EB < 1) continue;
+              const int ra = (nls + na - 1) / na, rb = (L + EB - 1) / EB, per = (nk_tail + S - 1) / S;
+              const double load_a = nk_short + ra * (per + (S > 1 ? cp : 0.0));
+              int k = (int)ceil((nk_short + rb * (nk_max + cp) - cp) / (1.0 + rb));
+              if (k < 1) k = 1;
+              if (nk_max - k < 4) continue;
+              const double load_b = nk_short + rb * (nk_max - k + cp), span = fmax(fmax(k + cp, load_a), load_b);
+              if (span < nbest) { nbest = span; nS = S; nk_cut = k; nna = na; nrounds = ra > rb ? ra : rb; }
+            }
+            if (nS && r + L <= 1024 && 8192 + ((long long)r * nS + 2LL * L) * 65536 * 4 <= ds.ws_bytes) {
+              tail_split = nS;
+              gp.bal_kmain = nk_cut; gp.bal_long = L; gp.bal_na = nna;
+              gp.tail_first = -1; gp.tail_rounds = 0; gp.tail_G = 0;
+              if (!(ds.ws && ds.claiming)) { gp.tail_first = first_short; gp.tail_rounds = nrounds; gp.tail_G = G; }
+            }
+          }
         }
       }
     }
@@ -446,12 +493,6 @@
   if (split_k > 1) {
     MMDIT_CHECK_ARG(dma && a0->c_dtype == MMDIT_F32 && a0->act == MMDIT_ACT_NONE && !a0->accumulate && split_k <= 64);
     for (int i = 0; i < count; i++) MMDIT_CHECK_ARG(!args[i].aux && !args[i].gate);
-  }
-  bool wgrad8 = dma && !fp8 && !conv && !gp.stream_k && cfg == CFG_256x256 && a0->a_kmajor && a0->b_kmajor &&
-            a0->c_dtype == MMDIT_F32 && a0->act == MMDIT_ACT_NONE;
-  for (int i = 0; i < count && wgrad8; i++) {
-    const mmdit_gemm_args* a = &args[i];
-    wgrad8 = !a->bias && !a->gate && !a->residual && !a->aux && a->N % 4 == 0 && a->ldc % 4 == 0 && aligned16(a->C);
   }
   gp.ws_slots = nullptr; gp.ws_count = nullptr; gp.sched = nullptr;
   gp.qk_on = 0; gp.qkQ = gp.qkK = gp.qkV = nullptr; gp.qk_heads = 0; gp.qk_s_total = 0;
@@ -471,9 +512,9 @@
     gp.qk_on = 1; gp.qk_heads = qkr->heads; gp.qk_s_total = qkr->s_total;
     gp.qkQ = (bf16_t*)qkr->Q; gp.qkK = (bf16_t*)qkr->K; gp.qkV = (bf16_t*)qkr->V;
   }
-  if (wgrad8 && gp.split_k > 1) {
+  if (wgrad8 && (gp.split_k > 1 || gp.bal_kmain > 0)) {
     const long long tail_tiles = tiles - full_tiles;
-    if (ds.ws && tail_tiles <= 1024 && 8192 + tail_tiles * gp.split_k * 65536LL * 4 <= ds.ws_bytes) {
+    if (ds.ws && tail_tiles + gp.bal_long <= 1024 && 8192 + (tail_tiles * gp.split_k + 2LL * gp.bal_long) * 65536LL * 4 <= ds.ws_bytes) {
       gp.ws_count = (int*)ds.ws;
       gp.ws_slots = (float*)((char*)ds.ws + 8192);
     }
@@ -501,7 +542,7 @@
   pl->kernel = conv8 ? KERNEL_8P_CONV : p8 ? KERNEL_8P : lean ? KERNEL_WIDE : dma ? KERNEL_DMA : KERNEL_REG;
   pl->cfg = cfg; pl->mx8 = mx8;
   pl->code = dma ? (cfg | (gp.stream_k ? 16 : 0) | (tail_mode ? 32 : 0) | (lean || wgrad8 ? 128 : 0) | (p8 || conv8 ? 256 : 0)) : 64;
-  const bool claimed = pl->kernel == KERNEL_8P && !mx8 && cfg == CFG_256x256 && gp.persistent && gp.tail_first < 0 && total_work(gp) > pl->cu;
+  const bool claimed = pl->kernel == KERNEL_8P && !mx8 && cfg == CFG_256x256 && gp.persistent && gp.tail_first < 0 && total_work_bal(gp) > pl->cu;
   pl->sched_page = claimed && ds.ws && ds.claiming ? (int*)((char*)ds.ws + 4096) : nullptr;
   return 0;
 }
@@ -510,7 +551,7 @@
   MMDIT_CHECK_ARG(args && count >= 1 && count <= MAXG);
   const mmdit_gemm_args* a0 = &args[0];
   const int dev = mmdit_current_device();
-  const DeviceState ds{g_claiming[dev] != 0, g_ws[dev], g_ws_bytes[dev]};
+  const DeviceState ds{g_claiming[dev] != 0, g_ws[dev], g_ws_bytes[dev], g_partial_units[dev] > 0 ? g_partial_units[dev] - 1.0 : WS_PARTIAL_UNITS};
   const int cus = mmdit_device_cus();
   MMDIT_CHECK_ARG(a0->cu_budget == 0 || (a0->cu_budget >= 64 && a0->cu_budget <= cus && a0->cu_budget % 8 == 0));
   pl->cu = a0->cu_budget ? a0->cu_budget : cus;
@@ -639,6 +680,86 @@
   return rc ? rc : pl.code;
 }
 
+extern "C" int mmdit_gemm_plan_items(const mmdit_gemm_args* args, int count, mmdit_gemm_work_item* items, int capacity) {
+  MMDIT_CHECK_ARG(capacity >= 0 && (items || capacity == 0));
+  GemmPlan pl;
+  const int rc = plan_gemm(args, count, nullptr, &pl);
+  if (rc) return rc;
+  const GroupParams& gp = pl.gp;
+  if (pl.kernel != KERNEL_8P || gp.stream_k) return MMDIT_ERR_SHAPE;
+  const int work = total_work_bal(gp), Tt = gp.total_tiles - gp.full_tiles;
+  const int all = mmdit_device_cus(), grid = pl.sched_page ? (work < all ? work : all) : gp.persistent && work > pl.cu ? pl.cu : work;
+  int n = 0;
+  int* claimer = nullptr;
+  if (pl.sched_page) {
+    claimer = (int*)malloc(sizeof(int) * (size_t)(work + 2 * grid));
+    if (!claimer) return MMDIT_ERR_ARG;
+    int* busy = claimer + work;
+    int* last_q = busy + grid;
+    int head[NXCD];
+    for (int q = 0; q < NXCD; q++) head[q] = 0;
+    auto units = [&](int pos) {
+      int sk, kind = 0, t;
+      if (gp.bal_kmain > 0) t = bal_work(gp, pos, 0, sk, kind);
+      else { t = work_tile(gp, pos, sk); kind = pos >= gp.full_tiles && gp.split_k > 1 ? 1 : 0; }
+      int pi = 0;
+      for (int i = 1; i < gp.count; i++) pi = t >= gp.p[i].tile_start ? i : pi;
+      const int nk = gp.p[pi].nk, per = (nk + gp.split_k - 1) / gp.split_k;
+      if (kind == 1) { const int k0 = sk * per, k1 = k0 + per < nk ? k0 + per : nk; return k1 > k0 ? k1 - k0 : 0; }
+      return kind == 2 ? gp.bal_kmain : kind == 3 ? nk - gp.bal_kmain : nk;
+    };
+    for (int b = 0; b < grid; b++) { busy[b] = 0; last_q[b] = b % NXCD; }
+    for (int done = 0; done < work; done++) {
+      int b = 0;
+      for (int i = 1; i < grid; i++) b = busy[i] < busy[b] ? i : b;
+      int pos = -1;
+      for (int k = 0; k < NXCD && pos < 0; k++) {
+        const int q = (last_q[b] + k) % NXCD;
+        if (head[q] * NXCD + q < work) { pos = head[q]++ * NXCD + q; last_q[b] = q; }
+      }
+      claimer[pos] = b;
+      busy[b] += units(pos) + 1;
+    }
+  }
+  for (int wg = 0; wg < grid; wg++) {
+    int end = work;
+    if (gp.tail_first >= 0) {
+      const int e = xcd_chunk(wg, gp.full_tiles) - gp.tail_first, E = gp.tail_G - gp.tail_first, left = Tt * gp.split_k - e;
+      end = gp.bal_kmain > 0 ? bal_static_end(gp, wg) : gp.full_tiles + (e < 0 || left <= 0 ? 0 : (left + E - 1) / E) * gp.tail_G;
+    }
+    for (int pos = claimer ? 0 : wg; pos < end; pos += claimer ? 1 : grid) {
+      if (claimer && claimer[pos] != wg) continue;
+      int t, sk, kind;
+      if (gp.bal_kmain > 0) {
+        t = bal_work(gp, pos, wg, sk, kind);
+      } else {
+        if (gp.tail_first >= 0 && pos >= gp.full_tiles) {
+          const int rnd = (pos - gp.full_tiles) / gp.tail_G, u = rnd * (gp.tail_G - gp.tail_first) + xcd_chunk(wg, gp.full_tiles) - gp.tail_first;
+          sk = u / Tt;
+          t = gp.full_tiles + u - sk * Tt;
+        } else {
+          t = work_tile(gp, pos, sk);
+        }
+        kind = pos >= gp.full_tiles && gp.split_k > 1 ? 1 : 0;
+      }
+      int pi = 0;
+      for (int i = 1; i < gp.count; i++) pi = t >= gp.p[i].tile_start ? i : pi;
+      const int nk = gp.p[pi].nk, per = (nk + gp.split_k - 1) / gp.split_k;
+      int k0 = 0, k1 = nk;
+      if (kind == 1) { k0 = sk * per; k1 = k0 + per < nk ? k0 + per : nk; if (k1 < k0) k1 = k0; }
+      else if (kind == 2) k1 = gp.bal_kmain;
+      else if (kind == 3) k0 = gp.bal_kmain;
+      int slot = -1;
+      if (gp.ws_slots && kind == 1) slot = (t - gp.full_tiles) * gp.split_k + sk;
+      if (gp.ws_slots && kind >= 2) slot = Tt * gp.split_k + 2 * t + sk;
+      if (n < capacity) items[n] = mmdit_gemm_work_item{pl.order[pi], t - gp.p[pi].tile_start, k0, k1 - k0, wg, slot};
+      n++;
+    }
+  }
+  free(claimer);
+  return n;
+}
+
 extern "C" int mmdit_gemm_zero_mask(const mmdit_gemm_args* args, int count, unsigned* mask) {
   MMDIT_CHECK_ARG(mask);
   GemmPlan pl;
diff --git a/stable-diffusion-3-from-scratch_amd/csrc/gemm8p.hip b/stable-diffusion-3-from-scratch_amd/csrc/gemm8p.hip
--- a/stable-diffusion-3-from-scratch_amd/csrc/gemm8p.hip
+++ b/stable-diffusion-3-from-scratch_amd/csrc/gemm8p.hip
@@ -601,11 +601,13 @@
   const int G = (int)gridDim.x;
   const bool hiw = wave + 8 * (PAW - 1) < GE::PA;
 
-  int pos = (int)blockIdx.x, end = total_work(gp);
+  constexpr bool BAL = EPI == EPI_F32;
+  int pos = (int)blockIdx.x, end = BAL ? total_work_bal(gp) : total_work(gp);
   if (gp.tail_first >= 0) {
     const int e = xcd_chunk((int)blockIdx.x, gp.full_tiles) - gp.tail_first, E = gp.tail_G - gp.tail_first;
     const int left = (gp.total_tiles - gp.full_tiles) * gp.split_k - e;
     end = gp.full_tiles + (e < 0 || left <= 0 ? 0 : (left + E - 1) / E) * gp.tail_G;
+    if constexpr (BAL) { if (MMDIT_GP_NOW(bal_kmain) > 0) end = bal_static_end(gp, (int)blockIdx.x); }
   }
   end = __builtin_amdgcn_readfirstlane(end);
 
@@ -1062,8 +1064,10 @@
   else {
     if (it.atomic && gp.ws_slots) {
       constexpr int TE = 256 * 256, NW = 8;
-      const int tt = it.tile - gp.full_tiles, S = gp.split_k;
-      float* slots = gp.ws_slots + (int64_t)tt * S * TE;
+      const bool cut = MMDIT_GP_NOW(bal_kmain) > 0 && it.tile < MMDIT_GP_NOW(bal_long);
+      const int Tt = gp.total_tiles - gp.full_tiles;
+      const int tt = cut ? Tt + it.tile : it.tile - gp.full_tiles, S = cut ? 2 : gp.split_k;
+      float* slots = gp.ws_slots + (int64_t)(cut ? Tt * gp.split_k + 2 * it.tile : tt * S) * TE;
       epi8_f32_slot<MT>(acc, slots + (int64_t)it.sk * TE, wr, wc, lane, stage);
       asm volatile("s_waitcnt vmcnt(0)" ::: "memory");
       __syncthreads();
@@ -1077,6 +1081,22 @@
           f32x4 tsum[4];
 #pragma unroll
           for (int u = 0; u < 4; u++) tsum[u] = (f32x4){0.f, 0.f, 0.f, 0.f};
+          if (S == 2) {
+            f32x4 v[4][2];
+#pragma unroll
+            for (int u = 0; u < 4; u++) {
+              const int idx = tid + (b0 + u) * (64 * NW), r = idx / 64, c = (idx % 64) * 4;
+#pragma unroll
+              for (int k = 0; k < 2; k++) {
+                const float* src = slots + (int64_t)k * TE + (int64_t)r * 256 + c;
+                asm volatile("global_load_dwordx4 %0, %1, off sc1" : "=v"(v[u][k]) : "v"(src) : "memory");
+              }
+            }
+#pragma unroll
+            for (int u = 0; u < 4; u++) asm volatile("s_waitcnt vmcnt(0)" : "+v"(v[u][0]), "+v"(v[u][1])::"memory");
+#pragma unroll
+            for (int u = 0; u < 4; u++) tsum[u] = (tsum[u] + v[u][0]) + v[u][1];
+          } else {
 #pragma unroll 1
           for (int s0 = 0; s0 < S; s0 += 4) {
             f32x4 v[4][4];
@@ -1097,6 +1117,7 @@
 #pragma unroll
               for (int k = 0; k < 4; k++)
                 if (s0 + k < S) tsum[u] += v[u][k];
+          }
           }
 #pragma unroll
           for (int u = 0; u < 4; u++) {
@@ -1125,7 +1146,7 @@
 #endif
   if (dyn) pos = claim_take(xq);
   bool left = false;
-  Item item = item_at(gp, pos, end), prev = item;
+  Item item = item_at<BAL>(gp, pos, end), prev = item;
   bool pending = false;
   bool streamed = false;
   while (item.valid) {
@@ -1136,7 +1157,7 @@
       item_setup(item);
     }
     if constexpr (STREAM) {
-      const Item nxt = item_at(gp, item.pos + G, end);
+      const Item nxt = item_at<BAL>(gp, item.pos + G, end);
       strm = !dyn && nxt.valid && nxt.pi == item.pi && nkt >= 2 && (nkt & 1) == 0 && nxt.h1 > nxt.h0;
 #ifdef MMDIT_PROBES
       if (gp.debug & 4096) strm = false;
@@ -1278,7 +1299,7 @@
       if (MT != 256) BAR8();
     }
     streamed = STREAM && strm;
-    item = item_at(gp, npos, end);
+    item = item_at<BAL>(gp, npos, end);
   }
   if (DEFER && pending) run_epilogue(prev);
   if (dyn) {
@@ -1301,7 +1322,7 @@
     if (e != hipSuccess) return (int)e;
     mmdit_device_mark(attr_done);
   }
-  const int work = total_work(gp);
+  const int work = total_work_bal(gp);
   const int all = mmdit_device_cus(), grid = gp.sched ? (work < all ? work : all) : gp.persistent && work > cu ? cu : work;
   hipLaunchKernelGGL(k, dim3(grid), dim3(512), smem, s, gp);
   return mmdit_launch_status();
diff --git a/stable-diffusion-3-from-scratch_amd/csrc/gemm_common.h b/stable-diffusion-3-from-scratch_amd/csrc/gemm_common.h
--- a/stable-diffusion-3-from-scratch_amd/csrc/gemm_common.h
+++ b/stable-diffusion-3-from-scratch_amd/csrc/gemm_common.h
@@ -29,6 +29,7 @@
   int count, total_tiles, act, accumulate, split_k, raster, debug, epi_direct;
   int full_tiles;
   int tail_first, tail_rounds, tail_G;
+  int bal_kmain, bal_long, bal_na;
   int stream_k, total_units, persistent;
   int mx;
   float* ws_slots;
@@ -39,19 +40,25 @@
   int qk_on, qk_heads, qk_s_total;
 };
 
+struct SchedView { int total_tiles, split_k, full_tiles, tail_first, tail_rounds, tail_G, bal_kmain, bal_long, bal_na; };
 __device__ __host__ __forceinline__ int total_work(const GroupParams& gp) {
   return gp.tail_first >= 0 ? gp.full_tiles + gp.tail_rounds * gp.tail_G : gp.full_tiles + (gp.total_tiles - gp.full_tiles) * gp.split_k;
 }
-__device__ __forceinline__ bool is_split_work(const GroupParams& gp, int work) { return work >= gp.full_tiles && gp.split_k > 1; }
-
-__device__ __forceinline__ int xcd_chunk(int w, int W) {
+__device__ __host__ __forceinline__ int total_work_bal(const GroupParams& gp) {
+  return total_work(gp) + (gp.bal_kmain > 0 && gp.tail_first < 0 ? gp.bal_long : 0);
+}
+template <typename GPV>
+__device__ __forceinline__ bool is_split_work(const GPV& gp, int work) { return work >= gp.full_tiles && gp.split_k > 1; }
+
+__device__ __host__ __forceinline__ int xcd_chunk(int w, int W) {
   const int q = W / NXCD, r = W % NXCD, xcd = w % NXCD, j = w / NXCD;
   return (xcd < r ? xcd * (q + 1) : r * (q + 1) + (xcd - r) * q) + j;
 }
 
 __device__ __forceinline__ const Problem& locate_in_problem(const GroupParams& gp, int t, int& tm, int& tn);
 
-__device__ __forceinline__ int work_tile(const GroupParams& gp, int work, int& sk) {
+template <typename GPV>
+__device__ __host__ __forceinline__ int work_tile(const GPV& gp, int work, int& sk) {
   int t;
   if (work < gp.full_tiles) {
     sk = 0;
@@ -62,6 +69,51 @@
     t = gp.full_tiles + lin - sk * Tt;
   }
   return t;
+}
+
+template <typename GPV>
+__device__ __host__ __forceinline__ int bal_work(const GPV& gp, int pos, int wg, int& sk, int& kind) {
+  const int bal_long = gp.bal_long, bal_na = gp.bal_na;
+  const int G = gp.full_tiles, Tt = gp.total_tiles - G, nls = Tt * gp.split_k;
+  if (pos < G) {
+    const int t = xcd_chunk(pos, G);
+    sk = 0;
+    kind = t < bal_long ? 2 : 0;
+    return t;
+  }
+  int u, nq = 1;
+  const bool fixed = gp.tail_first >= 0;
+  if (fixed) {
+    const int rnd = (pos - G) / gp.tail_G, e = xcd_chunk(wg, G) - gp.tail_first, EB = gp.tail_G - gp.tail_first - bal_na;
+    u = e < bal_na ? rnd * bal_na + e : nls + rnd * EB + (e - bal_na);
+  } else {
+    const int W = nls + bal_long, up = pos - G, q = up % NXCD, j = up / NXCD;
+    const int x0 = bal_long / (G / NXCD), base = W / NXCD, rem = W % NXCD;
+    nq = NXCD - x0;
+    u = q >= x0 ? j * nq + (q - x0) : nq * base + (rem > x0 ? rem - x0 : 0) + j * x0 + q;
+  }
+  if (u < nls) {
+    int lin = u;
+    if (!fixed) {
+      const int Q = nls / nq, R = nls % nq, qq = u % nq, jj = u / nq;
+      lin = (qq < R ? qq * (Q + 1) : R * (Q + 1) + (qq - R) * Q) + jj;
+    }
+    sk = lin / Tt;
+    kind = gp.split_k > 1 ? 1 : 0;
+    return G + lin - sk * Tt;
+  }
+  sk = 1;
+  kind = 3;
+  return u - nls;
+}
+template <typename GPV>
+__device__ __host__ __forceinline__ int bal_static_end(const GPV& gp, int wg) {
+  const int G = gp.full_tiles, nls = (gp.total_tiles - G) * gp.split_k;
+  const int e = xcd_chunk(wg, G) - gp.tail_first, EB = gp.tail_G - gp.tail_first - gp.bal_na;
+  int rounds = 0;
+  if (e >= 0 && e < gp.bal_na) rounds = nls > e ? (nls - e + gp.bal_na - 1) / gp.bal_na : 0;
+  else if (e >= gp.bal_na) rounds = gp.bal_long > e - gp.bal_na ? (gp.bal_long - (e - gp.bal_na) + EB - 1) / EB : 0;
+  return G + rounds * gp.tail_G;
 }
 
 __device__ __forceinline__ const Problem& locate_tile(const GroupParams& gp, int work, int& tm, int& tn, int& sk) {
diff --git a/stable-diffusion-3-from-scratch_amd/csrc/gemm_tile.h b/stable-diffusion-3-from-scratch_amd/csrc/gemm_tile.h
--- a/stable-diffusion-3-from-scratch_amd/csrc/gemm_tile.h
+++ b/stable-diffusion-3-from-scratch_amd/csrc/gemm_tile.h
@@ -1,6 +1,7 @@
 #pragma once
 #include "gemm_common.h"
 #include <type_traits>
+#include <cstddef>
 
 namespace gemm {
 namespace {
@@ -429,6 +430,52 @@
   bool valid;
 };
 
+#define MMDIT_GP_NOW(field) \
+  (*(const volatile int __attribute__((address_space(4)))*)((const char __attribute__((address_space(4)))*)__builtin_amdgcn_kernarg_segment_ptr() + offsetof(GroupParams, field)))
+
+template <bool BAL, typename GPV>
+__device__ __forceinline__ void round_tail_item(const GroupParams& gp, const GPV& sv, int pos, Item& it) {
+  if constexpr (BAL) {
+    if (sv.bal_kmain > 0) {
+      int sk, kind;
+      const int t = bal_work(sv, pos, (int)blockIdx.x, sk, kind);
+      const Problem& p = locate_in_problem(gp, t, it.tm, it.tn);
+      const int per = (p.nk + sv.split_k - 1) / sv.split_k;
+      int kt0 = 0, kt1 = p.nk;
+      if (kind == 1) { kt0 = sk * per; kt1 = max(kt0, min(p.nk, kt0 + per)); }
+      else if (kind == 2) kt1 = sv.bal_kmain;
+      else if (kind == 3) kt0 = sv.bal_kmain;
+      it.pi = (int)(&p - &gp.p[0]);
+      it.h0 = 2 * kt0;
+      it.h1 = 2 * kt1;
+      it.sk = sk;
+      it.atomic = kind != 0;
+      it.tile = t;
+      return;
+    }
+  }
+  int sk, t;
+  if (sv.tail_first >= 0 && pos >= sv.full_tiles) {
+    const int rnd = (pos - sv.full_tiles) / sv.tail_G, l = xcd_chunk((int)blockIdx.x, sv.full_tiles);
+    const int Tt = sv.total_tiles - sv.full_tiles, u = rnd * (sv.tail_G - sv.tail_first) + l - sv.tail_first;
+    sk = u / Tt;
+    t = sv.full_tiles + u - sk * Tt;
+  } else {
+    t = work_tile(sv, pos, sk);
+  }
+  const Problem& p = locate_in_problem(gp, t, it.tm, it.tn);
+  const int S = is_split_work(sv, pos) ? sv.split_k : 1;
+  const int nk_all = p.nk, per = (nk_all + S - 1) / S;
+  const int kt0 = sk * per, kt1 = max(kt0, min(nk_all, kt0 + per));
+  it.pi = (int)(&p - &gp.p[0]);
+  it.h0 = 2 * kt0;
+  it.h1 = 2 * kt1;
+  it.sk = sk;
+  it.atomic = S > 1;
+  it.tile = t;
+}
+
+template <bool BAL = false>
 __device__ __forceinline__ Item item_at(const GroupParams& gp, int pos, int end) {
   Item it;
   it.pos = pos;
@@ -451,26 +498,12 @@
     it.h1 = 2 * k1;
     it.sk = k0 == 0 ? 0 : 1;
     it.atomic = true;
+  } else if constexpr (BAL) {
+    const SchedView sv = {MMDIT_GP_NOW(total_tiles), MMDIT_GP_NOW(split_k), MMDIT_GP_NOW(full_tiles), MMDIT_GP_NOW(tail_first), MMDIT_GP_NOW(tail_rounds),
+                          MMDIT_GP_NOW(tail_G), MMDIT_GP_NOW(bal_kmain), MMDIT_GP_NOW(bal_long), MMDIT_GP_NOW(bal_na)};
+    round_tail_item<true>(gp, sv, pos, it);
   } else {
-    int sk, t;
-    if (gp.tail_first >= 0 && pos >= gp.full_tiles) {
-      const int rnd = (pos - gp.full_tiles) / gp.tail_G, l = xcd_chunk((int)blockIdx.x, gp.full_tiles);
-      const int Tt = gp.total_tiles - gp.full_tiles, u = rnd * (gp.tail_G - gp.tail_first) + l - gp.tail_first;
-      sk = u / Tt;
-      t = gp.full_tiles + u - sk * Tt;
-    } else {
-      t = work_tile(gp, pos, sk);
-    }
-    const Problem& p = locate_in_problem(gp, t, it.tm, it.tn);
-    const int S = is_split_work(gp, pos) ? gp.split_k : 1;
-    const int nk_all = p.nk, per = (nk_all + S - 1) / S;
-    const int kt0 = sk * per, kt1 = max(kt0, min(nk_all, kt0 + per));
-    it.pi = (int)(&p - &gp.p[0]);
-    it.h0 = 2 * kt0;
-    it.h1 = 2 * kt1;
-    it.sk = sk;
-    it.atomic = S > 1;
-    it.tile = t;
+    round_tail_item<false>(gp, gp, pos, it);
   }
   return it;
 }
```
